# Nelarius/rayfinder

Hardware: AMD Instinct MI355X
Metric: Mrays/sec at 1920x1080 Sponza, 8 bounces; achieved HBM GB/s on traversal (higher is better)
Workload: dtype f32

## Files before the change

rayfinder_amd/csrc/rf_device.hpp:

```cpp
#pragma once

#include "rf_types.hpp"

#include <hip/hip_runtime.h>

namespace rf
{
constexpr int      kBlock = 256;
constexpr int      kLdsStack = 24;
constexpr int      kSpillStack = 72;
constexpr uint32_t kMiss = 0xFFFFFFFFu;
constexpr uint32_t kLeafAxis = 3u;
constexpr uint32_t kTriStride = 4u;

struct DeviceScene
{
    const float4*            nodes;
    const float4*            triangles;
    const float4*            attributes;
    const float4*            shadeRecords;
    const TextureDescriptor* textureDescriptors;
    const uint32_t*          texels;
    uint64_t                 numTexels;
    const uint8_t*           blueNoise;
    const float*             albedoLut;
};

#if defined(__HIPCC__)
struct RayPrep
{
    Vec3     origin;
    Vec3     direction;
    Vec3     invDir;
    uint32_t negX, negY, negZ;
};

__device__ __forceinline__ RayPrep prepareRay(Vec3 o, Vec3 d)
{
    RayPrep r;
    r.origin = o;
    r.direction = d;
    r.invDir = vec3(1.0f / d.x, 1.0f / d.y, 1.0f / d.z);
    r.negX = r.invDir.x < 0.0f;
    r.negY = r.invDir.y < 0.0f;
    r.negZ = r.invDir.z < 0.0f;
    return r;
}

__device__ __forceinline__ bool slabTest(const RayPrep& r, float4 lo, float4 hi, float rayTMax)
{
    float       tmin = ((r.negX ? hi.x : lo.x) - r.origin.x) * r.invDir.x;
    float       tmax = ((r.negX ? lo.x : hi.x) - r.origin.x) * r.invDir.x;
    const float tymin = ((r.negY ? hi.y : lo.y) - r.origin.y) * r.invDir.y;
    const float tymax = ((r.negY ? lo.y : hi.y) - r.origin.y) * r.invDir.y;
    if ((tmin > tymax) || (tymin > tmax)) return false;
    tmin = maxf(tymin, tmin);
    tmax = minf(tymax, tmax);
    const float tzmin = ((r.negZ ? hi.z : lo.z) - r.origin.z) * r.invDir.z;
    const float tzmax = ((r.negZ ? lo.z : hi.z) - r.origin.z) * r.invDir.z;
    if ((tmin > tzmax) || (tzmin > tmax)) return false;
    tmin = maxf(tzmin, tmin);
    tmax = minf(tzmax, tmax);
    return (tmin < rayTMax) && (tmax > 0.0f);
}

__device__ __forceinline__ Vec3 offsetRay(Vec3 p, Vec3 n)
{
    constexpr float kOrigin = 1.0f / 32.0f;
    constexpr float kFloatScale = 1.0f / 65536.0f;
    constexpr float kIntScale = 256.0f;
    const int       ox = static_cast<int>(kIntScale * n.x);
    const int       oy = static_cast<int>(kIntScale * n.y);
    const int       oz = static_cast<int>(kIntScale * n.z);
    const Vec3      shifted = vec3(__int_as_float(__float_as_int(p.x) + (p.x < 0 ? -ox : ox)),
                                   __int_as_float(__float_as_int(p.y) + (p.y < 0 ? -oy : oy)),
                                   __int_as_float(__float_as_int(p.z) + (p.z < 0 ? -oz : oz)));
    return vec3(fabsf(p.x) < kOrigin ? p.x + kFloatScale * n.x : shifted.x,
                fabsf(p.y) < kOrigin ? p.y + kFloatScale * n.y : shifted.y,
                fabsf(p.z) < kOrigin ? p.z + kFloatScale * n.z : shifted.z);
}

struct TriangleHit
{
    float t, u, v;
};

__device__ __forceinline__ bool
intersectTriangle(Vec3 origin, Vec3 direction, Vec3 p0, Vec3 p1, Vec3 p2, float rayTMax, TriangleHit& hit)
{
    constexpr float kEpsilon = 0.00001f;
    const Vec3      e1 = p1 - p0;
    const Vec3      e2 = p2 - p0;
    const Vec3      h = cross(direction, e2);
    const float     det = dot(e1, h);
    if (det > -kEpsilon && det < kEpsilon) return false;
    const float invDet = 1.0f / det;
    const Vec3  s = origin - p0;
    const float u = invDet * dot(s, h);
    if (u < 0.0f || u > 1.0f) return false;
    const Vec3  q = cross(s, e1);
    const float v = invDet * dot(direction, q);
    if (v < 0.0f || u + v > 1.0f) return false;
    const float t = invDet * dot(e2, q);
    if (t > kEpsilon && t < rayTMax)
    {
        hit.t = t;
        hit.u = u;
        hit.v = v;
        return true;
    }
    return false;
}
__device__ __forceinline__ bool
intersectTriangle(const RayPrep& r, Vec3 p0, Vec3 p1, Vec3 p2, float rayTMax, TriangleHit& hit)
{
    return intersectTriangle(r.origin, r.direction, p0, p1, p2, rayTMax, hit);
}

struct ClosestHit
{
    uint32_t triangle;
    float    t, u, v;
    Vec3     p;
};

struct TraversalCounters
{
    uint32_t nodesVisited = 0;
    uint32_t triangleTests = 0;
    uint32_t stackHigh = 0;
    uint32_t abandoned = 0;
};

template<bool ANY_HIT, bool COUNT, int LDS = kLdsStack>
__device__ __forceinline__ bool traverse(const DeviceScene& scene, Vec3 origin, Vec3 direction, float rayTMax,
                                         uint32_t* ldsStackLane, ClosestHit& out, TraversalCounters& counters)
{
    const RayPrep ray = prepareRay(origin, direction);
    constexpr int kSpill = kLdsStack + kSpillStack - LDS;
    uint32_t      spill[kSpill];
    int           stackSize = 0;
    uint32_t      current = 0;
    bool          found = false;
    out.triangle = kMiss;

    for (;;)
    {
        const float4 lo = scene.nodes[2 * current];
        const float4 hi = scene.nodes[2 * current + 1];
        if (COUNT) ++counters.nodesVisited;
        bool advance = false;
        if (slabTest(ray, lo, hi, rayTMax))
        {
            const uint32_t link = __float_as_uint(lo.w);
            const uint32_t meta = __float_as_uint(hi.w);
            const uint32_t axis = meta & 3u;
            if (axis == kLeafAxis)
            {
                const uint32_t count = meta >> 2;
                for (uint32_t i = 0; i < count; ++i)
                {
                    const uint32_t tri = link + i;
                    const float4   a = scene.triangles[kTriStride * tri];
                    const float4   b = scene.triangles[kTriStride * tri + 1];
                    const float4   c = scene.triangles[kTriStride * tri + 2];
                    if (COUNT) ++counters.triangleTests;
                    TriangleHit th;
                    const Vec3  p0 = vec3(a.x, a.y, a.z), p1 = vec3(b.x, b.y, b.z), p2 = vec3(c.x, c.y, c.z);
                    if (intersectTriangle(ray, p0, p1, p2, rayTMax, th))
                    {
                        if (ANY_HIT) return true;
                        rayTMax = th.t;
                        found = true;
                        const Vec3 e1 = p1 - p0, e2 = p2 - p0;
                        const Vec3 p = p0 + th.u * e1 + th.v * e2;
                        const Vec3 n = normalize(cross(e1, e2));
                        out.p = offsetRay(p, n);
                        out.t = th.t;
// ... 46 lines not shown
    if (x < -745.0) return 0.0;
    const double k = __builtin_rint(x * 1.44269504088896338700e+00);
    double       r = __builtin_fma(-k, 6.93147180369123816490e-01, x);
    r = __builtin_fma(-k, 1.90821492927058770002e-10, r);
    double p = 1.6059043836821613e-10;
    p = __builtin_fma(p, r, 2.08767569878681e-09);
    p = __builtin_fma(p, r, 2.505210838544172e-08);
    p = __builtin_fma(p, r, 2.755731922398589e-07);
    p = __builtin_fma(p, r, 2.7557319223985893e-06);
    p = __builtin_fma(p, r, 2.48015873015873e-05);
    p = __builtin_fma(p, r, 0.0001984126984126984);
    p = __builtin_fma(p, r, 0.001388888888888889);
    p = __builtin_fma(p, r, 0.008333333333333333);
    p = __builtin_fma(p, r, 0.041666666666666664);
    p = __builtin_fma(p, r, 0.16666666666666666);
    p = __builtin_fma(p, r, 0.5);
    p = __builtin_fma(p, r, 1.0);
    p = __builtin_fma(p, r, 1.0);
    return __builtin_ldexp(p, static_cast<int>(k));
}
__device__ __forceinline__ double dReduce(double x, long long& quadrant)
{
    const double k = __builtin_rint(x * 6.36619772367581382433e-01);
    double       r = __builtin_fma(-k, 1.57079632673412561417e+00, x);
    r = __builtin_fma(-k, 6.07710050650619224932e-11, r);
    r = __builtin_fma(-k, 2.02226624879595063154e-21, r);
    quadrant = static_cast<long long>(k);
    return r;
}
__device__ __forceinline__ double dSinCosKernel(double r, bool cosine)
{
    const double z = r * r;
    const double c5 = cosine ? -1.13596475577881948265e-11 : 1.58969099521155010221e-10, c4 = cosine ? 2.08757232129817482790e-09 : -2.50507602534068634195e-08;
    const double c3 = cosine ? -2.75573143513906633035e-07 : 2.75573137070700676789e-06, c2 = cosine ? 2.48015872894767294178e-05 : -1.98412698298579493134e-04;
    const double c1 = cosine ? -1.38888888888741095749e-03 : 8.33333333332248946124e-03, c0 = cosine ? 4.16666666666666019037e-02 : -1.66666666666666324348e-01;
    const double t = c0 + z * (c1 + z * (c2 + z * (c3 + z * (c4 + z * c5))));
    return cosine ? (1.0 - 0.5 * z) + (z * z) * t : r + (r * z) * t;
}
__device__ __forceinline__ double dSin(double x)
{
    if (!(__builtin_fabs(x) < 1.0e15)) return x - x;
    long long    q;
    const double r = dReduce(x, q), v = dSinCosKernel(r, (q & 1) != 0);
    return (q & 2) ? -v : v;
}
__device__ __forceinline__ double dCos(double x)
{
    if (!(__builtin_fabs(x) < 1.0e15)) return x - x;
    long long    q;
    const double r = dReduce(x, q), v = dSinCosKernel(r, (q & 1) == 0);
    return ((q + 1) & 2) ? -v : v;
}
__device__ __forceinline__ double dAcosRatio(double z)
{
    const double p = z * (1.66666666666666657415e-01 + z * (-3.25565818622400915405e-01 + z * (2.01212532134862925881e-01 + z * (-4.00555345006794114027e-02 + z * (7.91534994289814532176e-04 + z * 3.47933107596021167570e-05)))));
    const double q = 1.0 + z * (-2.40339491173441421878e+00 + z * (2.02094576023350569471e+00 + z * (-6.88283971605453293030e-01 + z * 7.70381505559019352791e-02)));
    return p / q;
}
__device__ __forceinline__ double dAcos(double x)
{
    const double pio2_hi = 1.57079632679489655800e+00, pio2_lo = 6.12323399573676603587e-17, pi = 3.14159265358979311600e+00;
    if (x != x) return x;
    if (__builtin_fabs(x) >= 1.0)
    {
        if (x == 1.0) return 0.0;
        if (x == -1.0) return pi + 2.0 * pio2_lo;
        return (x - x) / (x - x);
    }
    const bool   small = __builtin_fabs(x) < 0.5, negative = x < 0.0;
    if (small && __builtin_fabs(x) <= 6.938893903907228e-18) return pio2_hi + pio2_lo;
    const double z = small ? x * x : (negative ? (1.0 + x) * 0.5 : (1.0 - x) * 0.5);
    const double r = dAcosRatio(z);
    if (small) return pio2_hi - (x - (pio2_lo - x * r));
    const double s = __builtin_sqrt(z);
    if (negative)
    {
        const double w = r * s - pio2_lo;
        return pi - 2.0 * (s + w);
    }
    const double df = __longlong_as_double(__double_as_longlong(s) & static_cast<long long>(0xFFFFFFFF00000000ull));
    const double c = (z - df * df) / (s + df), w = r * s + c;
    return 2.0 * (df + w);
}
__device__ __forceinline__ float wSin(float x) { return static_cast<float>(dSin(static_cast<double>(x))); }
__device__ __forceinline__ float wCos(float x) { return static_cast<float>(dCos(static_cast<double>(x))); }
__device__ __forceinline__ float wAcos(float x) { return static_cast<float>(dAcos(static_cast<double>(x))); }
__device__ __forceinline__ float wExp(float x) { return static_cast<float>(dExp(static_cast<double>(x))); }
__device__ __forceinline__ float wPow(float x, float y)
{
    return static_cast<float>(pow(static_cast<double>(x), static_cast<double>(y)));
}
__device__ __forceinline__ float wPow15(float x)
{
    const double xd = static_cast<double>(x);
    return static_cast<float>(xd * __builtin_sqrt(xd));
}
__device__ __forceinline__ float wFract(float x) { return x - floorf(x); }

template<bool F32> __device__ __forceinline__ float tSin(float x) { if constexpr (F32) return sinf(x); else return wSin(x); }
template<bool F32> __device__ __forceinline__ float tCos(float x) { if constexpr (F32) return cosf(x); else return wCos(x); }
template<bool F32> __device__ __forceinline__ float tAcos(float x) { if constexpr (F32) return acosf(x); else return wAcos(x); }
template<bool F32> __device__ __forceinline__ float tExp(float x) { if constexpr (F32) return expf(x); else return wExp(x); }
template<bool F32> __device__ __forceinline__ float tPow15(float x) { if constexpr (F32) return powf(x, 1.5f); else return wPow15(x); }

constexpr float kPi = 3.1415927f;
constexpr float kFrac1Pi = 0.31830987f;
constexpr float kTMax = 10000.0f;
constexpr uint32_t kSolarCosThetaMaxBits = 0x3F7FFF5Au;
constexpr uint32_t kSolarInvPdfBits = 0x38826048u;

__host__ __device__ __forceinline__ void pixarOnb(Vec3 n, Vec3& u, Vec3& v)
{
    const float s = (n.z >= 0.0f) ? 1.0f : -1.0f;
    const float a = -1.0f / (s + n.z);
    const float b = n.x * n.y * a;
    u = vec3(1.0f + s * n.x * n.x * a, s * b, -s * n.x);
    v = vec3(b, s + n.y * n.y * a, -n.y);
}

__device__ __forceinline__ Vec3 basisTimes(Vec3 c0, Vec3 c1, Vec3 c2, Vec3 v)
{
    return (v.x * c0 + v.y * c1) + v.z * c2;
}

template<bool F32 = false>
__device__ __forceinline__ float skyRadiance(const SkyStateGpu& sky, float cosTheta, float gamma, float cosGamma, int channel)
{
    const float  r = sky.skyRadiances[channel];
    const float* p = sky.params + 9 * channel;
    const float  cosGamma2 = cosGamma * cosGamma;
    const float  expM = tExp<F32>(p[4] * gamma);
    const float  mieLhs = 1.0f + cosGamma2;
    const float  mieRhs = tPow15<F32>(1.0f + p[8] * p[8] - 2.0f * p[8] * cosGamma);
    const float  mie = mieLhs / mieRhs;
    const float  zenith = rf_sqrt(cosTheta);
    const float  lhs = 1.0f + p[0] * tExp<F32>(p[1] / (cosTheta + 0.01f));
    const float  rhs = p[2] + p[3] * expM + p[5] * cosGamma2 + p[6] * mie + p[7] * zenith;
    return r * (lhs * rhs);
}

__device__ __forceinline__ Vec3 evalTexture(const DeviceScene& scene, const float* lut, uint32_t descriptorIdx, float uvx, float uvy)
{
    const TextureDescriptor d = scene.textureDescriptors[descriptorIdx];
    const float             u = wFract(uvx);
    const float             v = wFract(uvy);
    const uint32_t          j = static_cast<uint32_t>(u * static_cast<float>(d.width));
    const uint32_t          i = static_cast<uint32_t>(v * static_cast<float>(d.height));
    uint64_t                idx = static_cast<uint64_t>(d.offset) + static_cast<uint64_t>(i * d.width + j);
    if (idx >= scene.numTexels) idx = scene.numTexels - 1;
    const uint32_t bgra = scene.texels[idx];
    return vec3(lut[(bgra >> 16) & 0xffu], lut[(bgra >> 8) & 0xffu], lut[bgra & 0xffu]);
}

__device__ __forceinline__ void animatedBlueNoiseN(const uint8_t* table, uint32_t x, uint32_t y, uint32_t n, float& nx, float& ny)
{
    const uint32_t idx = (y % 128u) * 128u + (x % 128u);
    const float    bx = static_cast<float>(table[2 * idx]) / 255.0f;
    const float    by = static_cast<float>(table[2 * idx + 1]) / 255.0f;
    const float    a1 = 0.7548776662466927f;
    const float    a2 = 0.5698402909980532f;
    nx = wFract(bx + wFract(a1 * static_cast<float>(n)));
    ny = wFract(by + wFract(a2 * static_cast<float>(n)));
}
__device__ __forceinline__ void animatedBlueNoise(const uint8_t* table, uint32_t x, uint32_t y, uint32_t frameIdx, uint32_t totalSampleCount, float& nx, float& ny)
{
    animatedBlueNoiseN(table, x, y, frameIdx % totalSampleCount, nx, ny);
}
#endif
}
```

rayfinder_amd/csrc/rf_kernels.hpp:

```cpp
#pragma once

#include "rf_renderer.hpp"

#include "rf_bvh.hpp"
#include "rf_camera.hpp"
#include "rf_data.hpp"
#include "rf_device.hpp"
#include "rf_hip_host.hpp"
#include "rf_wide.hpp"

#include <hip/hip_runtime.h>

#include <algorithm>
#include <cfloat>
#include <cmath>
#include <cstdio>
#include <cstdlib>
#include <cstring>
#include <functional>
#include <stdexcept>
#include <string>
#include <type_traits>

namespace rf
{
namespace kern
{
struct __attribute__((packed, aligned(4))) P3
{
    float x, y, z;
};

struct PathStreams
{
    P3*     rayO;
    P3*     rayD;
    P3*     thr;
    float4* rad;
    float4* hit;
    P3*     pending;
    P3*     noise;
    P3*     rayDOut;
    P3*     thrOut;
    P3*     noiseOut;
};

typedef float v3f __attribute__((ext_vector_type(3)));
__device__ __forceinline__ Vec3 load3(const float4* p)
{
    const v3f v = *reinterpret_cast<const v3f*>(p);
    return vec3(v.x, v.y, v.z);
}
__device__ __forceinline__ Vec3 load3(const P3* p)
{
    const P3 v = *p;
    return vec3(v.x, v.y, v.z);
}
__device__ __forceinline__ void store3(P3* p, Vec3 v)
{
    P3 o;
    o.x = v.x, o.y = v.y, o.z = v.z;
    *p = o;
}
typedef float v3fu __attribute__((ext_vector_type(3), aligned(4)));
__device__ __forceinline__ void store3nt(P3* p, Vec3 v)
{
    v3fu o;
    o.x = v.x, o.y = v.y, o.z = v.z;
    __builtin_nontemporal_store(o, reinterpret_cast<v3fu*>(p));
}
__device__ __forceinline__ Vec3 load3nt(const P3* p)
{
    const v3fu v = __builtin_nontemporal_load(reinterpret_cast<const v3fu*>(p));
    return vec3(v.x, v.y, v.z);
}

__device__ __forceinline__ Vec3     load3s(const float4* p) { return load3(p); }
__device__ __forceinline__ Vec3     load3s(const P3* p) { return load3(p); }
__device__ __forceinline__ uint32_t loadQ(const uint32_t* p) { return *p; }
__device__ __forceinline__ void     store4s(float4* p, float x, float y, float z, float w) { *p = make_float4(x, y, z, w); }

struct DeviceCounters
{
    unsigned long long primaryRays, closestRays, shadowRays;
    unsigned long long closestNodeVisits, closestTriangleTests, shadowNodeVisits, shadowTriangleTests;
    unsigned int       stackHigh;
    unsigned int       pad;
    unsigned long long closestRecordFetches, shadowRecordFetches;
    unsigned long long descendTrips[2], leafTrips[2], leafPhases[2], refillTrips[2], popLaneTrips[2], outerTrips[2];
    unsigned long long scalarRedo[2];
    unsigned long long abandonedRays;
    unsigned long long occluderTried, occluderHit, occludedRays;
    unsigned long long descendParked[2], descendIdle[2], leafInterior[2], leafIdle[2];
};

struct FastDiv
{
    uint32_t mul, shift1, shift2, divisor;
    static FastDiv make(uint32_t d)
    {
        FastDiv f{0u, 0u, 0u, d ? d : 1u};
        uint32_t l = 0;
        while ((1ull << l) < f.divisor) ++l;
        f.mul = static_cast<uint32_t>(((1ull << 32) * ((1ull << l) - f.divisor)) / f.divisor + 1ull);
        f.shift1 = l < 1u ? l : 1u;
        f.shift2 = l > 1u ? l - 1u : 0u;
        return f;
    }
    __host__ __device__ __forceinline__ uint32_t div(uint32_t n) const
    {
#if defined(__HIP_DEVICE_COMPILE__)
        const uint32_t t = __umulhi(mul, n);
#else
        const uint32_t t = static_cast<uint32_t>((static_cast<uint64_t>(mul) * n) >> 32);
#endif
        return (t + ((n - t) >> shift1)) >> shift2;
    }
    __host__ __device__ __forceinline__ void divmod(uint32_t n, uint32_t& q, uint32_t& r) const
    {
        q = div(n);
        r = n - q * divisor;
    }
};

struct FrameParams
{
    uint32_t width, height;
    Camera   camera;
    uint32_t samplesPerPixel, numBounces;
    uint32_t firstFrame;
    uint32_t numSamples;
    uint32_t numTiles;
    uint32_t pixelsPadded;
    uint32_t slotGroupShift;
    const uint32_t* samplePerm;
    const uint32_t* sampleInvPerm;
    uint32_t tilesX;
    uint32_t skipOrigins;
    const uint32_t* tileValidBefore;
    uint32_t        validPixels;
    FastDiv         divNumSamples, divPixelsPadded, divTilesX, divSamplesPerPixel;
};

__device__ __forceinline__ uint32_t validRankInTile(uint32_t w, uint32_t vw, uint32_t vh)
{
    const uint32_t block = w >> 6, lane = w & 63u, bx = block & 3u, by = block >> 2, lx = lane & 7u, ly = lane >> 3;
    const uint32_t ch = min(8u, vh - min(vh, 8u * by)), cw = min(8u, vw - min(vw, 8u * bx));
    return vw * min(vh, 8u * by) + ch * min(vw, 8u * bx) + cw * ly + lx;
}

constexpr uint32_t kSlotSampleMajor = 31u;

__device__ __forceinline__ void slotToSamplePixel(const FrameParams& fp, uint32_t slot, uint32_t& k, uint32_t& lp)
{
    if (fp.slotGroupShift == kSlotSampleMajor) fp.divPixelsPadded.divmod(slot, k, lp);
    else
    {
        const uint32_t g = fp.slotGroupShift, chunk = slot >> g;
        uint32_t       group;
        fp.divNumSamples.divmod(chunk, group, k);
        lp = (group << g) + (slot & ((1u << g) - 1u));
    }
}
__device__ __forceinline__ size_t samplePixelToSlot(const FrameParams& fp, uint32_t k, uint32_t lp)
{
    if (fp.slotGroupShift == kSlotSampleMajor) return static_cast<size_t>(k) * fp.pixelsPadded + lp;
    const uint32_t g = fp.slotGroupShift;
    return ((static_cast<size_t>(lp >> g) * fp.numSamples + k) << g) + (lp & ((1u << g) - 1u));
}

__device__ __forceinline__ bool localPixelToXY(const FrameParams& fp, const uint32_t* tileIds, uint32_t lp, uint32_t& x, uint32_t& y)
{
    const uint32_t tile = tileIds[lp >> 10];
    const uint32_t w = lp & 1023u;
    const uint32_t block = w >> 6, lane = w & 63u;
    uint32_t       tileX, tileY;
    fp.divTilesX.divmod(tile, tileY, tileX);
    x = tileX * kTileSize + (block & 3u) * 8u + (lane & 7u);
    y = tileY * kTileSize + (block >> 2) * 8u + (lane >> 3);
    return x < fp.width && y < fp.height;
}

constexpr int kItems = 4;

template<int ITEMS>
__device__ __forceinline__ void blockAppend(const bool (&keep)[ITEMS], const uint32_t (&slot)[ITEMS], uint32_t* queue, uint32_t* count, uint32_t* sScratch,
                                            uint32_t (*position)[ITEMS] = nullptr, const uint32_t (*second)[ITEMS] = nullptr, uint32_t* queue2 = nullptr)
{
    const uint32_t lane = __lane_id(), wave = threadIdx.x >> 6;
    uint32_t       offs[ITEMS];
    uint32_t       waveTotal = 0;
#pragma unroll
    for (int k = 0; k < ITEMS; ++k)
    {
        const unsigned long long mask = __ballot(keep[k]);
        offs[k] = waveTotal + __popcll(mask & ((1ull << lane) - 1ull));
        waveTotal += __popcll(mask);
    }
    if (lane == 0) sScratch[wave] = waveTotal;
    __syncthreads();
    if (threadIdx.x == 0)
    {
        const uint32_t total = sScratch[0] + sScratch[1] + sScratch[2] + sScratch[3];
        sScratch[4] = total ? atomicAdd(count, total) : 0u;
    }
    __syncthreads();
    uint32_t base = sScratch[4];
    for (uint32_t w = 0; w < wave; ++w) base += sScratch[w];
#pragma unroll
    for (int k = 0; k < ITEMS; ++k)
    {
        if (keep[k]) queue[base + offs[k]] = slot[k];
        if (second != nullptr && keep[k]) queue2[base + offs[k]] = (*second)[k];
        if (position) (*position)[k] = base + offs[k];
    }
    __syncthreads();
}

__device__ __forceinline__ unsigned long long waveSum(unsigned long long v)
{
    for (int off = 32; off > 0; off >>= 1) v += __shfl_down(v, off);
    return v;
}
__device__ __forceinline__ uint32_t waveMax(uint32_t v)
{
    for (int off = 32; off > 0; off >>= 1) v = max(v, static_cast<uint32_t>(__shfl_down(v, off)));
    return v;
}

template<bool MAX>
__device__ __forceinline__ uint32_t waveScanInclusive(uint32_t x)
{
    const auto step = [&](auto ctrl, auto rowMask) {
        const uint32_t y = static_cast<uint32_t>(__builtin_amdgcn_update_dpp(0, static_cast<int>(x), decltype(ctrl)::value, decltype(rowMask)::value, 0xF, true));
        x = MAX ? max(x, y) : x + y;
    };
    step(std::integral_constant<int, 0x111>{}, std::integral_constant<int, 0xF>{});
    step(std::integral_constant<int, 0x112>{}, std::integral_constant<int, 0xF>{});
    step(std::integral_constant<int, 0x114>{}, std::integral_constant<int, 0xF>{});
    step(std::integral_constant<int, 0x118>{}, std::integral_constant<int, 0xF>{});
    step(std::integral_constant<int, 0x142>{}, std::integral_constant<int, 0xA>{});
    step(std::integral_constant<int, 0x143>{}, std::integral_constant<int, 0xC>{});
    return x;
}
__device__ __forceinline__ uint32_t laneGather(uint32_t value, uint32_t srcLane) { return static_cast<uint32_t>(__builtin_amdgcn_ds_bpermute(static_cast<int>(srcLane << 2), static_cast<int>(value))); }
__device__ __forceinline__ float    laneGather(float value, uint32_t srcLane) { return __uint_as_float(laneGather(__float_as_uint(value), srcLane)); }

__device__ __forceinline__ uint32_t sampleKey(uint32_t firstFrame, uint32_t spp, uint32_t k)
{
    const uint32_t n = (firstFrame + k) % spp;
    const float    rx = wFract(0.7548776662466927f * static_cast<float>(n)), ry = wFract(0.5698402909980532f * static_cast<float>(n));
    uint32_t       x = static_cast<uint32_t>(rx * 65536.0f) & 0xFFFFu, y = static_cast<uint32_t>(ry * 65536.0f) & 0xFFFFu;
    const auto     spread = [](uint32_t v) {
        v = (v | (v << 8)) & 0x00FF00FFu;
        v = (v | (v << 4)) & 0x0F0F0F0Fu;
        v = (v | (v << 2)) & 0x33333333u;
        v = (v | (v << 1)) & 0x55555555u;
        return v;
    };
    return spread(x) | (spread(y) << 1);
}

__device__ __forceinline__ Vec3 hitPoint(const DeviceScene& scene, uint32_t tri, float u, float v)
{
    const Vec3 p0 = load3(scene.triangles + kTriStride * tri), p1 = load3(scene.triangles + kTriStride * tri + 1),
               p2 = load3(scene.triangles + kTriStride * tri + 2);
    const Vec3   e1 = p1 - p0, e2 = p2 - p0;
    const Vec3   p = p0 + u * e1 + v * e2;
    return offsetRay(p, normalize(cross(e1, e2)));
}

struct SunBasis
{
    Vec3 u, v;
};

__device__ __forceinline__ Vec3 sunSample(const SkyStateGpu& sky, const SunBasis& basis, float nx, float cosPhi, float sinPhi)
{
    const float cosThetaMax = __uint_as_float(kSolarCosThetaMaxBits);
    const float cosTheta = 1.0f - nx * (1.0f - cosThetaMax);
    const float sinTheta = rf_sqrt(1.0f - cosTheta * cosTheta);
    const Vec3  local = vec3(cosPhi * sinTheta, sinPhi * sinTheta, cosTheta);
    const Vec3  sun = vec3(sky.sunDirection[0], sky.sunDirection[1], sky.sunDirection[2]);
    return basisTimes(basis.u, basis.v, sun, local);
}

constexpr uint32_t kShadeLastBounce = 1u, kShadeFirstBounce = 2u;
constexpr uint32_t kShadeSelfShadow = 4u;
constexpr uint32_t kLookFirstBounce = 1u, kLookNoRayCount = 2u;


constexpr uint32_t kSortBins = 256;
#if defined(RF_EXP_ACC_PIXELS)
constexpr uint32_t kAccPixels = RF_EXP_ACC_PIXELS;
#else
constexpr uint32_t kAccPixels = 4;
#endif
constexpr uint32_t kAccMaxSamples = 1024;
constexpr uint32_t kAovPixels = 8, kAovChunk = 32;

constexpr uint32_t kChunk = 128;
constexpr uint32_t kShards = 16;
constexpr uint32_t kLineWords = 16;
constexpr uint32_t kRefillMin = 40;
constexpr uint32_t kLeafVote = 20;

constexpr int kLayoutBinary = 0, kLayoutCompact = 1, kLayoutHot = 2, kLayoutQuad = 3, kLayoutQuadHalf = 4, kLayoutQuadLocal = 5, kLayoutOct = 6, kLayoutScalar = 7, kLayoutPacket = 8;
constexpr uint32_t kFlagShadowDirFromStream = 1u;
constexpr uint32_t kFlagUniformTri = 8u;
constexpr uint32_t kFlagUniformFetch = 4u;
constexpr uint32_t kFlagFirstBounce = 2u;
constexpr uint32_t kFlagOccluderCache = 16u;
constexpr uint32_t kFlagOccluderNoTry = 32u;
constexpr uint32_t kFlagNoRayCount = 64u;
constexpr uint32_t kFlagConstOrigin = 128u;
constexpr uint32_t kFlagDenseLeafShift = 8u;
#if defined(RF_EXP_OCC_SLOTS)
constexpr int kOccSlots = RF_EXP_OCC_SLOTS;
#else
constexpr int kOccSlots = 4;
#endif
static_assert(kOccSlots == 1 || kOccSlots == 2 || kOccSlots == 4, "one aligned load per cell");
constexpr uint32_t kNodeIdle = 0xFFFFFFFFu;
constexpr uint32_t kNodeDone = 0xFFFFFFFEu;


using SamplePermutationKernel = void (*)(uint32_t firstFrame, uint32_t spp, uint32_t numSamples, uint32_t* perm, uint32_t* inv);
using RaygenKernel = void (*)(FrameParams fp, DeviceScene scene, const uint32_t* tileIds, PathStreams ps, uint32_t* queue, uint32_t* queueCount, DeviceCounters* counters);
using TraceClosestKernel = void (*)(DeviceScene scene, PathStreams ps, const uint32_t* queue, const uint32_t* queueCount, DeviceCounters* counters);
using ShadeKernel = void (*)(DeviceScene scene, SkyStateGpu sky, SunBasis sunBasis, PathStreams ps, const uint32_t* queue, const uint32_t* queueCount, uint32_t* hitQueue, uint32_t* hitCount, uint32_t* missQueue, uint32_t* missSlots, uint32_t* missCount, uint32_t* shadowList, uint32_t* shadowListCount, uint32_t bounceFlags, uint32_t sortScale, float4* aov);
using SkyKernel = void (*)(SkyStateGpu sky, PathStreams ps, const uint32_t* missSlots, const uint32_t* missQueue, const uint32_t* missCount, uint32_t firstBounce);
using TraceShadowKernel = void (*)(DeviceScene scene, SkyStateGpu sky, SunBasis sunBasis, PathStreams ps, const uint32_t* queue, const uint32_t* queueCount, DeviceCounters* counters, uint32_t firstBounce);
using TraceWideKernel = void (*)(DeviceScene scene, WideScene wide, SkyStateGpu sky, SunBasis sunBasis, PathStreams ps, const uint32_t* queue, const uint32_t* queueCount, uint32_t* cursor, DeviceCounters* counters, uint32_t refillMin, uint32_t leafVote, uint32_t chunkMax, float tMax, uint32_t flags);
using ShadowFirstLookKernel = void (*)(DeviceScene scene, WideScene wide, SkyStateGpu sky, SunBasis sunBasis, PathStreams ps, const uint32_t* queue, const uint32_t* inList, const uint32_t* inCount, uint32_t* list, uint32_t* listCount, DeviceCounters* counters, float tMax, uint32_t flags);
using TracePacketKernel = void (*)(DeviceScene scene, WideScene wide, SkyStateGpu sky, SunBasis sunBasis, PathStreams ps, const uint32_t* queue, const uint32_t* queueCount, DeviceCounters* counters, float tMax, uint32_t flags);
using HitPointsKernel = void (*)(DeviceScene scene, const float4* hit, P3* rayO, uint32_t n);
using BounceTotalsKernel = void (*)(const uint32_t* queueCounts, uint32_t numBounces, unsigned long long* totals, const uint32_t* listCounts, unsigned long long lookMask, unsigned long long* lookBatch, const uint32_t* shadowListCounts, unsigned long long selfMask, DeviceCounters* counters);
using AccumulateKernel = void (*)(FrameParams fp, const uint32_t* tileIds, PathStreams ps, float4* image);
using AccumulateRunsKernel = void (*)(FrameParams fp, const uint32_t* tileIds, PathStreams ps, float4* image);
using AccumulateAovKernel = void (*)(FrameParams fp, const uint32_t* tileIds, const float4* aov, float4* albedoCoverage, float4* normalDepth);
using TonemapKernel = void (*)(const float4* image, uint32_t n, uint32_t accumulatedSamples, float exposure, uint32_t* out);
using PrimaryStatsKernel = void (*)(DeviceScene scene, Camera cam, uint32_t width, uint32_t height, uint32_t* nodesVisited, uint8_t* hitOut, float* tOut, uint32_t* triTests, DeviceCounters* counters);
using IntersectRaysKernel = void (*)(DeviceScene scene, const float* rays, uint64_t n, float tMax, uint32_t* triOut, float* tOut, float* uvOut, float* pOut, uint32_t* nvOut, uint32_t* ttOut, DeviceCounters* counters);
using OccludedRaysKernel = void (*)(DeviceScene scene, const float* rays, uint64_t n, float tMax, float* visOut, DeviceCounters* counters);
using DeferredLightingKernel = void (*)(DeviceScene scene, SkyStateGpu sky, SunBasis sunBasis, Camera cam, uint32_t width, uint32_t height, uint32_t frameCount, float jitterX, float jitterY, float exposure, float* sampleBuffer, float* accumulationBuffer, uint32_t* bgraOut, DeviceCounters* counters);

TraceWideKernel       traceWideKernel(bool anyHit, bool count, bool nearestFirst, int compact, bool denseLeaves);
TraceClosestKernel    traceClosestKernel(bool count);
TraceShadowKernel     traceShadowKernel(bool count);
ShadowFirstLookKernel shadowFirstLookKernel();
TracePacketKernel     tracePacketKernel(bool anyHit);
HitPointsKernel       hitPointsKernel();
PrimaryStatsKernel    primaryStatsKernel();
IntersectRaysKernel   intersectRaysKernel();
OccludedRaysKernel    occludedRaysKernel();
SamplePermutationKernel samplePermutationKernel();
RaygenKernel            raygenKernel(bool f32Transcendentals);
ShadeKernel             shadeKernel(bool sorted, bool aov = false);
SkyKernel               skyKernel(bool f32Transcendentals);
BounceTotalsKernel      bounceTotalsKernel();
AccumulateKernel        accumulateKernel();
AccumulateRunsKernel    accumulateRunsKernel(uint32_t pixelsPerWorkgroup);
AccumulateAovKernel     accumulateAovKernel(bool runs);
TonemapKernel           tonemapKernel();
DeferredLightingKernel  deferredLightingKernel();
}
using namespace kern;
}
```

rayfinder_amd/csrc/rf_renderer.hip:

```cpp
#include "rayfinder_amd.h"
#include "rf_denoise.hpp"
#include "rf_kernels.hpp"
#include "rf_noise.hpp"

#include <map>

#include <algorithm>
#include <cfloat>
#include <cmath>
#include <cstdio>
#include <cstdlib>
#include <cstring>
#include <functional>
#include <stdexcept>
#include <string>
#include <type_traits>

namespace rf
{
bool operator==(const RenderParameters& a, const RenderParameters& b)
{
    return a.width == b.width && a.height == b.height && std::memcmp(&a.camera, &b.camera, sizeof(Camera)) == 0 &&
           a.samplingParams == b.samplingParams && a.sky == b.sky && a.exposure == b.exposure;
}

namespace
{
uint32_t tileMortonKey(uint32_t tx, uint32_t ty)
{
    const auto spread = [](uint32_t v) {
        v &= 0xFFFFu;
        v = (v | (v << 8)) & 0x00FF00FFu;
        v = (v | (v << 4)) & 0x0F0F0F0Fu;
        v = (v | (v << 2)) & 0x33333333u;
        v = (v | (v << 1)) & 0x55555555u;
        return v;
    };
    return spread(tx) | (spread(ty) << 1);
}
}

std::vector<uint32_t> tilesForRank(uint32_t width, uint32_t height, uint32_t rank, uint32_t worldSize)
{
    const uint32_t tilesX = TileGrid(width, height).tilesX, n = TileGrid(width, height).count();
    std::vector<uint32_t> order(n);
    for (uint32_t i = 0; i < n; ++i) order[i] = i;
    if (worldSize > 1)
    {
        std::stable_sort(order.begin(), order.end(), [tilesX](uint32_t a, uint32_t b) { return tileMortonKey(a % tilesX, a / tilesX) < tileMortonKey(b % tilesX, b / tilesX); });
    }
    std::vector<uint32_t> mine;
    for (uint32_t i = 0; i < n; ++i)
        if ((i % worldSize + i / worldSize) % worldSize == rank) mine.push_back(order[i]);
    std::sort(mine.begin(), mine.end());
    return mine;
}

void untileHost(const float* compact, const uint32_t* tileIds, uint32_t numTiles, uint32_t width, uint32_t height, float* image)
{
    untileHostTexels(compact, tileIds, numTiles, width, height, 4 * sizeof(float), image);
}

void untileHostTexels(const void* compact, const uint32_t* tileIds, uint32_t numTiles, uint32_t width, uint32_t height, size_t texelBytes, void* image)
{
    const uint32_t tilesX = TileGrid(width, height).tilesX;
    const auto*    src = static_cast<const unsigned char*>(compact);
    auto*          dst = static_cast<unsigned char*>(image);
    for (uint32_t t = 0; t < numTiles; ++t)
    {
        const uint32_t tx = tileIds[t] % tilesX, ty = tileIds[t] / tilesX;
        for (uint32_t w = 0; w < kTileSize * kTileSize; ++w)
        {
            const uint32_t block = w >> 6, lane = w & 63u;
            const uint32_t x = tx * kTileSize + (block & 3u) * 8u + (lane & 7u);
            const uint32_t y = ty * kTileSize + (block >> 2) * 8u + (lane >> 3);
            if (x >= width || y >= height) continue;
            std::memcpy(dst + texelBytes * (static_cast<size_t>(y) * width + x), src + texelBytes * (static_cast<size_t>(t) * 1024 + w), texelBytes);
        }
    }
}

struct SumChannel
{
    bool                 on = false;
    bool                 dirty = true;
    uint32_t             samples = 0;
    DeviceBuffer<float4> buffers[2];
    uint32_t             numBuffers = 0;

    SumChannel(bool on_, uint32_t numBuffers_) : on(on_), numBuffers(numBuffers_) {}
    void restart()
    {
        samples = 0;
        dirty = true;
    }
    void release()
    {
        for (auto& b : buffers) b.release();
    }
    bool covers(uint32_t accumulated) const { return !dirty && samples == accumulated; }
    bool empty() const { return !on || dirty || samples == 0u; }
    void zeroIfStale(hipStream_t stream, uint64_t pixelsPadded)
    {
        if (!on || !dirty) return;
        if (numBuffers != 0u && buffers[0].count < pixelsPadded)
        {
            RF_HIP(hipStreamSynchronize(stream));
            for (uint32_t i = 0; i < numBuffers; ++i) buffers[i].alloc(pixelsPadded);
        }
        for (uint32_t i = 0; i < numBuffers; ++i) RF_HIP(hipMemsetAsync(buffers[i].ptr, 0, pixelsPadded * sizeof(float4), stream));
        dirty = false;
    }
};

struct Renderer::Impl
{
    int         device = 0;
    hipStream_t stream = nullptr;

    DeviceBuffer<float4>            nodes, triangles, wideNodes, wideCompact, wideHot, wideOwn, wideQuad;
    DeviceBuffer<uint4>             wideQuadHalf, wideQuadLocal, wideOct;
    DeviceBuffer<uint2>             bigLeaves;
    WideScene                       wide{};
    DeviceBuffer<float4>            attributes;
    DeviceBuffer<float4>            shadeRecords;
    DeviceBuffer<TextureDescriptor> textureDescriptors;
    DeviceBuffer<uint32_t>          texels;
    DeviceBuffer<uint8_t>           blueNoise;
    DeviceBuffer<float>             albedoLut;
    DeviceScene                     scene{};

    RenderParameters params;
    SkyStateGpu      sky{};
    SunBasis         sunBasis{};

    void updateSunBasis() { pixarOnb(vec3(sky.sunDirection[0], sky.sunDirection[1], sky.sunDirection[2]), sunBasis.u, sunBasis.v); }
    uint32_t         maxWidth = 0, maxHeight = 0;
    uint32_t         frameCount = 0, accumulated = 0;
    uint32_t         rank = 0, worldSize = 1;

    std::vector<uint32_t>   tiles;
    DeviceBuffer<uint32_t>  tileIds;
    DeviceBuffer<uint32_t>  tileValidBefore;
    bool                    optDenseRaygen = true;
    DeviceBuffer<float4>    ownedImage;
    float4*                 image = nullptr;
    uint64_t                imageBytes = 0;
    SumChannel              imageSums{true, 0};
    SumChannel              aovSums{false, 2};
    uint32_t                aovFlags = 0;
    bool                    aovTileCounts() const { return (aovFlags & kAovTileCounts) != 0u; }
    SumChannel              momentSums{false, 1};
    float4*                 aovAlbedoCoverage() const { return aovSums.buffers[0].ptr; }
    float4*                 aovNormalDepth() const { return aovSums.buffers[1].ptr; }
    float4*                 moments() const { return momentSums.buffers[0].ptr; }
    DenoiseWork             denoiseWork;
    bool                    denoisedValid = false;
    uint32_t                denoisedSamples = 0;
    NoiseWork               noiseWork;
    std::vector<uint32_t>   tileSamples;
    DeviceBuffer<uint32_t>  tileSamplesDevice;
    DeviceBuffer<float4>    meanImage;

    bool nonUniform() const { return !tileSamples.empty(); }
    void requireUniform(const char* what, const char* unless = "") const
    {
        if (nonUniform())
            throw std::invalid_argument(std::string(what) + ": the tiles hold different sample counts after rf_renderer_render_adaptive" + unless +
                                        " (continue with render_adaptive, or restart the accumulation with rf_renderer_set_render_parameters)");
    }

    uint64_t                validPixels = 0;
    unsigned long long      primaryRaysHost = 0;
    uint64_t                maxPaths = 0;
    DeviceBuffer<P3>        sRayO, sRayD, sRayD2, sThr, sThr2, sPending, sNoise, sNoise2;
    DeviceBuffer<float4>    sRad, sHit;
    DeviceBuffer<float4>    sAov;
    DeviceBuffer<uint32_t>  queueA, queueB, missQueue, missSlots, shadowList, queueCounts;
    DeviceBuffer<DeviceCounters> counters;
    DeviceBuffer<unsigned long long> bounceTotals;

    uint32_t               deferredFrameCount = 0;
    DeviceBuffer<float>    deferredSample, deferredAccum;
    DeviceBuffer<uint32_t> deferredBgra;

    bool counting = false, timing = false;
    int      traversalVariant = 2;
    uint32_t wideBlocks = 0;
    bool     wideBlocksForced = false;
    uint32_t multiProcessors = 0;
    std::map<std::pair<const void*, uint32_t>, uint32_t> residentCache;
    uint32_t skyBlocks = 2048;
    bool     wideUsable = true;
    int      queryVariant = 0;
    bool     shadowNearestFirst = true;
    uint32_t optShadowFirstLookFromBounce = 2;
    bool     occluderGridWarm = false;
    DeviceBuffer<unsigned long long> lookBatch;
    unsigned long long*              lookBatchHost = nullptr;
    hipEvent_t                       lookEvent = nullptr;
    bool                             lookPending = false;
    uint32_t                         firstLookHoldOff = 0;
    uint32_t occluderHintLevels = 0;
    bool     leafBoxesValid = false;
    uint32_t optOccluderGridLog2Cells = 22;
    uint32_t optOccluderGridCells = 1024;
    DeviceBuffer<uint32_t> occluderGrid;
    uint32_t optOccluderCacheBounces = 64;
    bool     optShadowSignOrder = true;
    uint32_t optRefillMin = kRefillMin, optLeafVote = kLeafVote, optChunk = kChunk;
    uint32_t optLeafVoteClosest = 14;
    uint32_t optDenseLeafMin = 5, optDenseLeafFromBounce = 1;
    uint32_t maxLeafTriangles = 0;
    uint32_t optShadeSortFromBounce = 2, sortScale = 0;
    uint32_t optChunkEarly = 256, optChunkEarlyBounces = 2;
    uint32_t optRefillMinDeep = 12, optRefillMinDeepDense = 22, optRefillMinDeepQuad = 40, optRefillDeepFromBounce = 2;
    uint32_t optShadeBlocks = 0;
    bool     optTranscendentalsF32 = false;
    bool     optShadowSelfTest = true;
    bool     selfShadowOk = false;
    bool     optConstPrimaryOrigin = true;
    bool                   optSampleSort = true, optAccumulateRuns = true;
    uint32_t               optCompactFromBounce = 3;
    uint32_t               optCompactShadowFromBounce = 2;
    uint32_t               optQuadFromBounce = 1, optQuadShadowFromBounce = 1;
    uint32_t               optQuadExceptMask = 0, optQuadShadowExceptMask = 0;
    uint32_t               optQuadHalfFromBounce = 0, optQuadHalfShadowFromBounce = 0;
    float                  quadHalfAreaRatio = 0.0f;
    uint32_t               optQuadLocalFromBounce = 0, optQuadLocalShadowFromBounce = 0;
    uint32_t               optOctFromBounce = 0;
    uint64_t               treeBytes = 0;
    uint32_t               optHotFromBounce = 0, optHotShadowFromBounce = 0;
    int                    optQueryCompact = 0;
    uint32_t               optExtraLds = 0;
    uint32_t               optPacketBounces = 0;
    int                    optUniformFetch = 2;
    DeviceBuffer<uint32_t> samplePerm;
    uint32_t optSlotGroupShift = 0;
    RenderStats hostStats;

    struct TimedLaunch
    {
        hipEvent_t start, stop;
        int        kind;
        uint32_t   bounce;
    };
    std::vector<TimedLaunch> timed;
    std::vector<hipEvent_t>  eventPool;

    struct BatchTiming
    {
        hipEvent_t start, stop;
        uint32_t   samples;
    };
    std::vector<BatchTiming> pendingBatches;
    std::deque<float>        passDurationsMs;

    hipEvent_t getEvent()
    {
        if (!eventPool.empty())
        {
            hipEvent_t e = eventPool.back();
            eventPool.pop_back();
            return e;
        }
        hipEvent_t e;
        RF_HIP(hipEventCreate(&e));
        return e;
    }

    uint64_t allocatedPaths = 0;
    uint64_t effectivePaths = 0;

    static constexpr uint64_t kBytesPerPath = 8 * sizeof(P3) + 2 * sizeof(float4) + 5 * sizeof(uint32_t);
    static constexpr uint64_t kAovBytesPerPath = 2 * sizeof(float4);
    uint64_t bytesPerPath() const { return kBytesPerPath + (aovSums.on ? kAovBytesPerPath : 0u); }
    uint64_t pathStateBytes() const { return allocatedPaths * kBytesPerPath + sAov.count * sizeof(float4); }
    bool pathStateHolds(uint64_t paths) const { return paths <= allocatedPaths && (!aovSums.on || sAov.count >= 2 * paths); }

    void releasePathState()
    {
        sRayO.release(), sRayD.release(), sRayD2.release(), sThr.release(), sThr2.release(), sRad.release(), sHit.release();
        sPending.release(), sNoise.release(), sNoise2.release(), queueA.release(), queueB.release(), missQueue.release(), missSlots.release(), shadowList.release();
        sAov.release();
        allocatedPaths = 0;
    }

    bool ensurePathState(uint64_t paths)
    {
        if (pathStateHolds(paths)) return true;
        RF_HIP(hipStreamSynchronize(stream));
        releasePathState();
        const auto tryAlloc = [](auto& buf, uint64_t n) -> bool {
            void* p = nullptr;
            const hipError_t e = hipMalloc(&p, n * sizeof(*buf.ptr));
            if (e == hipErrorOutOfMemory || e == hipErrorMemoryAllocation)
            {
                (void)hipGetLastError();
                return false;
            }
            RF_HIP(e);
            buf.ptr = static_cast<decltype(buf.ptr)>(p);
            buf.count = n;
            return true;
        };
        const bool ok = tryAlloc(sRayO, paths) && tryAlloc(sRayD, paths) && tryAlloc(sRayD2, paths) && tryAlloc(sThr, paths) && tryAlloc(sThr2, paths) &&
                        tryAlloc(sRad, paths) && tryAlloc(sHit, paths) && tryAlloc(sPending, paths) && tryAlloc(sNoise, paths) && tryAlloc(sNoise2, paths) &&
                        tryAlloc(queueA, paths) && tryAlloc(queueB, paths) && tryAlloc(missQueue, paths) && tryAlloc(missSlots, paths) && tryAlloc(shadowList, paths) &&
                        (!aovSums.on || tryAlloc(sAov, 2 * paths));
        if (!ok)
        {
            releasePathState();
            return false;
        }
        allocatedPaths = paths;
        return true;
    }

    uint64_t pathsThatFit()
    {
        size_t freeBytes = 0, totalBytes = 0;
        RF_HIP(hipMemGetInfo(&freeBytes, &totalBytes));
        const uint64_t budget = static_cast<uint64_t>(freeBytes) + pathStateBytes();
        return budget / 10 * 9 / bytesPerPath();
    }

    void configureShard()
    {
// ... 124 lines not shown
        uint32_t occMask;
        bool     firstLookReady;
        bool     runs, tileList;
        uint32_t accumulateKernel, accumulatePixels, aovPixels, momentPixels;
    };
    struct BouncePlan
    {
        TraversalPlan closest, shadow;
        bool          shadeSorted, shadeAov;
        uint32_t      shadeFlags, sortScale, skyFirstBounce;
        uint32_t      itemGridCap;
        bool          cached, firstLook, selfShadow;
        uint32_t      lookFlags, shadowSource;
    };
    struct BatchCounters
    {
        uint32_t*                 base;
        uint32_t                  numBounces;
        static constexpr uint32_t kLine = kLineWords, kCursorWords = kLine * kShards;
        uint32_t words() const { return kLine * (2 * numBounces + 1) + kCursorWords * 2 * numBounces + kLine * numBounces + kLine * numBounces; }
        uint32_t queueWord(uint32_t b) const { return kLine * b; }
        uint32_t missWord(uint32_t b) const { return kLine * (numBounces + 1) + kLine * (b - 1); }
        uint32_t cursorClosestWord(uint32_t b) const { return kLine * (2 * numBounces + 1) + kCursorWords * 2 * (b - 1); }
        uint32_t cursorShadowWord(uint32_t b) const { return cursorClosestWord(b) + kCursorWords; }
        uint32_t listWord(uint32_t b) const { return kLine * (2 * numBounces + 1) + kCursorWords * 2 * numBounces + kLine * (b - 1); }
        uint32_t shadowListWord(uint32_t b) const { return listWord(b) + kLine * numBounces; }
        uint32_t shadowCountWord(uint32_t b, uint32_t source) const { return source == kFromLookList ? listWord(b) : (source == kFromShadeList ? shadowListWord(b) : queueWord(b)); }
        uint32_t* queueCount(uint32_t b) const { return base + queueWord(b); }
        uint32_t* missCount(uint32_t b) const { return base + missWord(b); }
        uint32_t* cursorClosest(uint32_t b) const { return base + cursorClosestWord(b); }
        uint32_t* cursorShadow(uint32_t b) const { return base + cursorShadowWord(b); }
        uint32_t* listCount(uint32_t b) const { return base + listWord(b); }
        uint32_t* shadowListCount(uint32_t b) const { return base + shadowListWord(b); }
        uint32_t* shadowCount(uint32_t b, uint32_t source) const { return base + shadowCountWord(b, source); }
    };
    struct WideArgs
    {
        PathStreams     ps;
        const uint32_t* queue;
        const uint32_t* count;
        uint32_t*       cursor;
        float           tMax;
        dim3            grid;
        uint32_t        blocksWanted = 0;
    };
    uint32_t residentBlocks(TraceWideKernel k, uint32_t extraLds)
    {
        const auto key = std::make_pair(reinterpret_cast<const void*>(k), extraLds);
        const auto it = residentCache.find(key);
        if (it != residentCache.end()) return it->second;
        int perCu = 0;
        RF_HIP(hipOccupancyMaxActiveBlocksPerMultiprocessor(&perCu, reinterpret_cast<const void*>(k), kBlock, extraLds));
        const uint32_t n = static_cast<uint32_t>(std::max(perCu, 1)) * std::max(multiProcessors, 1u);
        residentCache[key] = n;
        return n;
    }
    void launchWide(const TraversalPlan& t, const WideScene& w, const WideArgs& a)
    {
        const TraceWideKernel k = traceWideKernel(t.anyHit, t.count, t.nearest, t.layout, t.dense);
        if (k == nullptr) throw std::logic_error("kTraceWide: record layout " + std::to_string(t.layout) + " is not compiled into this build");
        dim3 grid = a.grid;
        if (a.blocksWanted != 0u && !wideBlocksForced && !t.count) grid = dim3(std::min(a.blocksWanted, residentBlocks(k, t.extraLds)));
        hipLaunchKernelGGL(k, grid, dim3(kBlock), t.extraLds, stream, scene, w, sky, sunBasis, a.ps, a.queue, a.count, a.cursor, counters.ptr, t.refillMin, t.leafVote, t.chunk, a.tMax, t.flags);
    }
    int layoutIfPresent(int want) const
    {
        switch (want)
        {
        case kLayoutOct: return wide.oct != nullptr ? want : kLayoutBinary;
        case kLayoutQuadLocal: return wide.quadLocal != nullptr ? want : kLayoutBinary;
        case kLayoutQuadHalf: return wide.quadHalf != nullptr ? want : kLayoutBinary;
        case kLayoutQuad: return wide.quad != nullptr ? want : kLayoutBinary;
        case kLayoutHot: return wide.hot != nullptr ? want : kLayoutBinary;
        case kLayoutCompact: return wide.compact != nullptr ? want : kLayoutBinary;
        default: return kLayoutBinary;
        }
    }
    bool denseWanted(uint32_t flags) const
    {
        const uint32_t threshold = (flags >> kFlagDenseLeafShift) & 15u;
        return threshold != 0u && maxLeafTriangles >= threshold;
    }
    static bool conservativeLayout(int layout) { return layout == kLayoutQuadLocal || layout == kLayoutQuadHalf; }
    static bool worksThroughList(int layout) { return layout == kLayoutQuad || layout == kLayoutQuadHalf || layout == kLayoutQuadLocal; }
    TraversalPlan resolveTraversal(bool anyHit, int layout, bool count, bool nearest, uint32_t flags, uint32_t refillMin, uint32_t chunk, uint32_t leafVote, uint32_t extraLds) const
    {
        TraversalPlan t{};
        t.kernel = layout == kLayoutScalar ? kKernelScalar : (layout == kLayoutPacket ? kKernelPacket : kKernelWide);
        t.layout = layout, t.anyHit = anyHit, t.count = count, t.flags = flags;
        if (t.kernel != kKernelWide) return t;
        if (count) t.layout = kLayoutBinary, t.nearest = anyHit && nearest;
        else if (!anyHit) t.layout = layout <= kLayoutOct ? layout : kLayoutBinary;
        else
        {
            t.layout = (layout <= kLayoutQuadLocal) ? layout : kLayoutBinary;
            t.nearest = (t.layout == kLayoutCompact || t.layout == kLayoutHot) ? true : nearest;
        }
        t.dense = !count && denseWanted(flags) && traceWideKernel(anyHit, false, t.nearest, t.layout, true) != nullptr;
        t.refillMin = refillMin, t.chunk = chunk, t.leafVote = leafVote ? leafVote : optLeafVote, t.extraLds = extraLds;
        return t;
    }
    int closestLayoutFor(uint32_t bounce) const
    {
        if (traversalVariant == 0) return kLayoutScalar;
        if (counting) return kLayoutBinary;
#if defined(RF_EXP_LEGACY_LAYOUTS)
        if (bounce <= optPacketBounces) return kLayoutPacket;
#endif
        const bool  quadNow = wide.quad != nullptr && optQuadFromBounce != 0u && bounce >= optQuadFromBounce && !((optQuadExceptMask >> std::min(bounce - 1u, 31u)) & 1u);
        const float camReach = std::max({std::fabs(params.camera.origin.x), std::fabs(params.camera.origin.y), std::fabs(params.camera.origin.z)}) + (std::fabs(params.camera.lensRadius) * 2.0f);
        const bool  primaryOutside = bounce == 1u && !(camReach <= wide.originBound);
        if (quadNow && !primaryOutside)
        {
            if (wide.oct != nullptr && optOctFromBounce != 0u && bounce >= optOctFromBounce) return kLayoutOct;
            if (wide.quadHalf != nullptr && optQuadHalfFromBounce != 0u && bounce >= optQuadHalfFromBounce) return kLayoutQuadHalf;
            if (wide.quadLocal != nullptr && optQuadLocalFromBounce != 0u && bounce >= optQuadLocalFromBounce) return kLayoutQuadLocal;
        }
        if (quadNow) return kLayoutQuad;
        if (wide.hot != nullptr && optHotFromBounce != 0u && bounce >= optHotFromBounce) return kLayoutHot;
        if (wide.compact != nullptr && optCompactFromBounce != 0u && bounce >= optCompactFromBounce) return kLayoutCompact;
        return kLayoutBinary;
    }
    int shadowLayoutFor(uint32_t bounce) const
    {
        if (traversalVariant == 0) return kLayoutScalar;
#if defined(RF_EXP_LEGACY_LAYOUTS)
        if (!counting && bounce <= optPacketBounces) return kLayoutPacket;
#endif
        if (counting || !shadowNearestFirst) return kLayoutBinary;
        const bool quadShadowNow = optQuadShadowFromBounce != 0u && bounce >= optQuadShadowFromBounce && !((optQuadShadowExceptMask >> std::min(bounce - 1u, 31u)) & 1u);
        if (quadShadowNow)
        {
            if (wide.quadLocal != nullptr && optQuadLocalShadowFromBounce != 0u && bounce >= optQuadLocalShadowFromBounce) return kLayoutQuadLocal;
            if (wide.quadHalf != nullptr && optQuadHalfShadowFromBounce != 0u && bounce >= optQuadHalfShadowFromBounce) return kLayoutQuadHalf;
            if (wide.quad != nullptr) return kLayoutQuad;
        }
        if (wide.hot != nullptr && optHotShadowFromBounce != 0u && bounce >= optHotShadowFromBounce) return kLayoutHot;
        if (wide.compact != nullptr && optCompactShadowFromBounce != 0u && bounce >= optCompactShadowFromBounce) return kLayoutCompact;
        return kLayoutBinary;
    }
    bool cachedShadowFor(uint32_t bounce) const
    {
        const int layout = shadowLayoutFor(bounce);
        const bool exactQuad = layout == kLayoutQuad && leafBoxesValid;
        return layout != kLayoutScalar && layout != kLayoutPacket && !counting && shadowNearestFirst && (conservativeLayout(layout) || exactQuad) && bounce <= optOccluderCacheBounces &&
               optOccluderGridCells != 0u;
    }

    struct ActiveTiles
    {
        uint32_t numTiles;
        uint64_t validPixels;
    };
    BatchPlan planBatch(uint32_t numSamples, const ActiveTiles* active) const
    {
        BatchPlan b{};
        const uint64_t validPixels = active ? active->validPixels : this->validPixels;
        b.numSamples = numSamples;
        b.numBounces = params.samplingParams.numBounces;
        b.numTiles = active ? active->numTiles : static_cast<uint32_t>(tiles.size());
        b.pixelsPadded = b.numTiles * 1024u;
        b.samplePerm = optSampleSort && numSamples > 1 && numSamples <= 8192 && optSlotGroupShift != kSlotSampleMajor;
        const auto finite3 = [](Vec3 v) { return std::isfinite(v.x) && std::isfinite(v.y) && std::isfinite(v.z); };
        const Camera& camNow = params.camera;
        b.primaryLayout = closestLayoutFor(1);
        b.constOrigin = optConstPrimaryOrigin && camNow.lensRadius == 0.0f && camNow.origin.x != 0.0f && camNow.origin.y != 0.0f && camNow.origin.z != 0.0f &&
                        finite3(camNow.origin) && finite3(camNow.right) && finite3(camNow.up) && b.primaryLayout != kLayoutScalar && b.primaryLayout != kLayoutPacket;
        b.denseRaygen = optDenseRaygen && (optSlotGroupShift == 0u || optSlotGroupShift == kSlotSampleMajor) && static_cast<uint64_t>(validPixels) * numSamples <= 0xFFFFFFFFull;
        b.occluderGrid = optOccluderCacheBounces != 0u && optOccluderGridCells != 0u;
        if (b.occluderGrid)
        {
            b.occluderGridEntries = (uint64_t{1} << optOccluderGridLog2Cells) * kOccSlots;
            const float extent = std::max({wide.rootHi.x - wide.rootLo.x, wide.rootHi.y - wide.rootLo.y, wide.rootHi.z - wide.rootLo.z, 1e-20f});
            b.occScale = static_cast<float>(optOccluderGridCells) / extent;
            b.occMask = static_cast<uint32_t>(b.occluderGridEntries / kOccSlots - 1);
        }
        b.runs = optSlotGroupShift == 0u && numSamples > 4u && optAccumulateRuns;
        b.tileList = active != nullptr;
        const uint32_t perThread = static_cast<uint32_t>(kBlock);
        if (b.tileList) b.accumulateKernel = kAccumulateTiles, b.accumulatePixels = b.runs ? kMomentPixels : perThread;
        else if (b.runs && numSamples <= kAccMaxSamples)
        {
            b.accumulateKernel = kAccumulateRuns, b.accumulatePixels = numSamples > 640u ? 1u : (numSamples > 160u ? 2u : kAccPixels);
        }
        else b.accumulateKernel = kAccumulatePixels, b.accumulatePixels = perThread;
        b.aovPixels = (aovSums.on && b.numBounces != 0u) ? (b.runs ? kAovPixels : perThread) : 0u;
        b.momentPixels = (!b.tileList && momentSums.on) ? (b.runs ? kMomentPixels : perThread) : 0u;
        return b;
    }
    bool nextBatchFirstLookReady(const BatchPlan& b) const
    {
        if (!b.occluderGrid || occluderGrid.count != b.occluderGridEntries || !occluderGridWarm) return false;
        if (lookPending && hipEventQuery(lookEvent) == hipSuccess) return !(lookBatchHost[1] != 0ull && lookBatchHost[0] * 4ull < lookBatchHost[1]) && firstLookHoldOff == 0u;
        return firstLookHoldOff <= 1u;
    }
    BouncePlan planBounce(uint32_t bounce, const BatchPlan& batch) const
    {
        BouncePlan p{};
        const uint32_t uniformFlag = ((optUniformFetch < 0 ? bounce <= 2 : optUniformFetch > 0) ? kFlagUniformFetch : 0u) | (optUniformFetch >= 2 ? kFlagUniformTri : 0u) |
                                     (bounce >= optDenseLeafFromBounce ? (std::min(optDenseLeafMin, 15u) << kFlagDenseLeafShift) : 0u);
        const uint32_t chunkNow = bounce <= optChunkEarlyBounces ? optChunkEarly : optChunk;
        const int      layoutClosest = closestLayoutFor(bounce);
        const uint32_t refillClosest = bounce >= optRefillDeepFromBounce ? (layoutClosest == kLayoutQuad ? optRefillMinDeepQuad : (denseWanted(uniformFlag) ? optRefillMinDeepDense : optRefillMinDeep)) : optRefillMin;
        const uint32_t leafVoteClosest = (!counting && !denseWanted(uniformFlag) && treeBytes <= (192ull << 20)) ? optLeafVoteClosest : 0u;
        const bool     wideClosest = layoutClosest != kLayoutScalar && layoutClosest != kLayoutPacket;
        p.closest = resolveTraversal(false, layoutClosest, counting, false, wideClosest ? (uniformFlag | (bounce == 1 && batch.constOrigin ? kFlagConstOrigin : 0u)) : 0u,
                                     counting ? optRefillMin : refillClosest, chunkNow, leafVoteClosest, counting ? 0u : optExtraLds);
        const int layoutShadow = shadowLayoutFor(bounce);
        p.selfShadow = optShadowSelfTest && selfShadowOk && !counting && bounce <= 64u && worksThroughList(layoutShadow);
        p.shadeAov = aovSums.on && bounce == 1;
        p.shadeSorted = !p.shadeAov && optShadeSortFromBounce != 0u && bounce >= optShadeSortFromBounce;
        p.shadeFlags = (bounce == batch.numBounces ? kShadeLastBounce : 0u) | (bounce == 1 ? kShadeFirstBounce : 0u) | (p.selfShadow ? kShadeSelfShadow : 0u);
        p.sortScale = p.shadeSorted ? sortScale : 0u;
        p.skyFirstBounce = bounce == 1 ? 1u : 0u;
        p.itemGridCap = optShadeBlocks;
        p.cached = cachedShadowFor(bounce);
        p.firstLook = p.cached && occluderHintLevels == 0u && optShadowFirstLookFromBounce != 0u && bounce >= optShadowFirstLookFromBounce && bounce <= 64u && batch.firstLookReady;
        p.shadowSource = p.firstLook ? kFromLookList : (p.selfShadow ? kFromShadeList : kFromQueue);
        p.lookFlags = p.firstLook ? ((bounce == 1 ? kLookFirstBounce : 0u) | (p.selfShadow ? kLookNoRayCount : 0u)) : 0u;
        const uint32_t shadowFlags = (bounce == 1 ? kFlagFirstBounce : 0u) | uniformFlag | (p.cached ? kFlagOccluderCache : 0u) | (p.firstLook ? (kFlagOccluderNoTry | kFlagNoRayCount) : 0u) | (p.selfShadow ? kFlagNoRayCount : 0u);
        const bool nearest = shadowNearestFirst && !(conservativeLayout(layoutShadow) && optShadowSignOrder);
        const uint32_t flagsRun = layoutShadow == kLayoutScalar ? (bounce == 1 ? 1u : 0u) : (layoutShadow == kLayoutPacket ? (shadowFlags & kFlagFirstBounce) : shadowFlags);
        p.shadow = resolveTraversal(true, layoutShadow, counting, nearest, flagsRun, optRefillMin, chunkNow, 0u, counting ? 0u : optExtraLds);
        return p;
    }

    void queryWide(const float* rays6, uint64_t n, float tMax, bool shadow, std::vector<float4>& out0, std::vector<float4>& out1)
    {
        if (n > 0xFFFFFFFFull) throw std::runtime_error("too many rays");
        const uint32_t denseFlag = std::min(optDenseLeafMin, 15u) << kFlagDenseLeafShift;
        if (!ensurePathState(n)) throw std::runtime_error("out of device memory for the ray batch");
        std::vector<P3>       o(n), d(n);
        std::vector<uint32_t> ids(n);
        for (uint64_t i = 0; i < n; ++i)
        {
            o[i] = P3{rays6[6 * i], rays6[6 * i + 1], rays6[6 * i + 2]};
            d[i] = P3{rays6[6 * i + 3], rays6[6 * i + 4], rays6[6 * i + 5]};
            ids[i] = static_cast<uint32_t>(i);
        }
        RF_HIP(hipStreamSynchronize(stream));
        RF_HIP(hipMemcpyAsync(sRayO.ptr, o.data(), n * sizeof(P3), hipMemcpyHostToDevice, stream));
        RF_HIP(hipMemcpyAsync(sRayD.ptr, d.data(), n * sizeof(P3), hipMemcpyHostToDevice, stream));
        RF_HIP(hipMemcpyAsync(queueA.ptr, ids.data(), n * sizeof(uint32_t), hipMemcpyHostToDevice, stream));
        const BatchCounters qc{nullptr, 0u};
        const uint32_t words = qc.words() + BatchCounters::kCursorWords;
        if (queueCounts.count < words) queueCounts.alloc(words);
        RF_HIP(hipMemsetAsync(queueCounts.ptr, 0, queueCounts.count * sizeof(uint32_t), stream));
        const uint32_t count = static_cast<uint32_t>(n);
        RF_HIP(hipMemcpyAsync(queueCounts.ptr, &count, sizeof count, hipMemcpyHostToDevice, stream));
        PathStreams ps{sRayO.ptr, sRayD.ptr, sThr.ptr, sRad.ptr, sHit.ptr, sPending.ptr, sNoise.ptr, sRayD2.ptr, sThr2.ptr, sNoise2.ptr};
        const dim3  grid(std::min<uint32_t>(static_cast<uint32_t>((n + kBlock - 1) / kBlock), wideBlocks));
        const WideArgs wa{ps, queueA.ptr, queueCounts.ptr + qc.queueWord(0), queueCounts.ptr + qc.cursorClosestWord(1), tMax, grid};
        if (shadow)
        {
            std::vector<P3> ones(n, P3{1.0f, 1.0f, 1.0f});
            RF_HIP(hipMemcpyAsync(sPending.ptr, ones.data(), n * sizeof(P3), hipMemcpyHostToDevice, stream));
            RF_HIP(hipMemsetAsync(sRad.ptr, 0, n * sizeof(float4), stream));
            RF_HIP(hipStreamSynchronize(stream));
            const int layout = layoutIfPresent((optQueryCompact == kLayoutOct || (!shadowNearestFirst && optQueryCompact < kLayoutQuad)) ? kLayoutBinary : optQueryCompact);
            launchWide(resolveTraversal(true, layout, false, shadowNearestFirst, kFlagShadowDirFromStream | denseFlag, optRefillMin, optChunk, 0u, 0u), wide, wa);
        }
        else
        {
            WideScene wq = wide;
            wq.rayList = nullptr;
            if (const char* listPath = std::getenv("RF_DEBUG_QUERY_LIST"))
            {
                std::vector<uint32_t> list(n);
                FILE* f = std::fopen(listPath, "rb");
                if (f == nullptr || std::fread(list.data(), sizeof(uint32_t), n, f) != n) throw std::runtime_error("RF_DEBUG_QUERY_LIST: cannot read the ray list");
                std::fclose(f);
                RF_HIP(hipMemcpyAsync(queueB.ptr, list.data(), n * sizeof(uint32_t), hipMemcpyHostToDevice, stream));
                RF_HIP(hipStreamSynchronize(stream));
                wq.rayList = queueB.ptr;
            }
            const bool timed = std::getenv("RF_DEBUG_QUERY_MS") != nullptr;
            hipEvent_t e0 = nullptr, e1 = nullptr;
            if (timed)
            {
                RF_HIP(hipEventCreate(&e0));
                RF_HIP(hipEventCreate(&e1));
                RF_HIP(hipEventRecord(e0, stream));
            }
            launchWide(resolveTraversal(false, layoutIfPresent(optQueryCompact), false, false, denseFlag, optRefillMin, optChunk, 0u, 0u), wq, wa);
            if (timed) RF_HIP(hipEventRecord(e1, stream));
            hipLaunchKernelGGL(hitPointsKernel(), dim3((count + 255) / 256), dim3(256), 0, stream, scene, sHit.ptr, sRayO.ptr, count);
            if (timed)
            {
                RF_HIP(hipStreamSynchronize(stream));
                float ms = 0.0f;
                RF_HIP(hipEventElapsedTime(&ms, e0, e1));
                std::fprintf(stderr, "[rf-query] closest-hit launch: %u rays, %.4f ms\n", count, ms);
                RF_HIP(hipEventDestroy(e0));
                RF_HIP(hipEventDestroy(e1));
            }
        }
        RF_HIP(hipGetLastError());
        RF_HIP(hipStreamSynchronize(stream));
        out0.resize(n);
        RF_HIP(hipMemcpy(out0.data(), shadow ? sRad.ptr : sHit.ptr, n * sizeof(float4), hipMemcpyDeviceToHost));
        if (!shadow)
        {
            std::vector<P3> packed(n);
            RF_HIP(hipMemcpy(packed.data(), sRayO.ptr, n * sizeof(P3), hipMemcpyDeviceToHost));
            out1.resize(n);
            for (uint64_t i = 0; i < n; ++i) out1[i] = make_float4(packed[i].x, packed[i].y, packed[i].z, 0.0f);
        }
    }

    void clearStaleSums(uint64_t pixelsPadded)
    {
        zeroImageIfStale(pixelsPadded * sizeof(float4));
        aovSums.zeroIfStale(stream, pixelsPadded);
        momentSums.zeroIfStale(stream, pixelsPadded);
    }

    uint32_t batchSamples(uint32_t todo, uint64_t pixelsPadded)
    {
        uint32_t       n = 0;
        uint64_t       depth = maxPaths;
        for (;;)
        {
            const uint32_t perBatch = static_cast<uint32_t>(std::max<uint64_t>(1, depth / pixelsPadded));
            const uint32_t numBatches = (todo + perBatch - 1) / perBatch;
            n = (todo + numBatches - 1) / numBatches;
            const uint64_t need = static_cast<uint64_t>(n) * pixelsPadded;
            if (pathStateHolds(need)) break;
            const uint64_t fit = pathsThatFit();
            if (need > fit && n > 1)
            {
                depth = std::max<uint64_t>(pixelsPadded, std::min(depth / 2, fit));
                continue;
            }
            if (ensurePathState(need)) break;
            if (n == 1) throw std::runtime_error("out of device memory: one sample of the frame (" + std::to_string(need * bytesPerPath() >> 20) + " MiB of path state) does not fit");
            depth = std::max<uint64_t>(pixelsPadded, depth / 2);
        }
        if (depth != effectivePaths)
        {
            if (depth < maxPaths)
                std::fprintf(stderr, "[rf] device memory is short: batches of %llu paths instead of the configured %llu (%u samples per batch); same image, shorter launches\n",
                             static_cast<unsigned long long>(depth), static_cast<unsigned long long>(maxPaths), n);
            else if (effectivePaths != 0 && effectivePaths < maxPaths)
                std::fprintf(stderr, "[rf] device memory is back: batches of the configured %llu paths again\n", static_cast<unsigned long long>(maxPaths));
            effectivePaths = depth;
        }
        return n;
    }

    const uint32_t* uploadTileSamples()
    {
        RF_HIP(hipStreamSynchronize(stream));
        if (tileSamplesDevice.count < tileSamples.size()) tileSamplesDevice.alloc(tileSamples.size());
        RF_HIP(hipMemcpy(tileSamplesDevice.ptr, tileSamples.data(), tileSamples.size() * sizeof(uint32_t), hipMemcpyHostToDevice));
        return tileSamplesDevice.ptr;
    }
    const float4* meanOnDevice()
    {
        const uint32_t n = static_cast<uint32_t>(tiles.size() * 1024);
        RF_HIP(hipStreamSynchronize(stream));
        if (meanImage.count < n) meanImage.alloc(n);
        zeroImageIfStale(static_cast<size_t>(n) * sizeof(float4));
        const uint32_t* counts = nonUniform() ? uploadTileSamples() : nullptr;
        hipLaunchKernelGGL(tileMeanKernel(), dim3((n + 255) / 256), dim3(256), 0, stream, static_cast<const float4*>(image), counts, accumulated, n, meanImage.ptr);
        RF_HIP(hipGetLastError());
        RF_HIP(hipStreamSynchronize(stream));
        return meanImage.ptr;
    }

    uint64_t uploadTileList(const std::vector<uint32_t>& list)
    {
        const auto [before, valid] = grid().validPrefix(list);
        if (list.size() > tileIds.count || before.size() > tileValidBefore.count) throw std::logic_error("tile list longer than the frame's");
        if (!list.empty()) RF_HIP(hipMemcpy(tileIds.ptr, list.data(), list.size() * sizeof(uint32_t), hipMemcpyHostToDevice));
        RF_HIP(hipMemcpy(tileValidBefore.ptr, before.data(), before.size() * sizeof(uint32_t), hipMemcpyHostToDevice));
        return valid;
    }

    uint32_t step(uint32_t todo, uint64_t pixelsPadded, const ActiveTiles* active)
    {
        const uint32_t n = batchSamples(todo, pixelsPadded);
        traceBatch(frameCount, n, active);
        hostStats.batchSamplesUsed = n, hostStats.batchPathsUsed = static_cast<uint64_t>(n) * pixelsPadded, ++hostStats.batchesTraced;
        frameCount += n;
        accumulated += n;
        if (aovSums.on) aovSums.samples += n;
        if (momentSums.on) momentSums.samples += n;
        return n;
    }

    struct BounceIo
    {
        uint32_t      bounce;
        PathStreams   ps;
        uint32_t*     in;
        uint32_t*     out;
        BatchCounters words;
        uint32_t      blocks, itemBlocks;
        dim3          persistentGrid;
    };
    static dim3 cappedGrid(uint32_t blocks, uint32_t cap) { return dim3(cap ? std::min(blocks, cap) : blocks); }
    void enqueueClosest(const TraversalPlan& t, const BounceIo& io)
    {
        uint32_t* const countIn = io.words.queueCount(io.bounce - 1);
        if (t.kernel == kKernelScalar)
            hipLaunchKernelGGL(traceClosestKernel(t.count), dim3(io.blocks), dim3(kBlock), 0, stream, scene, io.ps, io.in, countIn, counters.ptr);
#if defined(RF_EXP_LEGACY_LAYOUTS)
        else if (t.kernel == kKernelPacket)
            hipLaunchKernelGGL(tracePacketKernel(false), io.persistentGrid, dim3(kBlock), 0, stream, scene, wide, sky, sunBasis, io.ps, io.in, countIn, counters.ptr, kTMax, t.flags);
#endif
        else
            launchWide(t, wide, WideArgs{io.ps, io.in, countIn, io.words.cursorClosest(io.bounce), kTMax, io.persistentGrid, io.blocks});
    }
    void enqueueShadeAndSky(const BouncePlan& p, const BounceIo& io)
    {
        uint32_t* const missCount = io.words.missCount(io.bounce);
        hipLaunchKernelGGL(shadeKernel(p.shadeSorted, p.shadeAov), cappedGrid(io.itemBlocks, p.itemGridCap), dim3(kBlock), 0, stream, scene, sky, sunBasis, io.ps, io.in,
                           io.words.queueCount(io.bounce - 1), io.out, io.words.queueCount(io.bounce), missQueue.ptr, missSlots.ptr, missCount, shadowList.ptr,
                           io.words.shadowListCount(io.bounce), p.shadeFlags, p.sortScale, p.shadeAov ? sAov.ptr : nullptr);
        hipLaunchKernelGGL(skyKernel(optTranscendentalsF32), dim3(std::min(io.blocks, skyBlocks)), dim3(kBlock), 0, stream, sky, io.ps, missSlots.ptr, missQueue.ptr, missCount, p.skyFirstBounce);
    }
    void enqueueShadow(const BouncePlan& p, const BounceIo& io)
    {
        uint32_t* const countOut = io.words.queueCount(io.bounce);
        WideScene       wide = this->wide;
        if (p.firstLook)
        {
            hipLaunchKernelGGL(shadowFirstLookKernel(), cappedGrid(io.itemBlocks, p.itemGridCap), dim3(kBlock), 0, stream, scene, wide, sky, sunBasis, io.ps, io.out,
                               p.selfShadow ? shadowList.ptr : nullptr, io.words.shadowCount(io.bounce, p.selfShadow ? kFromShadeList : kFromQueue), io.in, io.words.listCount(io.bounce),
                               counters.ptr, kTMax, p.lookFlags);
            wide.rayList = io.in;
        }
        else if (p.selfShadow) wide.rayList = shadowList.ptr;
        const TraversalPlan& t = p.shadow;
        if (t.kernel == kKernelScalar)
            hipLaunchKernelGGL(traceShadowKernel(t.count), dim3(io.blocks), dim3(kBlock), 0, stream, scene, sky, sunBasis, io.ps, io.out, countOut, counters.ptr, t.flags);
#if defined(RF_EXP_LEGACY_LAYOUTS)
        else if (t.kernel == kKernelPacket)
            hipLaunchKernelGGL(tracePacketKernel(true), io.persistentGrid, dim3(kBlock), 0, stream, scene, wide, sky, sunBasis, io.ps, io.out, countOut, counters.ptr, kTMax, t.flags);
#endif
        else
            launchWide(t, wide, WideArgs{io.ps, io.out, io.words.shadowCount(io.bounce, p.shadowSource), io.words.cursorShadow(io.bounce), kTMax, io.persistentGrid, io.blocks});
    }
    void enqueueSums(const BatchPlan& b, const FrameParams& fp, const PathStreams& ps)
    {
        const auto sumGrid = [&](uint32_t pixelsPerGroup) { return dim3((fp.pixelsPadded + pixelsPerGroup - 1) / pixelsPerGroup); };
        const dim3 sumBlock(b.runs ? 64u : static_cast<uint32_t>(kBlock));
        if (b.accumulateKernel == kAccumulateTiles)
        {
            hipLaunchKernelGGL(accumulateTilesKernel(b.runs), sumGrid(b.accumulatePixels), sumBlock, 0, stream, fp, tileIds.ptr, static_cast<const float4*>(ps.rad), image, moments());
            if (b.aovPixels != 0u)
                hipLaunchKernelGGL(accumulateTilesAovKernel(b.runs), sumGrid(b.aovPixels), sumBlock, 0, stream, fp, tileIds.ptr, static_cast<const float4*>(sAov.ptr), aovAlbedoCoverage(),
                                   aovNormalDepth());
            return;
        }
        if (b.accumulateKernel == kAccumulateRuns)
            hipLaunchKernelGGL(accumulateRunsKernel(b.accumulatePixels), sumGrid(b.accumulatePixels), dim3(64), b.accumulatePixels * 3u * (b.numSamples + 1u) * sizeof(float), stream, fp,
                               tileIds.ptr, ps, image);
        else
            hipLaunchKernelGGL(accumulateKernel(), sumGrid(b.accumulatePixels), dim3(kBlock), 0, stream, fp, tileIds.ptr, ps, image);
        if (b.aovPixels != 0u)
            hipLaunchKernelGGL(accumulateAovKernel(b.runs), sumGrid(b.aovPixels), sumBlock, 0, stream, fp, tileIds.ptr, sAov.ptr, aovAlbedoCoverage(), aovNormalDepth());
        if (b.momentPixels != 0u)
            hipLaunchKernelGGL(accumulateMomentsKernel(b.runs), sumGrid(b.momentPixels), sumBlock, 0, stream, fp, tileIds.ptr, static_cast<const float4*>(ps.rad), moments());
    }

    void traceBatch(uint32_t firstFrame, uint32_t numSamples, const ActiveTiles* active = nullptr)
    {
        const uint64_t validPixels = active ? active->validPixels : this->validPixels;
        BatchPlan      batch = planBatch(numSamples, active);
        FrameParams    fp{};
        fp.width = params.width;
        fp.height = params.height;
        fp.camera = params.camera;
        fp.samplesPerPixel = params.samplingParams.numSamplesPerPixel;
        fp.numBounces = batch.numBounces;
        fp.firstFrame = firstFrame;
        fp.numSamples = numSamples;
        fp.numTiles = batch.numTiles;
        fp.pixelsPadded = batch.pixelsPadded;
        fp.slotGroupShift = optSlotGroupShift;
        fp.samplePerm = fp.sampleInvPerm = nullptr;
        if (batch.samplePerm)
        {
            if (samplePerm.count < 2ull * numSamples) samplePerm.alloc(2ull * numSamples);
            fp.samplePerm = samplePerm.ptr;
            fp.sampleInvPerm = samplePerm.ptr + numSamples;
        }
        fp.tilesX = grid().tilesX;
        if (fp.numTiles == 0) return;
        fp.divNumSamples = FastDiv::make(fp.numSamples), fp.divPixelsPadded = FastDiv::make(fp.pixelsPadded), fp.divTilesX = FastDiv::make(fp.tilesX);
        fp.divSamplesPerPixel = FastDiv::make(fp.samplesPerPixel);
        fp.skipOrigins = batch.constOrigin ? 1u : 0u;
        fp.tileValidBefore = batch.denseRaygen ? tileValidBefore.ptr : nullptr;
        fp.validPixels = static_cast<uint32_t>(validPixels);
        wide.constOriginX = params.camera.origin.x, wide.constOriginY = params.camera.origin.y, wide.constOriginZ = params.camera.origin.z;

        const uint64_t paths = static_cast<uint64_t>(numSamples) * fp.pixelsPadded;
        const uint32_t blocks = static_cast<uint32_t>((paths + kBlock - 1) / kBlock);
        primaryRaysHost += static_cast<unsigned long long>(numSamples) * validPixels;
        PathStreams    ps{sRayO.ptr, sRayD.ptr, sThr.ptr, sRad.ptr, sHit.ptr, sPending.ptr, sNoise.ptr, sRayD2.ptr, sThr2.ptr, sNoise2.ptr};
        const uint32_t numBounces = fp.numBounces;

        wide.occGrid = nullptr;
        wide.rayList = nullptr;
        if (batch.occluderGrid)
        {
            if (occluderGrid.count != batch.occluderGridEntries)
            {
                occluderGrid.alloc(batch.occluderGridEntries);
                occluderGridWarm = false;
                RF_HIP(hipMemsetAsync(occluderGrid.ptr, 0, batch.occluderGridEntries * sizeof(uint32_t), stream));
            }
            wide.occGrid = occluderGrid.ptr;
            wide.occScale = batch.occScale;
            wide.occMask = batch.occMask;
        }
        if (lookBatch.count == 0)
        {
            lookBatch.alloc(2);
            RF_HIP(hipHostMalloc(reinterpret_cast<void**>(&lookBatchHost), 2 * sizeof(unsigned long long)));
            RF_HIP(hipEventCreateWithFlags(&lookEvent, hipEventDisableTiming));
        }
        if (lookPending && hipEventQuery(lookEvent) == hipSuccess)
        {
            lookPending = false;
            if (lookBatchHost[1] != 0ull && lookBatchHost[0] * 4ull < lookBatchHost[1]) firstLookHoldOff = 16u;
        }
        else if (firstLookHoldOff != 0u) --firstLookHoldOff;
        batch.firstLookReady = occluderGridWarm && firstLookHoldOff == 0u;
        RF_HIP(hipMemsetAsync(lookBatch.ptr, 0, 2 * sizeof(unsigned long long), stream));
        BatchTiming bt{getEvent(), getEvent(), numSamples};
        RF_HIP(hipEventRecord(bt.start, stream));

        const uint32_t countWords = BatchCounters{nullptr, numBounces}.words();
        if (queueCounts.count < countWords) queueCounts.alloc(countWords);
        const BatchCounters words{queueCounts.ptr, numBounces};
        unsigned long long  lookMask = 0ull, selfMask = 0ull;
        const uint32_t      itemBlocks = static_cast<uint32_t>((paths + kBlock * kItems - 1) / (kBlock * kItems));
        RF_HIP(hipMemsetAsync(queueCounts.ptr, 0, queueCounts.count * sizeof(uint32_t), stream));

        BounceIo io{0u, ps, queueA.ptr, queueB.ptr, words, blocks, itemBlocks, dim3(std::min(blocks, wideBlocks))};
        if (fp.samplePerm)
            hipLaunchKernelGGL(samplePermutationKernel(), dim3((numSamples + 255) / 256), dim3(256), 0, stream, firstFrame, fp.samplesPerPixel, numSamples,
                               const_cast<uint32_t*>(fp.samplePerm), const_cast<uint32_t*>(fp.sampleInvPerm));
        launchTimed(0, [&] {
            hipLaunchKernelGGL(raygenKernel(optTranscendentalsF32), dim3(itemBlocks), dim3(kBlock), 0, stream, fp, scene, tileIds.ptr, io.ps, io.in, words.queueCount(0), counters.ptr);
        });
        for (io.bounce = 1; io.bounce <= numBounces; ++io.bounce)
        {
            const BouncePlan plan = planBounce(io.bounce, batch);
            if (plan.selfShadow) selfMask |= 1ull << (io.bounce - 1);
            if (plan.firstLook) lookMask |= 1ull << (io.bounce - 1);
            launchTimed(1, [&] { enqueueClosest(plan.closest, io); }, io.bounce - 1);
            launchTimed(2, [&] { enqueueShadeAndSky(plan, io); });
            launchTimed(3, [&] { enqueueShadow(plan, io); }, io.bounce - 1);
            std::swap(io.in, io.out);
            std::swap(io.ps.rayD, io.ps.rayDOut);
            std::swap(io.ps.thr, io.ps.thrOut);
            std::swap(io.ps.noise, io.ps.noiseOut);
        }
        hipLaunchKernelGGL(bounceTotalsKernel(), dim3(1), dim3(64), 0, stream, words.base, std::min(numBounces, 64u), bounceTotals.ptr, words.listCount(1), lookMask, lookBatch.ptr, words.shadowListCount(1), selfMask, counters.ptr);
        if (lookMask != 0ull && lookBatchHost != nullptr)
        {
            RF_HIP(hipMemcpyAsync(lookBatchHost, lookBatch.ptr, 2 * sizeof(unsigned long long), hipMemcpyDeviceToHost, stream));
            RF_HIP(hipEventRecord(lookEvent, stream));
            lookPending = true;
        }
        if (wide.occGrid != nullptr) occluderGridWarm = true;
        launchTimed(4, [&] { enqueueSums(batch, fp, io.ps); });
        RF_HIP(hipGetLastError());
        RF_HIP(hipEventRecord(bt.stop, stream));
        pendingBatches.push_back(bt);
        if (timing) collectTimings();
        if (pendingBatches.size() > 64) collectBatchTimings();
    }
};

Renderer::Renderer(const RendererDescriptor& desc, const SceneView& sceneView) : mImpl(std::make_unique<Impl>())
{
    Impl& m = *mImpl;
    requireAnyDevice();
    m.device = desc.deviceOrdinal;
    RF_HIP(hipSetDevice(m.device));
    RF_HIP(hipStreamCreateWithFlags(&m.stream, hipStreamNonBlocking));

    if (sceneView.bvhNodes.empty()) throw std::runtime_error("scene has no BVH nodes");
    if (sceneView.positionAttributes.size() != sceneView.vertexAttributes.size())
        throw std::runtime_error("position and vertex attribute counts differ");
    validateScene(sceneView.bvhNodes, sceneView.positionAttributes.size(), sceneView.vertexAttributes, sceneView.baseColorTextures.size());
    m.sortScale = static_cast<uint32_t>(std::min<uint64_t>((static_cast<uint64_t>(kSortBins) << 32) / std::max<uint64_t>(sceneView.positionAttributes.size(), 1), 0xFFFFFFFFull));

    bool                  treeNestedRegular = false;
    std::vector<uint32_t> quadIndexOfNode;
    {
        std::vector<float4> packed(2 * sceneView.bvhNodes.size());
        for (size_t i = 0; i < sceneView.bvhNodes.size(); ++i)
        {
            const BvhNode& n = sceneView.bvhNodes[i];
            const bool     leaf = n.triangleCount > 0;
            if (n.triangleCount >= (1u << 30)) throw std::runtime_error("BVH leaf too large");
            const uint32_t link = leaf ? n.trianglesOffset : n.secondChildOffset;
            const uint32_t meta = leaf ? ((n.triangleCount << 2) | kLeafAxis) : (n.splitAxis & 3u);
            if (!leaf && n.splitAxis > 2) throw std::runtime_error("interior BVH node with invalid split axis");
            packed[2 * i] = make_float4(n.aabb.min.x, n.aabb.min.y, n.aabb.min.z, bitsFloat(link));
            packed[2 * i + 1] = make_float4(n.aabb.max.x, n.aabb.max.y, n.aabb.max.z, bitsFloat(meta));
        }
        m.nodes.upload(packed.data(), packed.size());
        const WideBuild wb = buildWide(sceneView.bvhNodes.data(), sceneView.bvhNodes.size());
        quadIndexOfNode = wb.quadIndexOfNode;
        treeNestedRegular = wb.boxesNested && wb.boxesRegular;
        m.wideNodes.upload(wb.nodes.data(), wb.nodes.size());
        m.bigLeaves.upload(wb.bigLeaves.data(), wb.bigLeaves.size());
        m.wide.nodes = m.wideNodes.ptr;
        m.wide.compact = nullptr;
#if defined(RF_EXP_LEGACY_LAYOUTS)
        if (wb.compactUsable && !wb.compact.empty())
        {
            m.wideCompact.upload(wb.compact.data(), wb.compact.size());
            m.wide.compact = m.wideCompact.ptr;
        }
#endif
        m.wide.hot = m.wide.own = nullptr;
#if defined(RF_EXP_LEGACY_LAYOUTS)
        if (wb.hotUsable && !wb.hot.empty())
        {
            m.wideHot.upload(wb.hot.data(), wb.hot.size());
            m.wideOwn.upload(wb.own.data(), wb.own.size());
            m.wide.hot = m.wideHot.ptr;
            m.wide.own = m.wideOwn.ptr;
        }
#endif
        m.wide.quad = nullptr;
        if (wb.quadUsable && !wb.quad.empty())
        {
            m.wideQuad.upload(wb.quad.data(), wb.quad.size());
            m.wide.quad = m.wideQuad.ptr;
        }
        m.wide.quadHalf = nullptr;
        m.wide.originBound = wb.originBound;
        if (!wb.quadHalf.empty())
        {
            m.wideQuadHalf.upload(wb.quadHalf.data(), wb.quadHalf.size());
            m.wide.quadHalf = m.wideQuadHalf.ptr;
            m.optQuadHalfFromBounce = m.optQuadHalfShadowFromBounce = wb.quadHalfAreaRatio <= kQuadHalfMaxAreaRatio ? 1u : 0u;
            m.quadHalfAreaRatio = wb.quadHalfAreaRatio;
        }
        m.wide.quadLocal = nullptr;
        if (!wb.quadLocal.empty())
        {
            m.wideQuadLocal.upload(wb.quadLocal.data(), wb.quadLocal.size());
            m.wide.quadLocal = m.wideQuadLocal.ptr;
            const float ratio = wb.quadHalf.empty() ? 2.0f : wb.quadHalfAreaRatio;
            m.optQuadLocalFromBounce = m.optQuadHalfFromBounce == 0u ? 2u : 0u;
            m.optQuadLocalShadowFromBounce = ratio <= kQuadLocalShadowMaxAreaRatio ? 2u : 0u;
        }
        m.wide.oct = nullptr;
        m.treeBytes = static_cast<uint64_t>(wb.quadLocal.size()) * sizeof(uint4) + static_cast<uint64_t>(sceneView.positionAttributes.size()) * kTriStride * sizeof(float4);
        if (!wb.oct.empty())
        {
            m.wideOct.upload(wb.oct.data(), wb.oct.size());
            m.wide.oct = m.wideOct.ptr;
            m.optOctFromBounce = 0u;
        }
        m.wide.bigLeaves = m.bigLeaves.ptr;
        m.wide.rootLo = wb.rootLo;
        m.wide.rootHi = wb.rootHi;
        m.wide.rootLeaf = wb.rootLeaf;
        m.wide.numRecords = static_cast<uint32_t>(wb.nodes.size() / 4);
        m.wideUsable = wb.boxesRegular;
    }
    {
        const size_t        n = sceneView.positionAttributes.size();
        std::vector<float4> padded(kTriStride * n, make_float4(0.0f, 0.0f, 0.0f, 0.0f));
        for (size_t i = 0; i < n; ++i)
        {
            const PositionAttribute& t = sceneView.positionAttributes[i];
            padded[kTriStride * i] = make_float4(t.p0.x, t.p0.y, t.p0.z, 0.0f);
            padded[kTriStride * i + 1] = make_float4(t.p1.x, t.p1.y, t.p1.z, 0.0f);
            padded[kTriStride * i + 2] = make_float4(t.p2.x, t.p2.y, t.p2.z, 0.0f);
        }
        {
            std::vector<float> diag;
            diag.reserve(sceneView.bvhNodes.size() / 2 + 1);
            for (const BvhNode& nd : sceneView.bvhNodes)
                if (nd.triangleCount != 0)
                {
                    m.maxLeafTriangles = std::max(m.maxLeafTriangles, nd.triangleCount);
                    const float dx = nd.aabb.max.x - nd.aabb.min.x, dy = nd.aabb.max.y - nd.aabb.min.y, dz = nd.aabb.max.z - nd.aabb.min.z;
                    diag.push_back(std::sqrt(dx * dx + dy * dy + dz * dz));
                }
            const Aabb& root = sceneView.bvhNodes[0].aabb;
            const float extent = std::max({root.max.x - root.min.x, root.max.y - root.min.y, root.max.z - root.min.z});
            m.occluderHintLevels = 0;
            if (!diag.empty() && extent > 0.0f)
            {
                std::nth_element(diag.begin(), diag.begin() + diag.size() / 2, diag.end());
                const float median = diag[diag.size() / 2];
                if (median > 0.0f && std::isfinite(median) && std::isfinite(extent))
                    m.occluderHintLevels = static_cast<uint32_t>(std::clamp(static_cast<int>(std::floor(std::log2(0.003f * extent / median))) + 1, 0, 3));
// ... 1207 lines not shown
```

rayfinder_amd/csrc/rf_shade.hip:

```cpp
#include "rf_kernels.hpp"

namespace rf
{
namespace
{
__global__ void kSamplePermutation(uint32_t firstFrame, uint32_t spp, uint32_t numSamples, uint32_t* perm, uint32_t* inv)
{
    const uint32_t k = blockIdx.x * blockDim.x + threadIdx.x;
    if (k >= numSamples) return;
    const uint32_t mine = sampleKey(firstFrame, spp, k);
    uint32_t       rank = 0;
    for (uint32_t j = 0; j < numSamples; ++j)
    {
        const uint32_t other = sampleKey(firstFrame, spp, j);
        rank += (other < mine || (other == mine && j < k)) ? 1u : 0u;
    }
    perm[rank] = k;
    inv[k] = rank;
}

template<bool F32>
__global__ __launch_bounds__(kBlock) void kRaygen(FrameParams fp, DeviceScene scene, const uint32_t* tileIds, PathStreams ps,
                                                   uint32_t* queue, uint32_t* queueCount, DeviceCounters* counters)
{
    __shared__ uint32_t sScratch[8];
    const uint32_t      total = fp.numSamples * fp.pixelsPadded;
    bool                keep[kItems];
    uint32_t            slots[kItems], pos[kItems], px[kItems], py[kItems], sample[kItems];
#pragma unroll
    for (int k = 0; k < kItems; ++k)
    {
        const uint32_t slot = (blockIdx.x * kItems + k) * kBlock + threadIdx.x;
        bool           valid = slot < total;
        uint32_t       x = 0, y = 0, sampleIdx = 0, lp = 0;
        if (valid) slotToSamplePixel(fp, slot, sampleIdx, lp);
        if (valid) valid = localPixelToXY(fp, tileIds, lp, x, y);
        keep[k] = valid;
        slots[k] = slot;
        px[k] = x, py[k] = y, sample[k] = sampleIdx;
    }
    if (fp.tileValidBefore != nullptr)
    {
#pragma unroll
        for (int k = 0; k < kItems; ++k)
        {
            if (!keep[k]) continue;
            uint32_t sampleIdx, lp;
            slotToSamplePixel(fp, slots[k], sampleIdx, lp);
            const uint32_t tile = tileIds[lp >> 10];
            uint32_t       tileX, tileY;
            fp.divTilesX.divmod(tile, tileY, tileX);
            const uint32_t x0 = tileX * kTileSize, y0 = tileY * kTileSize;
            const uint32_t rank = fp.tileValidBefore[lp >> 10] + validRankInTile(lp & 1023u, min(kTileSize, fp.width - x0), min(kTileSize, fp.height - y0));
            pos[k] = fp.slotGroupShift == kSlotSampleMajor ? sampleIdx * fp.validPixels + rank : rank * fp.numSamples + sampleIdx;
            queue[pos[k]] = slots[k];
        }
        if (blockIdx.x == 0 && threadIdx.x == 0) *queueCount = fp.validPixels * fp.numSamples;
    }
    else
        blockAppend<kItems>(keep, slots, queue, queueCount, sScratch, &pos);
#pragma unroll
    for (int k = 0; k < kItems; ++k)
    {
        if (!keep[k]) continue;
        const uint32_t x = px[k], y = py[k];
        const uint32_t frame = fp.firstFrame + (fp.samplePerm ? fp.samplePerm[sample[k]] : sample[k]);
        float          nx, ny;
        animatedBlueNoiseN(scene.blueNoise, x, y, frame - fp.divSamplesPerPixel.div(frame) * fp.samplesPerPixel, nx, ny);

        const float u = (static_cast<float>(x) + 0.5f) / static_cast<float>(fp.width);
        const float v = (static_cast<float>(y) + 0.5f) / static_cast<float>(fp.height);
        const float s = u + nx / static_cast<float>(fp.width);
        const float t = (1.0f - v) + ny / static_cast<float>(fp.height);

        const float phi = 2.0f * kPi * ny;
        const float cosPhi = tCos<F32>(phi), sinPhi = tSin<F32>(phi);
        const float r = rf_sqrt(nx);
        const float lensX = fp.camera.lensRadius * (r * cosPhi);
        const float lensY = fp.camera.lensRadius * (r * sinPhi);
        const Vec3  origin = fp.camera.origin + (lensX * fp.camera.right + lensY * fp.camera.up);
        const Vec3  dir = normalize(fp.camera.lowerLeftCorner + s * fp.camera.horizontal + t * fp.camera.vertical - origin);

        if (!fp.skipOrigins) store3(ps.rayO + pos[k], origin);
        store3(ps.rayD + pos[k], dir);
        store3(ps.noise + pos[k], vec3(nx, cosPhi, sinPhi));
    }
    (void)counters;
}

typedef float v4f __attribute__((ext_vector_type(4)));
__device__ __forceinline__ void storeAov(float4* aov, uint32_t slot, Vec3 albedo, float coverage, Vec3 normal, float depth)
{
    v4f* const p = reinterpret_cast<v4f*>(aov + 2 * static_cast<size_t>(slot));
    __builtin_nontemporal_store(v4f{albedo.x, albedo.y, albedo.z, coverage}, p);
    __builtin_nontemporal_store(v4f{normal.x, normal.y, normal.z, depth}, p + 1);
}

#if defined(RF_EXP_SHADE_WAVES)
#define RF_SHADE_BOUNDS __launch_bounds__(kBlock, RF_EXP_SHADE_WAVES)
#else
#define RF_SHADE_BOUNDS __launch_bounds__(kBlock)
#endif
template<bool SORTED, bool AOV>
__global__ RF_SHADE_BOUNDS void kShade(DeviceScene scene, SkyStateGpu sky, SunBasis sunBasis, PathStreams ps, const uint32_t* queue,
                                                  const uint32_t* queueCount, uint32_t* hitQueue, uint32_t* hitCount, uint32_t* missQueue, uint32_t* missSlots,
                                                  uint32_t* missCount, uint32_t* shadowList, uint32_t* shadowListCount, uint32_t bounceFlags, uint32_t sortScale, float4* aov)
{
    static_assert(kSortBins == kBlock, "one bin per thread");
    static_assert(!(SORTED && AOV), "the AOVs are written by the unsorted bounce-1 kernel");
    __shared__ uint32_t sScratch[8];
    __shared__ uint32_t sHist[SORTED ? kSortBins : 1], sStart[SORTED ? kSortBins : 1], sPerm[SORTED ? kItems * kBlock : 1];
    __shared__ float    sLut[256];
    constexpr uint32_t  kTile = kItems * kBlock;
    __shared__ float    sIn[SORTED ? 10 * kTile : 1];
    const uint32_t      count = *queueCount;
    const uint32_t tiles = (count + kItems * kBlock - 1) / (kItems * kBlock);
    if (blockIdx.x >= tiles) return;
    static_assert(kBlock == 256, "one table entry per thread");
    sLut[threadIdx.x] = scene.albedoLut[threadIdx.x];
    __syncthreads();
    const bool isLastBounce = (bounceFlags & kShadeLastBounce) != 0u, isFirstBounce = (bounceFlags & kShadeFirstBounce) != 0u;
    const bool selfShadow = (bounceFlags & kShadeSelfShadow) != 0u;
  for (uint32_t tile = blockIdx.x; tile < tiles; tile += gridDim.x)
  {
    bool       isHit[kItems], isMiss[kItems];
    uint32_t   slots[kItems], missEntries[kItems], missSlot[kItems], outPos[kItems], hitTri[kItems];
    Vec3       hitRecs[kItems];
#pragma unroll
    for (int k = 0; k < kItems; ++k)
    {
        const uint32_t i = (tile * kItems + k) * kBlock + threadIdx.x;
        const uint32_t iL = i < count ? i : 0u;
        slots[k] = queue[iL];
        hitRecs[k] = SORTED ? load3(ps.hit + iL) : vec3(ps.hit[iL].x, 0.0f, 0.0f);
    }
#pragma unroll
    for (int k = 0; k < kItems; ++k)
    {
        const uint32_t i = (tile * kItems + k) * kBlock + threadIdx.x;
        const bool     valid = i < count;
        const uint32_t tri = valid ? __float_as_uint(hitRecs[k].x) : kMiss;
        slots[k] = valid ? slots[k] : 0u;
        missSlot[k] = slots[k];
        missEntries[k] = valid ? i : 0u;
        hitTri[k] = tri;
        isMiss[k] = valid && tri == kMiss;
        isHit[k] = valid && tri != kMiss;
        if constexpr (AOV)
            if (isMiss[k]) storeAov(aov, slots[k], Vec3{}, 0.0f, Vec3{}, 0.0f);
    }
    if constexpr (SORTED)
    {
        Vec3 thrIn[kItems], noiseIn[kItems];
#pragma unroll
        for (int k = 0; k < kItems; ++k)
        {
            const uint32_t i = (tile * kItems + k) * kBlock + threadIdx.x;
            const uint32_t iL = isHit[k] ? i : 0u;
            thrIn[k] = isFirstBounce ? vec3(1.0f, 1.0f, 1.0f) : load3nt(ps.thr + iL);
            noiseIn[k] = load3nt(ps.noise + iL);
        }
#pragma unroll
        for (int k = 0; k < kItems; ++k)
        {
            if (!isHit[k]) continue;
            const uint32_t l = static_cast<uint32_t>(k) * kBlock + threadIdx.x;
            const Vec3     t = thrIn[k], z = noiseIn[k], hitRec = hitRecs[k];
            sIn[l] = t.x, sIn[kTile + l] = t.y, sIn[2 * kTile + l] = t.z;
            sIn[3 * kTile + l] = z.x, sIn[4 * kTile + l] = z.y, sIn[5 * kTile + l] = z.z;
            sIn[6 * kTile + l] = hitRec.x, sIn[7 * kTile + l] = hitRec.y, sIn[8 * kTile + l] = hitRec.z;
            sIn[9 * kTile + l] = __uint_as_float(slots[k]);
        }
    }
    uint32_t sortedHits = 0, sortedBase = 0;
    if constexpr (SORTED)
    {
        uint32_t bin[kItems], rank[kItems];
        sHist[threadIdx.x] = 0u;
        __syncthreads();
#pragma unroll
        for (int k = 0; k < kItems; ++k)
        {
            bin[k] = rank[k] = 0u;
            if (!isHit[k]) continue;
            bin[k] = min(__umulhi(hitTri[k], sortScale), kSortBins - 1u);
            rank[k] = atomicAdd(&sHist[bin[k]], 1u);
        }
        __syncthreads();
        {
            const uint32_t n = sHist[threadIdx.x], lane = __lane_id(), wave = threadIdx.x >> 6;
            uint32_t       incl = n;
            for (int off = 1; off < 64; off <<= 1)
            {
                const uint32_t up = __shfl_up(incl, off);
                if (static_cast<int>(lane) >= off) incl += up;
            }
            if (lane == 63) sScratch[wave] = incl;
            __syncthreads();
            uint32_t before = 0;
            for (uint32_t w = 0; w < wave; ++w) before += sScratch[w];
            sStart[threadIdx.x] = before + incl - n;
            if (threadIdx.x == 0)
            {
                const uint32_t total = sScratch[0] + sScratch[1] + sScratch[2] + sScratch[3];
                sScratch[5] = total;
                sScratch[4] = total ? atomicAdd(hitCount, total) : 0u;
            }
        }
        __syncthreads();
#pragma unroll
        for (int k = 0; k < kItems; ++k)
            if (isHit[k]) sPerm[sStart[bin[k]] + rank[k]] = static_cast<uint32_t>(k) * kBlock + threadIdx.x;
        __syncthreads();
        const uint32_t tileHits = sScratch[5], base = sScratch[4];
        sortedHits = tileHits, sortedBase = base;
#pragma unroll
        for (int k = 0; k < kItems; ++k)
        {
            const uint32_t p = static_cast<uint32_t>(k) * kBlock + threadIdx.x;
            isHit[k] = p < tileHits;
            outPos[k] = base + p;
            if (!isHit[k]) continue;
            const uint32_t local = sPerm[p];
            hitTri[k] = local;
            slots[k] = __float_as_uint(sIn[9 * kTile + local]);
            hitQueue[outPos[k]] = slots[k];
        }
        __syncthreads();
    }
    else
        blockAppend<kItems>(isHit, slots, hitQueue, hitCount, sScratch, &outPos);
    blockAppend<kItems>(isMiss, missEntries, missQueue, missCount, sScratch, nullptr, &missSlot, missSlots);

    constexpr bool kPipelined = SORTED;
    Vec3           hits[kPipelined ? kItems : 1];
    const auto     entryIndex = [&](int k) -> uint32_t {
        return SORTED ? (tile * kItems + hitTri[k] / kBlock) * kBlock + (hitTri[k] % kBlock) : (tile * kItems + static_cast<uint32_t>(k)) * kBlock + threadIdx.x;
    };
    if constexpr (kPipelined)
    {
#pragma unroll
        for (int k = 0; k < kItems; ++k) hits[k] = isHit[k] ? vec3(sIn[6 * kTile + hitTri[k]], sIn[7 * kTile + hitTri[k]], sIn[8 * kTile + hitTri[k]]) : Vec3{};
    }
    struct ShadeRecord
    {
        Vec3   p0, p1, p2;
        float4 a0, a1, a2, a3;
        Vec3   boxLo;
        float4 boxHi;
    };
    const auto fetchRecord = [&](uint32_t tri) {
        ShadeRecord   r;
        const float4* rec = scene.shadeRecords + 8 * static_cast<size_t>(tri);
#if defined(RF_EXP_SHADE_ABLATE) && RF_EXP_SHADE_ABLATE >= 3
        if constexpr (SORTED) rec = scene.shadeRecords + 8 * static_cast<size_t>(tri & 63u);
#endif
        if (selfShadow)
        {
            const float4 q0 = rec[0], q1 = rec[1], q2 = rec[2];
            r.p0 = vec3(q0.x, q0.y, q0.z), r.p1 = vec3(q1.x, q1.y, q1.z), r.p2 = vec3(q2.x, q2.y, q2.z);
            r.boxLo = vec3(q0.w, q1.w, q2.w);
            r.boxHi = rec[7];
        }
        else
        {
            r.p0 = load3(rec), r.p1 = load3(rec + 1), r.p2 = load3(rec + 2);
            r.boxLo = Vec3{}, r.boxHi = make_float4(0.0f, 0.0f, 0.0f, 0.0f);
        }
        r.a0 = rec[3], r.a1 = rec[4], r.a2 = rec[5], r.a3 = rec[6];
        return r;
    };
    const auto shade = [&](int k, float hu, float hv, float hitT, const ShadeRecord& cur, uint32_t out) -> bool {
        const uint32_t i = entryIndex(k);
        (void)i;
        Vec3 shadowOrigin;
        {
            const Vec3 p0 = cur.p0, p1 = cur.p1, p2 = cur.p2;
            const Vec3 e1 = p1 - p0, e2 = p2 - p0;
            const Vec3 hp = offsetRay(p0 + hu * e1 + hv * e2, normalize(cross(e1, e2)));
            store3nt(ps.rayO + out, hp);
            shadowOrigin = hp;
        }
        Vec3 throughput, nz;
        if constexpr (SORTED)
        {
            const uint32_t local = hitTri[k];
            throughput = vec3(sIn[local], sIn[kTile + local], sIn[2 * kTile + local]);
            nz = vec3(sIn[3 * kTile + local], sIn[4 * kTile + local], sIn[5 * kTile + local]);
        }
        else
        {
            throughput = isFirstBounce ? vec3(1.0f, 1.0f, 1.0f) : load3nt(ps.thr + i);
            nz = load3nt(ps.noise + i);
        }
        const float nx = nz.x, cosPhi = nz.y, sinPhi = nz.z;
        store3nt(ps.noiseOut + out, nz);
        const float4  a0 = cur.a0, a1 = cur.a1, a2 = cur.a2, a3 = cur.a3;
        const Vec3    n0 = vec3(a0.x, a0.y, a0.z), n1 = vec3(a0.w, a1.x, a1.y), n2 = vec3(a1.z, a1.w, a2.x);
        const float   b0 = 1.0f - hu - hv, b1 = hu, b2 = hv;
        const Vec3    n = (b0 * n0 + b1 * n1) + b2 * n2;
        const float   uvx = (b0 * a2.y + b1 * a2.w) + b2 * a3.y;
        const float   uvy = (b0 * a2.z + b1 * a3.x) + b2 * a3.z;
#if defined(RF_EXP_SHADE_ABLATE) && (RF_EXP_SHADE_ABLATE == 1 || RF_EXP_SHADE_ABLATE == 4)
        const Vec3    albedo = SORTED ? vec3(sLut[__float_as_uint(a3.w) & 255u], uvx - floorf(uvx), uvy - floorf(uvy)) : evalTexture(scene, sLut, __float_as_uint(a3.w), uvx, uvy);
#else
        const Vec3    albedo = evalTexture(scene, sLut, __float_as_uint(a3.w), uvx, uvy);
#endif
        if constexpr (AOV)
        {
            const float nn = dot(n, n);
            const Vec3  unitN = (nn != 0.0f && isfinite(nn)) ? normalize(n) : Vec3{};
            storeAov(aov, slots[k], albedo, 1.0f, unitN, hitT);
        }
        else (void)hitT, (void)aov;

        const Vec3 lightDirection = sunSample(sky, sunBasis, nx, cosPhi, sinPhi);
        const Vec3 lightIntensity = vec3(sky.solarRadiances[0], sky.solarRadiances[1], sky.solarRadiances[2]);
        const Vec3 brdf = albedo * kFrac1Pi;
        const Vec3 reflectance = brdf * dot(n, lightDirection);
        const Vec3 pend = (throughput * lightIntensity) * reflectance;
        bool       settled = false;
        if (selfShadow && cur.boxHi.w != 0.0f)
        {
            const RayPrep ray = prepareRay(shadowOrigin, lightDirection);
            if (classifyRay(ray) == kRayPlain)
            {
                const PackedRay pr = packRay(ray);
                float           bn, bf;
                bool            boxNaN;
                slabSingleBounds(pr, cur.boxLo.x, cur.boxLo.y, cur.boxLo.z, cur.boxHi.x, cur.boxHi.y, cur.boxHi.z, bn, bf, boxNaN);
                if (bn <= bf && bf > 0.0f && bn < kTMax)
                {
                    TriangleHit th;
                    settled = intersectTriangle(shadowOrigin, lightDirection, cur.p0, cur.p1, cur.p2, kTMax, th);
                }
            }
        }
        if (settled)
        {
            const Vec3 add = (pend * 0.0f) * __uint_as_float(kSolarInvPdfBits);
            const bool unchanged = !isFirstBounce && add.x == 0.0f && add.y == 0.0f && add.z == 0.0f;
            if (!unchanged)
            {
                const uint32_t slot = slots[k];
                const Vec3     radiance = (isFirstBounce ? vec3(0.0f, 0.0f, 0.0f) : load3(ps.rad + slot)) + add;
                ps.rad[slot] = make_float4(radiance.x, radiance.y, radiance.z, 0.0f);
            }
        }
        else store3nt(ps.pending + out, pend);

        if (!isLastBounce)
        {
            const float sinTheta = rf_sqrt(1.0f - nx);
            const Vec3  local = vec3(cosPhi * sinTheta, sinPhi * sinTheta, rf_sqrt(nx));
            Vec3        bu, bv;
            pixarOnb(n, bu, bv);
            const Vec3 wi = basisTimes(bu, bv, n, local);
            const Vec3 t2 = throughput * albedo;
            store3nt(ps.rayDOut + out, wi);
            store3nt(ps.thrOut + out, t2);
        }
        return !settled;
    };
    bool needShadow[kItems];
    if constexpr (kPipelined)
    {
        const uint32_t tileHits = sortedHits, base = sortedBase;
        ShadeRecord    cur{};
        if (threadIdx.x < tileHits) cur = fetchRecord(__float_as_uint(hits[0].x));
#pragma unroll
        for (int k = 0; k < kItems; ++k)
        {
            const uint32_t p = static_cast<uint32_t>(k) * kBlock + threadIdx.x, pNext = p + kBlock;
            ShadeRecord    next{};
            if (k + 1 < kItems && pNext < tileHits) next = fetchRecord(__float_as_uint(hits[k + 1 < kItems ? k + 1 : k].x));
            needShadow[k] = p < tileHits && shade(k, hits[k].y, hits[k].z, 0.0f, cur, base + p);
            cur = next;
        }
    }
    else
    {
#pragma unroll
        for (int k = 0; k < kItems; ++k) needShadow[k] = false;
#pragma unroll 1
        for (int k = 0; k < kItems; ++k)
        {
            if (!isHit[k]) continue;
            Vec3  h;
            float hitT = 0.0f;
            if constexpr (AOV)
            {
                const float4 rec = ps.hit[entryIndex(k)];
                h = vec3(rec.x, rec.y, rec.z), hitT = rec.w;
            }
            else h = load3(ps.hit + entryIndex(k));
            const bool need = shade(k, h.y, h.z, hitT, fetchRecord(__float_as_uint(h.x)), outPos[k]);
#pragma unroll
            for (int j = 0; j < kItems; ++j) needShadow[j] = j == k ? need : needShadow[j];
        }
    }
    if (selfShadow) blockAppend<kItems>(needShadow, outPos, shadowList, shadowListCount, sScratch);
    if constexpr (SORTED) __syncthreads();
  }
}

template<bool F32>
__global__ __launch_bounds__(kBlock) void kSky(SkyStateGpu sky, PathStreams ps, const uint32_t* missSlots, const uint32_t* missQueue, const uint32_t* missCount,
                                                uint32_t firstBounce)
{
    const uint32_t n = *missCount;
    const bool     first = firstBounce != 0u;
    for (uint32_t i = blockIdx.x * kBlock + threadIdx.x; i < n; i += gridDim.x * kBlock)
    {
        const uint32_t q = missQueue[i];
        const uint32_t slot = missSlots[i];
        const Vec3     v = load3(ps.rayD + q);
        const Vec3     thrIn = load3(ps.thr + q), radIn = load3(ps.rad + slot);
        const Vec3     thr = first ? vec3(1.0f, 1.0f, 1.0f) : thrIn;
        const Vec3     rad = first ? vec3(0.0f, 0.0f, 0.0f) : radIn;
        const Vec3     s = vec3(sky.sunDirection[0], sky.sunDirection[1], sky.sunDirection[2]);
        const float    theta = tAcos<F32>(v.y);
        const float    gamma = tAcos<F32>(minf(maxf(dot(v, s), -1.0f), 1.0f));
        const float cosGamma = tCos<F32>(gamma), cosTheta = fabsf(tCos<F32>(theta));
        const Vec3  dome = vec3(skyRadiance<F32>(sky, cosTheta, gamma, cosGamma, 0), skyRadiance<F32>(sky, cosTheta, gamma, cosGamma, 1), skyRadiance<F32>(sky, cosTheta, gamma, cosGamma, 2));
        const Vec3  radiance = rad + thr * dome;
        ps.rad[slot] = make_float4(radiance.x, radiance.y, radiance.z, 0.0f);
    }
}

__global__ void kBounceTotals(const uint32_t* queueCounts, uint32_t numBounces, unsigned long long* totals, const uint32_t* listCounts, unsigned long long lookMask, unsigned long long* lookBatch,
                              const uint32_t* shadowListCounts, unsigned long long selfMask, DeviceCounters* counters)
{
    const uint32_t b = threadIdx.x;
    if (b >= numBounces) return;
    const uint32_t k = min(b, RenderStats::kMaxBounceStats - 1);
    atomicAdd(&totals[k], static_cast<unsigned long long>(queueCounts[kLineWords * b]));
    atomicAdd(&totals[RenderStats::kMaxBounceStats + k], static_cast<unsigned long long>(queueCounts[kLineWords * (b + 1)]));
    const bool self = ((selfMask >> b) & 1ull) != 0ull;
    if (self)
    {
        const unsigned long long rays = queueCounts[kLineWords * (b + 1)];
        atomicAdd(&totals[3 * RenderStats::kMaxBounceStats + k], rays - shadowListCounts[kLineWords * b]);
        atomicAdd(&counters->shadowRays, rays);
    }
    if ((lookMask >> b) & 1ull)
    {
        const unsigned long long rays = self ? shadowListCounts[kLineWords * b] : queueCounts[kLineWords * (b + 1)], answered = rays - listCounts[kLineWords * b];
        atomicAdd(&totals[2 * RenderStats::kMaxBounceStats + k], answered);
        atomicAdd(&lookBatch[0], answered);
// ... 124 lines not shown
    out[i] = q[2] | (q[1] << 8) | (q[0] << 16) | (255u << 24);
}

__device__ __forceinline__ Vec3 offsetPositionDeferred(Vec3 p, Vec3 n)
{
    constexpr float kOrigin = 1.0f / 32.0f, kFloatScale = 1.0f / 16384.0f, kIntScale = 1024.0f;
    const int       ox = static_cast<int>(kIntScale * n.x), oy = static_cast<int>(kIntScale * n.y), oz = static_cast<int>(kIntScale * n.z);
    const Vec3      shifted = vec3(__int_as_float(__float_as_int(p.x) + (p.x < 0 ? -ox : ox)), __int_as_float(__float_as_int(p.y) + (p.y < 0 ? -oy : oy)),
                                   __int_as_float(__float_as_int(p.z) + (p.z < 0 ? -oz : oz)));
    return vec3(fabsf(p.x) < kOrigin ? p.x + kFloatScale * n.x : shifted.x, fabsf(p.y) < kOrigin ? p.y + kFloatScale * n.y : shifted.y,
                fabsf(p.z) < kOrigin ? p.z + kFloatScale * n.z : shifted.z);
}

struct DeferredSurface
{
    Vec3 plain, offset, normal, albedo;
};

__device__ __forceinline__ DeferredSurface deferredSurface(const DeviceScene& scene, const float* lut, const ClosestHit& h)
{
    DeferredSurface out;
    const Vec3 p0 = load3(scene.triangles + kTriStride * h.triangle), p1 = load3(scene.triangles + kTriStride * h.triangle + 1),
               p2 = load3(scene.triangles + kTriStride * h.triangle + 2);
    const Vec3 e1 = p1 - p0, e2 = p2 - p0;
    out.plain = p0 + h.u * e1 + h.v * e2;
    out.offset = offsetPositionDeferred(out.plain, normalize(cross(e1, e2)));
    const float4* va = scene.attributes + 4 * static_cast<size_t>(h.triangle);
    const float4  a0 = va[0], a1 = va[1], a2 = va[2], a3 = va[3];
    const Vec3    n0 = vec3(a0.x, a0.y, a0.z), n1 = vec3(a0.w, a1.x, a1.y), n2 = vec3(a1.z, a1.w, a2.x);
    const float   b0 = 1.0f - h.u - h.v, b1 = h.u, b2 = h.v;
    out.normal = (b0 * n0 + b1 * n1) + b2 * n2;
    const float uvx = (b0 * a2.y + b1 * a2.w) + b2 * a3.y, uvy = (b0 * a2.z + b1 * a3.x) + b2 * a3.z;
    out.albedo = evalTexture(scene, lut, __float_as_uint(a3.w), uvx, uvy);
    return out;
}

__device__ __forceinline__ Vec3 skyWithSun(const SkyStateGpu& sky, Vec3 v)
{
    const Vec3  s = vec3(sky.sunDirection[0], sky.sunDirection[1], sky.sunDirection[2]);
    const float theta = wAcos(v.y), gamma = wAcos(minf(maxf(dot(v, s), -1.0f), 1.0f));
    const float cosGamma = wCos(gamma), cosTheta = fabsf(wCos(theta));
    const bool  inDisk = gamma / __uint_as_float(0x3B91D640u) <= 1.0f;
    return vec3(skyRadiance(sky, cosTheta, gamma, cosGamma, 0) + (inDisk ? sky.solarRadiances[0] : 0.0f),
                skyRadiance(sky, cosTheta, gamma, cosGamma, 1) + (inDisk ? sky.solarRadiances[1] : 0.0f),
                skyRadiance(sky, cosTheta, gamma, cosGamma, 2) + (inDisk ? sky.solarRadiances[2] : 0.0f));
}

__global__ __launch_bounds__(kBlock) void kDeferredLighting(DeviceScene scene, SkyStateGpu sky, SunBasis sunBasis, Camera cam, uint32_t width, uint32_t height,
                                                             uint32_t frameCount, float jitterX, float jitterY, float exposure, float* sampleBuffer,
                                                             float* accumulationBuffer, uint32_t* bgraOut, DeviceCounters* counters)
{
    __shared__ uint32_t sStack[kLdsStack * kBlock];
    __shared__ float    sLut[256];
    sLut[threadIdx.x] = scene.albedoLut[threadIdx.x];
    __syncthreads();
    const uint32_t blocksX = (width + 7u) / 8u;
    const uint32_t wave = (blockIdx.x * kBlock + threadIdx.x) >> 6, lane = threadIdx.x & 63u;
    const uint32_t x = (wave % blocksX) * 8u + (lane & 7u), y = (wave / blocksX) * 8u + (lane >> 3);
    unsigned long long closest = 0, shadow = 0;
    if (x < width && y < height)
    {
    const float W = static_cast<float>(width), H = static_cast<float>(height);
    const float su = (static_cast<float>(x) + 0.5f) / W - (jitterX - 0.5f) / (2.0f * W);
    const float tv = (1.0f - (static_cast<float>(y) + 0.5f) / H) - (jitterY - 0.5f) / (2.0f * H);
    const Vec3  rd = normalize(cam.lowerLeftCorner + cam.horizontal * su + cam.vertical * tv - cam.origin);
    TraversalCounters  tc;
    ClosestHit         h;
    closest = 1;
    Vec3               color;
    const Vec3         lightIntensity = vec3(sky.solarRadiances[0], sky.solarRadiances[1], sky.solarRadiances[2]);
    if (!traverse<false, false>(scene, cam.origin, rd, kTMax, &sStack[threadIdx.x], h, tc)) color = skyWithSun(sky, rd);
    else
    {
        DeferredSurface sf = deferredSurface(scene, sLut, h);
        Vec3            normal = sf.normal, albedo = sf.albedo;
        Vec3            position = offsetPositionDeferred(sf.plain, normal);
        float           ux, uy;
        animatedBlueNoise(scene.blueNoise, x, y, frameCount, 1u << 20, ux, uy);
        const float phi = 2.0f * kPi * uy;
        const float cosPhi = wCos(phi), sinPhi = wSin(phi);
        const Vec3  light = sunSample(sky, sunBasis, ux, cosPhi, sinPhi);
        const auto  lightSample = [&](Vec3 pos, Vec3 n, Vec3 alb) {
            const Vec3 reflectance = (alb * kFrac1Pi) * dot(n, light);
            ClosestHit unused;
            ++shadow;
            const float vis = traverse<true, false>(scene, pos, light, kTMax, &sStack[threadIdx.x], unused, tc) ? 0.0f : 1.0f;
            return ((lightIntensity * reflectance) * vis) * __uint_as_float(kSolarInvPdfBits);
        };
        Vec3 radiance = vec3(0.0f, 0.0f, 0.0f), throughput = vec3(1.0f, 1.0f, 1.0f);
        radiance = radiance + throughput * lightSample(position, normal, albedo);
        for (int bounce = 1; bounce < 2; ++bounce)
        {
            const float sinTheta = rf_sqrt(1.0f - ux);
            Vec3        bu, bv;
            pixarOnb(normal, bu, bv);
            const Vec3 wi = basisTimes(bu, bv, normal, vec3(cosPhi * sinTheta, sinPhi * sinTheta, rf_sqrt(ux)));
            throughput = throughput * albedo;
            ++closest;
            if (traverse<false, false>(scene, position, wi, kTMax, &sStack[threadIdx.x], h, tc))
            {
                sf = deferredSurface(scene, sLut, h);
                position = sf.offset;
                normal = sf.normal;
                albedo = sf.albedo;
            }
            else
            {
                radiance = radiance + throughput * skyWithSun(sky, wi);
                break;
            }
            radiance = radiance + throughput * lightSample(position, normal, albedo);
        }
        color = radiance;
    }
    const size_t idx = static_cast<size_t>(y) * width + x;
    sampleBuffer[3 * idx] = color.x;
    sampleBuffer[3 * idx + 1] = color.y;
    sampleBuffer[3 * idx + 2] = color.z;
    Vec3 outc = color;
    if (frameCount != 0u)
    {
        const Vec3 prev = vec3(accumulationBuffer[3 * idx], accumulationBuffer[3 * idx + 1], accumulationBuffer[3 * idx + 2]);
        outc = 0.1f * color + 0.9f * prev;
    }
    accumulationBuffer[3 * idx] = outc.x;
    accumulationBuffer[3 * idx + 1] = outc.y;
    accumulationBuffer[3 * idx + 2] = outc.z;
    const float in[3] = {outc.x, outc.y, outc.z};
    uint32_t    q[3];
    for (int c = 0; c < 3; ++c)
    {
        const float xx = exposure * in[c];
        const float a = 2.51f, b = 0.03f, cc = 2.43f, d = 0.59f, e = 0.14f;
        float       yy = (xx * (a * xx + b)) / (xx * (cc * xx + d) + e);
        yy = minf(maxf(yy, 0.0f), 1.0f);
        q[c] = static_cast<uint32_t>(floorf(wPow(yy, 1.0f / 2.2f) * 255.0f + 0.5f));
    }
    bgraOut[idx] = q[2] | (q[1] << 8) | (q[0] << 16) | (255u << 24);
    if (tc.abandoned) atomicAdd(&counters->abandonedRays, 1ull);
    }
    const unsigned long long cr = waveSum(closest), sr = waveSum(shadow);
    if (__lane_id() == 0)
    {
        atomicAdd(&counters->closestRays, cr);
        atomicAdd(&counters->shadowRays, sr);
    }
}

}

namespace kern
{
SamplePermutationKernel samplePermutationKernel() { return kSamplePermutation; }
RaygenKernel            raygenKernel(bool f32) { return f32 ? kRaygen<true> : kRaygen<false>; }
ShadeKernel             shadeKernel(bool sorted, bool aov) { return aov ? kShade<false, true> : sorted ? kShade<true, false> : kShade<false, false>; }
SkyKernel               skyKernel(bool f32) { return f32 ? kSky<true> : kSky<false>; }
BounceTotalsKernel      bounceTotalsKernel() { return kBounceTotals; }
AccumulateKernel        accumulateKernel() { return kAccumulate; }
AccumulateRunsKernel    accumulateRunsKernel(uint32_t pixels) { return pixels == 1u ? kAccumulateRuns<1> : pixels == 2u ? kAccumulateRuns<2> : kAccumulateRuns<kAccPixels>; }
AccumulateAovKernel     accumulateAovKernel(bool runs) { return runs ? kAccumulateAovRuns : kAccumulateAov; }
TonemapKernel           tonemapKernel() { return kTonemap; }
DeferredLightingKernel  deferredLightingKernel() { return kDeferredLighting; }
}
}
```

rayfinder_amd/csrc/rf_trace.hip:

```cpp
#include "rf_kernels.hpp"

namespace rf
{
namespace
{
template<bool COUNT>
__global__ __launch_bounds__(kBlock) void kTraceClosest(DeviceScene scene, PathStreams ps, const uint32_t* queue,
                                                         const uint32_t* queueCount, DeviceCounters* counters)
{
    __shared__ uint32_t sStack[kLdsStack * kBlock];
    const uint32_t      i = blockIdx.x * kBlock + threadIdx.x;
    const uint32_t      count = *queueCount;
    if (blockIdx.x * kBlock >= count) return;
    TraversalCounters tc;
    if (i < count)
    {
        const Vec3 o = load3(ps.rayO + i);
        const Vec3 d = load3(ps.rayD + i);
        ClosestHit h;
        traverse<false, COUNT>(scene, o, d, kTMax, &sStack[threadIdx.x], h, tc);
        if (tc.abandoned) atomicAdd(&counters->abandonedRays, 1ull);
        ps.hit[i] = make_float4(__uint_as_float(h.triangle), h.u, h.v, h.t);
    }
    if (COUNT)
    {
        const unsigned long long nv = waveSum(tc.nodesVisited), tt = waveSum(tc.triangleTests);
        const uint32_t           sh = waveMax(tc.stackHigh);
        if (__lane_id() == 0)
        {
            atomicAdd(&counters->closestNodeVisits, nv);
            atomicAdd(&counters->closestTriangleTests, tt);
            atomicMax(&counters->stackHigh, sh);
        }
    }
    if (i == 0) atomicAdd(&counters->closestRays, static_cast<unsigned long long>(count));
}

template<bool COUNT>
__global__ __launch_bounds__(kBlock) void kTraceShadow(DeviceScene scene, SkyStateGpu sky, SunBasis sunBasis, PathStreams ps, const uint32_t* queue,
                                                        const uint32_t* queueCount, DeviceCounters* counters, uint32_t firstBounce)
{
    __shared__ uint32_t sStack[kLdsStack * kBlock];
    const uint32_t      i = blockIdx.x * kBlock + threadIdx.x;
    const uint32_t      count = *queueCount;
    if (blockIdx.x * kBlock >= count) return;
    TraversalCounters tc;
    if (i < count)
    {
        const uint32_t slot = queue[i];
        const Vec3     o = load3(ps.rayO + i);
        const Vec3     nz = load3(ps.noiseOut + i);
        const Vec3     l = sunSample(sky, sunBasis, nz.x, nz.y, nz.z);
        ClosestHit     h;
        const bool     occluded = traverse<true, COUNT>(scene, o, l, kTMax, &sStack[threadIdx.x], h, tc);
        if (tc.abandoned) atomicAdd(&counters->abandonedRays, 1ull);
        const float    visibility = occluded ? 0.0f : 1.0f;
        const Vec3     pend = load3(ps.pending + i);
        const Vec3     rad0 = firstBounce ? vec3(0.0f, 0.0f, 0.0f) : load3(ps.rad + slot);
        const Vec3 add = (pend * visibility) * __uint_as_float(kSolarInvPdfBits);
        const Vec3 radiance = rad0 + add;
        ps.rad[slot] = make_float4(radiance.x, radiance.y, radiance.z, 0.0f);
    }
    if (COUNT)
    {
        const unsigned long long nv = waveSum(tc.nodesVisited), tt = waveSum(tc.triangleTests);
        if (__lane_id() == 0)
        {
            atomicAdd(&counters->shadowNodeVisits, nv);
            atomicAdd(&counters->shadowTriangleTests, tt);
        }
    }
    if (i == 0) atomicAdd(&counters->shadowRays, static_cast<unsigned long long>(count));
}

__device__ __forceinline__ uint32_t occluderCellIndex(const WideScene& wide, float ox, float oy, float oz)
{
    const uint32_t cx = static_cast<uint32_t>(__float2int_rd((ox - wide.rootLo.x) * wide.occScale)), cy = static_cast<uint32_t>(__float2int_rd((oy - wide.rootLo.y) * wide.occScale)),
                   cz = static_cast<uint32_t>(__float2int_rd((oz - wide.rootLo.z) * wide.occScale));
    return ((cx * 73856093u) ^ (cy * 19349663u) ^ (cz * 83492791u)) & wide.occMask;
}
__device__ __forceinline__ void loadOccluderCell(const uint32_t* cell, uint32_t (&e)[kOccSlots])
{
    if constexpr (kOccSlots == 1) e[0] = *cell;
    else if constexpr (kOccSlots == 2)
    {
        const uint2 v = *reinterpret_cast<const uint2*>(cell);
        e[0] = v.x, e[1] = v.y;
    }
    else
    {
        const uint4 v = *reinterpret_cast<const uint4*>(cell);
        e[0] = v.x, e[1] = v.y, e[kOccSlots > 2 ? 2 : 0] = v.z, e[kOccSlots > 3 ? 3 : 0] = v.w;
    }
}
__device__ __forceinline__ void storeOccluderCell(uint32_t* cell, const uint32_t (&e)[kOccSlots])
{
    if constexpr (kOccSlots == 1) *cell = e[0];
    else if constexpr (kOccSlots == 2) *reinterpret_cast<uint2*>(cell) = make_uint2(e[0], e[1]);
    else *reinterpret_cast<uint4*>(cell) = make_uint4(e[0], e[1], e[kOccSlots > 2 ? 2 : 0], e[kOccSlots > 3 ? 3 : 0]);
}

template<bool COUNT, bool NEAREST_FIRST>
constexpr int wideStackDepth()
{
    return (COUNT && !NEAREST_FIRST) ? 28 : kWideLdsStack;
}

#if defined(RF_EXP_ANYHIT_WAVES)
constexpr int kWideWavesAnyHit = RF_EXP_ANYHIT_WAVES;
#else
constexpr int kWideWavesAnyHit = kWideWaves;
#endif
template<bool ANY_HIT, bool COUNT, bool NEAREST_FIRST = false, int COMPACT = 0, bool DENSE_LEAVES = false>
__global__ __launch_bounds__(kBlock, (COUNT && !NEAREST_FIRST) ? 2 : ((ANY_HIT && !COUNT) ? kWideWavesAnyHit : kWideWaves)) void kTraceWide(DeviceScene scene, WideScene wide, SkyStateGpu sky, SunBasis sunBasis, PathStreams ps,
                                                                                        const uint32_t* queue, const uint32_t* queueCount, uint32_t* cursor,
                                                                                        DeviceCounters* counters, uint32_t refillMin, uint32_t leafVote,
                                                                                        uint32_t chunkMax, float tMax, uint32_t flags)
{
    constexpr int  kDepth = wideStackDepth<COUNT, NEAREST_FIRST>();
    constexpr bool kRefCount = COUNT && !NEAREST_FIRST;
    static_assert(!(COMPACT != 0 && COUNT), "the compact-record and quad-record variants have no counting build");
    static_assert(COMPACT >= 0 && COMPACT <= 6, "0: 64-byte records, 1: compact-capable, 2: 32-byte, 3: quad, 4: half-precision quad, 5: local-grid quad, 6: local-grid oct (closest-hit)");
    static_assert(!(COMPACT == 6 && ANY_HIT), "the oct records serve the closest-hit launches (the any-hit launches start at occluder-cache entries that name quad records)");
#if !defined(RF_EXP_LEGACY_LAYOUTS)
    static_assert(COMPACT != 1 && COMPACT != 2, "the compact-capable and the 32-byte records are experiment-build layouts (make EXP=RF_EXP_LEGACY_LAYOUTS)");
#endif
    constexpr bool kConservative = COMPACT == 4 || COMPACT == 5 || COMPACT == 6;
    using StackEntry = std::conditional_t<ANY_HIT && !kRefCount, uint32_t, uint2>;
    __shared__ StackEntry sStack[kDepth * kBlock];
    const uint32_t   count = *queueCount;
    const uint32_t   lane = __lane_id();
    const bool       shadowDirFromStream = flags & kFlagShadowDirFromStream;
    const bool       firstBounce = flags & kFlagFirstBounce;
    const bool       uniformFetch = flags & kFlagUniformFetch, uniformTri = flags & kFlagUniformTri;
    constexpr bool kOccluderCache = ANY_HIT && !COUNT && (COMPACT == 3 || COMPACT == 4 || COMPACT == 5);
    const bool     leafBoxAtLeaf = kConservative || (COMPACT == 3 && kOccluderCache && (flags & kFlagOccluderCache) != 0u && wide.occGrid != nullptr);
    const bool     occluderCache = kOccluderCache && (flags & kFlagOccluderCache) != 0u && wide.occGrid != nullptr;
    const auto occluderCell = [&](float ox, float oy, float oz) -> uint32_t { return occluderCellIndex(wide, ox, oy, oz); };
    constexpr uint32_t kNegTriedHint = 16u;

    uint32_t chunk = chunkMax;
    while (chunk > 64u && static_cast<unsigned long long>(chunk) * 8ull * gridDim.x * (kBlock / 64) > count) chunk >>= 1;
    const uint32_t shardLen = ((count + kShards - 1) / kShards + chunk - 1) / chunk * chunk;
    uint32_t       shard = blockIdx.x % kShards, shardsTried = 0;
    uint32_t       chunkPos = 0, chunkEnd = 0;
    bool           exhausted = count == 0;

    uint32_t  node = kNodeIdle;
    uint32_t  slot = 0;
    uint32_t  resultIndex = 0;
    Vec3      pendingTerm{};
    float tOuterLo = 0.0f, tOuterHi = 0.0f;
    bool  haveOuter = false;
    BoxT  own{};
    float hbx = 0.0f, hby = 0.0f, hbz = 0.0f;
    uint32_t lselX = 0u, lselY = 0u, lselZ = 0u;
    uint32_t octKey = 0u;
    uint32_t hrot = 0u, hrotY = 0u, hrotZ = 0u;
    PackedRay pr{};
    Vec3      rayDir{};
    uint32_t  negMask = 0;
    float     rayTMax = tMax;
    constexpr bool     kEagerLeaves = !ANY_HIT && !COUNT && !DENSE_LEAVES;
#if defined(RF_EXP_LEAF_REPEAT)
    constexpr uint32_t kLeafRepeat = RF_EXP_LEAF_REPEAT;
#else
    constexpr uint32_t kLeafRepeat = 8u;
#endif
    constexpr bool kPtrStack = !COUNT && !ANY_HIT;
    const int     spBase = kPtrStack ? static_cast<int>(threadIdx.x * sizeof(uint2)) : 0;
    constexpr int kSpStep = kPtrStack ? static_cast<int>(kBlock * sizeof(uint2)) : 1;
    constexpr int kSpLimit = kPtrStack ? kDepth * static_cast<int>(kBlock * sizeof(uint2)) : kDepth;
    int       stackSize = spBase;
    const auto stackAt = [&](int s) -> StackEntry& {
        if constexpr (kPtrStack) return *reinterpret_cast<StackEntry*>(reinterpret_cast<char*>(sStack) + s);
        else return sStack[s * kBlock + threadIdx.x];
    };
    bool      needScalar = false;
    constexpr bool kStackWordsOnly = ANY_HIT && !kRefCount;
    static_assert(std::is_same_v<StackEntry, uint32_t> == kStackWordsOnly, "the LDS stack's entry type follows kStackWordsOnly");
    constexpr bool kSpill = !kRefCount;
    constexpr int  kEvict = kDepth >= 9 ? 6 : (kDepth > 4 ? kDepth - 3 : 1), kSpillBlocks = 36 / kEvict;
    static_assert(kEvict >= 3 && kEvict <= kDepth - 2, "a quad step checks the bound once (depth < kDepth - 2) and then pushes up to three entries: an eviction must make room for all three");
    using SpillEntry = std::conditional_t<kStackWordsOnly, uint32_t, uint2>;
    SpillEntry spillBuf[kSpill ? kEvict * kSpillBlocks : 1];
    const auto slotS = [&](int i) -> int { return kPtrStack ? spBase + i * kSpStep : i; };
    const auto evict = [&]() -> bool {
        if constexpr (!kSpill) return false;
        const uint32_t spilled = negMask >> 8;
        if (spilled + kEvict > static_cast<uint32_t>(kEvict * kSpillBlocks)) return false;
        for (int i = 0; i < kEvict; ++i)
        {
            if constexpr (kStackWordsOnly) spillBuf[spilled + i] = stackAt(slotS(i));
            else spillBuf[spilled + i] = stackAt(slotS(i));
        }
        const int depth = kPtrStack ? (stackSize - spBase) / kSpStep : stackSize;
        for (int i = kEvict; i < depth; ++i)
        {
            if constexpr (kStackWordsOnly) stackAt(slotS(i - kEvict)) = stackAt(slotS(i));
            else stackAt(slotS(i - kEvict)) = stackAt(slotS(i));
        }
        stackSize -= kEvict * kSpStep;
        negMask += static_cast<uint32_t>(kEvict) << 8;
        return true;
    };
    const auto unspill = [&]() {
        negMask -= static_cast<uint32_t>(kEvict) << 8;
        const uint32_t spilled = negMask >> 8;
        for (int i = 0; i < kEvict; ++i)
        {
            if constexpr (kStackWordsOnly) stackAt(slotS(i)) = spillBuf[spilled + i];
            else stackAt(slotS(i)) = spillBuf[spilled + i];
        }
        stackSize = slotS(kEvict);
    };
    auto      push = [&](uint32_t word, float tmin) -> bool {
        if (stackSize >= kSpLimit && !evict()) return false;
        if constexpr (kStackWordsOnly) stackAt(stackSize) = word;
        else stackAt(stackSize) = make_uint2(word, __float_as_uint(tmin));
        stackSize += kSpStep;
        return true;
    };
    auto      pushUnchecked = [&](uint32_t word, float tmin) {
        if constexpr (kStackWordsOnly) stackAt(stackSize) = word;
        else stackAt(stackSize) = make_uint2(word, __float_as_uint(tmin));
        stackSize += kSpStep;
    };
    ClosestHit        best{};
    bool              occluded = false;
    TraversalCounters tc;
    uint32_t          rayNodes = 0, rayTris = 0, rayStackHigh = 0;
    uint32_t          recordFetches = 0;
    uint32_t          wDescend = 0, wLeaf = 0, wLeafPhase = 0, wRefill = 0, wPop = 0, wOuter = 0;
#if defined(RF_EXP_PHASE)
    constexpr bool kPhase = true;
    uint32_t       phaseTris = 0, phaseLeafWave = 0, phaseOccTried = 0, phaseOccHit = 0, phaseOccluded = 0;
    uint32_t       phaseParked = 0, phaseIdle = 0, phaseLeafInterior = 0, phaseLeafIdle = 0;
    bool           phaseFromCache = false;
#else
    constexpr bool kPhase = COUNT;
#endif

    auto popNext = [&]() {
        if (COMPACT != 0) haveOuter = false;
        node = kNodeDone;
        if constexpr (kStackWordsOnly)
        {
            if (stackSize > spBase)
            {
                stackSize -= kSpStep;
                node = stackAt(stackSize);
                if (COUNT) ++wPop;
            }
            return;
        }
        else
        {
            while (stackSize > spBase)
            {
                stackSize -= kSpStep;
                uint2 e = stackAt(stackSize);
                asm volatile("" : "+v"(e.x), "+v"(e.y));
                if (COUNT) ++wPop;
                if (kRefCount) ++rayNodes;
                if (__uint_as_float(e.y) < rayTMax)
                {
                    node = e.x;
                    break;
                }
            }
        }
    };

    for (;;)
    {
        if (kPhase) ++wOuter;
        const unsigned long long idleMask = __ballot(node == kNodeIdle);
        const uint32_t           idleCount = __popcll(idleMask);
        if (!exhausted && idleCount >= refillMin)
        {
            if (kPhase) ++wRefill;
            const uint32_t rankInIdle = __popcll(idleMask & ((1ull << lane) - 1ull));
            uint32_t       assigned = 0, myPos = 0xFFFFFFFFu;
            while (assigned < idleCount)
            {
                while (chunkPos == chunkEnd && !exhausted)
                {
                    const uint32_t shardBegin = shard * shardLen, shardEnd = min(shardBegin + shardLen, count);
                    uint32_t       base = 0;
                    if (lane == 0) base = shardBegin < count ? atomicAdd(cursor + shard * kLineWords, chunk) : shardLen;
                    base = shardBegin + static_cast<uint32_t>(__builtin_amdgcn_readfirstlane(static_cast<int>(base)));
                    if (base >= shardEnd)
                    {
                        shard = (shard + 1) % kShards;
                        if (++shardsTried == kShards) exhausted = true;
                    }
                    else
                    {
                        chunkPos = base;
                        chunkEnd = min(base + chunk, shardEnd);
                    }
                }
                if (chunkPos == chunkEnd) break;
                const uint32_t take = min(idleCount - assigned, chunkEnd - chunkPos);
                if (rankInIdle - assigned < take) myPos = chunkPos + (rankInIdle - assigned);
                chunkPos += take;
                assigned += take;
            }
            if (node == kNodeIdle && myPos != 0xFFFFFFFFu)
            {
                resultIndex = myPos;
                if (!ANY_HIT && wide.rayList != nullptr) resultIndex = wide.rayList[myPos];
                bool triedCell = false;
                if constexpr (kOccluderCache)
                {
                    if (wide.rayList != nullptr)
                    {
                        const uint32_t e = wide.rayList[myPos];
                        resultIndex = e & 0x7FFFFFFFu;
                        triedCell = (e >> 31) != 0u;
                    }
                }
                if (ANY_HIT) slot = loadQ(queue + resultIndex);
                if (ANY_HIT) pendingTerm = load3s(ps.pending + resultIndex);
                Vec3 dir{};
                if (!(ANY_HIT && !shadowDirFromStream)) dir = load3s(ps.rayD + resultIndex);
                const Vec3 o = (!ANY_HIT && (flags & kFlagConstOrigin) != 0u) ? vec3(wide.constOriginX, wide.constOriginY, wide.constOriginZ) : load3s(ps.rayO + resultIndex);
                if (ANY_HIT && !shadowDirFromStream)
                {
                    const Vec3 nz = load3s(ps.noiseOut + resultIndex);
                    dir = sunSample(sky, sunBasis, nz.x, nz.y, nz.z);
                }
                const RayPrep ray = prepareRay(o, dir);
                pr = packRay(ray);
                rayDir = dir;
                rayTMax = tMax;
                stackSize = spBase;
#if defined(RF_EXP_PHASE)
                phaseFromCache = false;
#endif
                best.triangle = kMiss;
                occluded = false;
                if (COMPACT == 1) haveOuter = false;
                if (COMPACT == 2)
                {
                    own = boxPlaneT(pr, make_float4(wide.rootLo.x, wide.rootLo.y, wide.rootHi.x, wide.rootHi.y), wide.rootLo.z, wide.rootHi.z);
                    haveOuter = true;
                }
                rayNodes = 1;
                rayTris = 0;
                rayStackHigh = 0;
                bool fastRay = false;
                if constexpr (kConservative && !COUNT)
                {
                    const float ax = fabsf(ray.invDir.x), ay = fabsf(ray.invDir.y), az = fabsf(ray.invDir.z);
                    fastRay = ax >= 1e-18f && ax <= 1e18f && ay >= 1e-18f && ay <= 1e18f && az >= 1e-18f && az <= 1e18f && fabsf(o.x) <= wide.originBound && fabsf(o.y) <= wide.originBound &&
                              fabsf(o.z) <= wide.originBound && wide.originBound < 1e30f;
                }
                uint32_t rayClass = kRayPlain;
                bool     rootOk = true;
                needScalar = false;
                if (__builtin_expect(!fastRay, 0))
                {
                    rayClass = classifyRay(ray);
                    needScalar = rayClass == kRayIrregular;
                    if constexpr (kConservative)
                    {
                        const auto ordinary = [](float inv) { const float a = fabsf(inv); return (a >= 1e-18f && a <= 1e18f) || a == __uint_as_float(0x7F800000u); };
                        const bool inside = fabsf(o.x) <= wide.originBound && fabsf(o.y) <= wide.originBound && fabsf(o.z) <= wide.originBound;
                        if (!(inside && ordinary(ray.invDir.x) && ordinary(ray.invDir.y) && ordinary(ray.invDir.z))) needScalar = true;
                        const float inf = __uint_as_float(0x7F800000u);
                        if (fabsf(pr.iXY.x) == inf) pr.iXY.x = __builtin_copysignf(1e30f, pr.iXY.x);
                        if (fabsf(pr.iXY.y) == inf) pr.iXY.y = __builtin_copysignf(1e30f, pr.iXY.y);
                        if (fabsf(pr.iZ) == inf) pr.iZ = __builtin_copysignf(1e30f, pr.iZ);
                    }
                    if (!(kConservative && !COUNT) || rayClass != kRayPlain)
                    {
                        float rootTMin;
                        rootOk = slabBounds(ray, wide.rootLo, wide.rootHi, rootTMin) && rootTMin < rayTMax;
                    }
                }
                negMask = ray.negX | (ray.negY << 1) | (ray.negZ << 2) | (rayClass == kRayHasInf ? 8u : 0u) | (triedCell ? 16u : 0u);
                if constexpr (kConservative)
                {
                    hbx = -(o.x * pr.iXY.x);
                    hby = -(o.y * pr.iXY.y);
                    hbz = -(o.z * pr.iZ);
                    hrot = ray.negX << 4, hrotY = ray.negY << 4, hrotZ = ray.negZ << 4;
                    lselX = ray.negX ? 0x00040005u : 0x00050004u, lselY = ray.negY ? 0x00040005u : 0x00050004u, lselZ = ray.negZ ? 0x00040005u : 0x00050004u;
                    const uint32_t signXY = ray.negX | (ray.negY << 1);
                    octKey = ray.negZ ? ((16u * (3u - signXY)) | (0x7777u << 8)) : 16u * signXY;
                }
                node = (needScalar || !rootOk) ? kNodeDone : (wide.rootLeaf != kWideNone ? wide.rootLeaf : 0u);
                if constexpr (kOccluderCache)
                {
                    uint32_t hint = 0u;
                    uint32_t later[kOccSlots > 1 ? kOccSlots - 1 : 1] = {};
                    if (occluderCache && (flags & kFlagOccluderNoTry) == 0u)
                    {
                        uint32_t e[kOccSlots];
                        loadOccluderCell(wide.occGrid + kOccSlots * static_cast<size_t>(occluderCell(o.x, o.y, o.z)), e);
                        if (e[0] != 0u)
                        {
                            hint = e[0];
#pragma unroll
                            for (int k = 1; k < kOccSlots; ++k) later[k - 1] = e[k];
                        }
                    }
                    if (occluderCache && hint != 0u && node == 0u)
                    {
                        push(0u, 0.0f);
#pragma unroll
                        for (int k = kOccSlots - 1; k >= 1; --k)
                            if (later[k - 1] != 0u) push(later[k - 1], 0.0f);
                        node = hint;
                        negMask |= kNegTriedHint;
#if defined(RF_EXP_PHASE)
                        ++phaseOccTried, phaseFromCache = true;
#endif
                    }
                }
            }
        }
        if (__ballot(node != kNodeIdle) == 0ull)
        {
            if (exhausted) break;
            continue;
        }

        if (!kEagerLeaves || !(__popcll(__ballot(static_cast<int32_t>(node) >= 0)) < leafVote &&
                               __popcll(__ballot(node - kWideLeafBit < kNodeDone - kWideLeafBit)) >= kLeafRepeat))
        do
        {
            if (kPhase) ++wDescend;
#if defined(RF_EXP_PHASE)
            if (node >= kNodeDone) ++phaseIdle;
            else if (static_cast<int32_t>(node) < 0) ++phaseParked;
#endif
            if (static_cast<int32_t>(node) >= 0)
            {
                if (kPhase) ++recordFetches;
                if constexpr (COMPACT == 6)
                {
                    const uint4* n = wide.oct + 8 * static_cast<size_t>(node);
                    const uint4  v0 = n[0], v1 = n[1], vx = n[2], vy = n[3], vz = n[4], wa = n[5], wb = n[6];
                    const float  ax = __uint_as_float(v0.w) * pr.iXY.x, ay = __uint_as_float(v1.x) * pr.iXY.y, az = __uint_as_float(v1.y) * pr.iZ;
                    const float  bx = __builtin_fmaf(-1024.0f, ax, (__uint_as_float(v0.x) - pr.oXY.x) * pr.iXY.x), by = __builtin_fmaf(-1024.0f, ay, (__uint_as_float(v0.y) - pr.oXY.y) * pr.iXY.y),
                                bz = __builtin_fmaf(-1024.0f, az, (__uint_as_float(v0.z) - pr.oZ) * pr.iZ);
                    float tq[8], fq[8];
                    localEntryBounds<0>(vx.x, vy.x, vz.x, lselX, lselY, lselZ, ax, ay, az, bx, by, bz, tq[0], fq[0]);
                    localEntryBounds<1>(vx.x, vy.x, vz.x, lselX, lselY, lselZ, ax, ay, az, bx, by, bz, tq[1], fq[1]);
                    localEntryBounds<0>(vx.y, vy.y, vz.y, lselX, lselY, lselZ, ax, ay, az, bx, by, bz, tq[2], fq[2]);
                    localEntryBounds<1>(vx.y, vy.y, vz.y, lselX, lselY, lselZ, ax, ay, az, bx, by, bz, tq[3], fq[3]);
                    localEntryBounds<0>(vx.z, vy.z, vz.z, lselX, lselY, lselZ, ax, ay, az, bx, by, bz, tq[4], fq[4]);
                    localEntryBounds<1>(vx.z, vy.z, vz.z, lselX, lselY, lselZ, ax, ay, az, bx, by, bz, tq[5], fq[5]);
                    localEntryBounds<0>(vx.w, vy.w, vz.w, lselX, lselY, lselZ, ax, ay, az, bx, by, bz, tq[6], fq[6]);
                    localEntryBounds<1>(vx.w, vy.w, vz.w, lselX, lselY, lselZ, ax, ay, az, bx, by, bz, tq[7], fq[7]);
                    const uint32_t words[8] = {wa.x, wa.y, wa.z, wa.w, wb.x, wb.y, wb.z, wb.w};
                    const unsigned long long table = (static_cast<unsigned long long>(v1.w) << 32) | v1.z;
                    const uint32_t           ord = static_cast<uint32_t>(table >> (octKey & 63u)) ^ (octKey >> 8);
                    const float tiny = __uint_as_float(1u), predTMax = __uint_as_float(__float_as_uint(rayTMax) - 1u);
                    uint32_t    pos[8], miss = 0u;
#pragma unroll
                    for (int j = 0; j < 4; ++j)
                    {
                        pos[2 * j] = (ord >> (4 * j)) & 7u;
                        pos[2 * j + 1] = pos[2 * j] ^ 1u;
                    }
                    float gap[8];
#pragma unroll
                    for (int e = 0; e < 8; ++e)
                    {
                        gap[e] = isaMin(fq[e], predTMax) - isaMax(tq[e], tiny);
                        miss |= (__float_as_uint(gap[e]) >> 31) << pos[e];
                    }
                    const uint32_t hits = ~miss & 0xFFu;
                    if (hits != 0u)
                    {
                        const int need = __popc(hits);
                        bool      room = true;
                        if constexpr (kPtrStack)
                        {
                            while (room && stackSize + need * kSpStep > kSpLimit + spBase) room = (stackSize - spBase) >= kEvict * kSpStep && evict();
// ... 677 lines not shown
        if (kSpill && node == kNodeDone && !needScalar && !occluded)
        {
            while (node == kNodeDone && (negMask >> 8) != 0u)
            {
                unspill();
                popNext();
            }
        }
        if (node == kNodeDone)
        {
            if (needScalar)
            {
                TraversalCounters c2;
                atomicAdd(&counters->scalarRedo[ANY_HIT ? 1 : 0], 1ull);
                best.triangle = kMiss;
                occluded = traverse<ANY_HIT, COUNT, 0>(scene, vec3(pr.oXY.x, pr.oXY.y, pr.oZ), rayDir, tMax, nullptr, best, c2);
                if (c2.abandoned) atomicAdd(&counters->abandonedRays, 1ull);
                rayTMax = best.triangle != kMiss ? best.t : tMax;
                rayNodes = c2.nodesVisited;
                rayTris = c2.triangleTests;
                rayStackHigh = c2.stackHigh;
            }
            if (COUNT)
            {
                tc.nodesVisited += rayNodes;
                tc.triangleTests += rayTris;
                tc.stackHigh = max(tc.stackHigh, rayStackHigh);
            }
            if constexpr (kOccluderCache)
            {
                if (occluderCache && (occluderWord != 0u || (!occluded && (negMask & kNegTriedHint) != 0u)))
                {
                    uint32_t* const cell = wide.occGrid + kOccSlots * static_cast<size_t>(occluderCell(pr.oXY.x, pr.oXY.y, pr.oZ));
                    uint32_t        old[kOccSlots], now[kOccSlots];
                    loadOccluderCell(cell, old);
                    if (occluderWord == 0u)
                    {
#pragma unroll
                        for (int k = 0; k < kOccSlots; ++k) now[k] = k + 1 < kOccSlots ? old[k + 1 < kOccSlots ? k + 1 : k] : 0u;
                        storeOccluderCell(cell, now);
                    }
                    else if (occluderWord != old[0])
                    {
                        int at = kOccSlots - 1;
#pragma unroll
                        for (int k = kOccSlots - 2; k >= 1; --k)
                            if (old[k] == occluderWord) at = k;
                        now[0] = occluderWord;
#pragma unroll
                        for (int k = 1; k < kOccSlots; ++k) now[k] = k <= at ? old[k - 1] : old[k];
                        storeOccluderCell(cell, now);
                    }
                }
            }
            if (ANY_HIT)
            {
                const float visibility = occluded ? 0.0f : 1.0f;
                const Vec3  add = (pendingTerm * visibility) * __uint_as_float(kSolarInvPdfBits);
                const bool unchanged = !firstBounce && add.x == 0.0f && add.y == 0.0f && add.z == 0.0f;
                if (!unchanged)
                {
                    const Vec3 radiance = (firstBounce ? vec3(0.0f, 0.0f, 0.0f) : load3s(ps.rad + slot)) + add;
                    store4s(ps.rad + slot, radiance.x, radiance.y, radiance.z, 0.0f);
                }
            }
            else
            {
                store4s(ps.hit + resultIndex, __uint_as_float(best.triangle), best.u, best.v, rayTMax);
            }
            node = kNodeIdle;
        }
    }

    if (COUNT)
    {
        const unsigned long long nv = waveSum(tc.nodesVisited), tt = waveSum(tc.triangleTests);
        const uint32_t           sh = waveMax(tc.stackHigh);
        if (lane == 0)
        {
            atomicAdd(ANY_HIT ? &counters->shadowNodeVisits : &counters->closestNodeVisits, nv);
            atomicAdd(ANY_HIT ? &counters->shadowTriangleTests : &counters->closestTriangleTests, tt);
            if (!ANY_HIT) atomicMax(&counters->stackHigh, sh);
        }
        const unsigned long long rf = waveSum(recordFetches);
        if (lane == 0) atomicAdd(ANY_HIT ? &counters->shadowRecordFetches : &counters->closestRecordFetches, rf);
        const int                k = ANY_HIT ? 1 : 0;
        const unsigned long long pops = waveSum(wPop);
        const uint32_t           d = waveMax(wDescend), l = waveMax(wLeaf), lp = waveMax(wLeafPhase), r = waveMax(wRefill), o = waveMax(wOuter);
        if (lane == 0)
        {
            atomicAdd(&counters->descendTrips[k], static_cast<unsigned long long>(d));
            atomicAdd(&counters->leafTrips[k], static_cast<unsigned long long>(l));
            atomicAdd(&counters->leafPhases[k], static_cast<unsigned long long>(lp));
            atomicAdd(&counters->refillTrips[k], static_cast<unsigned long long>(r));
            atomicAdd(&counters->popLaneTrips[k], pops);
            atomicAdd(&counters->outerTrips[k], static_cast<unsigned long long>(o));
        }
    }
#if defined(RF_EXP_PHASE)
    if (!COUNT)
    {
        const int                k = ANY_HIT ? 1 : 0;
        const unsigned long long laneSteps = waveSum(recordFetches), laneLeaves = waveSum(wLeafPhase), laneTris = waveSum(phaseTris);
        const uint32_t           d = waveMax(wDescend), lp = waveMax(phaseLeafWave), r = waveMax(wRefill), o = waveMax(wOuter);
        if (lane == 0)
        {
            atomicAdd(ANY_HIT ? &counters->shadowRecordFetches : &counters->closestRecordFetches, laneSteps);
            atomicAdd(&counters->descendTrips[k], static_cast<unsigned long long>(d));
            atomicAdd(&counters->leafPhases[k], static_cast<unsigned long long>(lp));
            atomicAdd(&counters->leafTrips[k], laneLeaves);
            atomicAdd(&counters->popLaneTrips[k], laneTris);
            atomicAdd(&counters->refillTrips[k], static_cast<unsigned long long>(r));
            atomicAdd(&counters->outerTrips[k], static_cast<unsigned long long>(o));
        }
        const unsigned long long pk = waveSum(phaseParked), pi = waveSum(phaseIdle), li = waveSum(phaseLeafInterior), ld = waveSum(phaseLeafIdle);
        if (lane == 0) atomicAdd(&counters->descendParked[k], pk), atomicAdd(&counters->descendIdle[k], pi), atomicAdd(&counters->leafInterior[k], li), atomicAdd(&counters->leafIdle[k], ld);
        const unsigned long long ot = waveSum(phaseOccTried), oh = waveSum(phaseOccHit), oc = waveSum(phaseOccluded);
        if (lane == 0 && ANY_HIT) atomicAdd(&counters->occluderTried, ot), atomicAdd(&counters->occluderHit, oh), atomicAdd(&counters->occludedRays, oc);
    }
#endif
    if (blockIdx.x == 0 && threadIdx.x == 0 && !(flags & kFlagNoRayCount)) atomicAdd(ANY_HIT ? &counters->shadowRays : &counters->closestRays, static_cast<unsigned long long>(count));
}


__global__ __launch_bounds__(kBlock) void kShadowFirstLook(DeviceScene scene, WideScene wide, SkyStateGpu sky, SunBasis sunBasis, PathStreams ps, const uint32_t* queue,
                                                            const uint32_t* inList, const uint32_t* inCount, uint32_t* list, uint32_t* listCount, DeviceCounters* counters, float tMax,
                                                            uint32_t flags)
{
    __shared__ uint32_t sScratch[8];
    const uint32_t      count = *inCount;
    const uint32_t      firstBounce = flags & kLookFirstBounce;
    const uint32_t      tiles = (count + kItems * kBlock - 1) / (kItems * kBlock);
    if (blockIdx.x == 0 && threadIdx.x == 0 && !(flags & kLookNoRayCount)) atomicAdd(&counters->shadowRays, static_cast<unsigned long long>(count));
    for (uint32_t tile = blockIdx.x; tile < tiles; tile += gridDim.x)
    {
        bool     keep[kItems];
        uint32_t entry[kItems];
#pragma unroll
        for (int k = 0; k < kItems; ++k)
        {
            const uint32_t j = (tile * kItems + k) * kBlock + threadIdx.x;
            keep[k] = j < count;
            entry[k] = j;
            if (j >= count) continue;
            const uint32_t i = inList != nullptr ? inList[j] : j;
            entry[k] = i;
            v3fu           o3 = *reinterpret_cast<const v3fu*>(ps.rayO + i);
            asm volatile("" : "+v"(o3));
            const Vec3     o = vec3(o3.x, o3.y, o3.z);
            uint32_t* const cell = wide.occGrid + kOccSlots * static_cast<size_t>(occluderCellIndex(wide, o.x, o.y, o.z));
            uint32_t        e[kOccSlots];
            loadOccluderCell(cell, e);
            if (e[0] == 0u) continue;
            const Vec3    nz = load3(ps.noiseOut + i);
            const Vec3    dir = sunSample(sky, sunBasis, nz.x, nz.y, nz.z);
            const RayPrep ray = prepareRay(o, dir);
            if (classifyRay(ray) != kRayPlain) continue;
            entry[k] = i | 0x80000000u;
            const PackedRay pr = packRay(ray);
            int             at = -1;
#pragma unroll
            for (int j = 0; j < kOccSlots; ++j)
            {
                const uint32_t w = e[j];
                if (at >= 0 || (w & kWideLeafBit) == 0u || ((w >> kWideIndexBits) & 7u) == 7u) continue;
                const uint32_t first = w & ((1u << kWideIndexBits) - 1u), n = ((w >> kWideIndexBits) & 7u) + 1u;
                const float4*  t0 = scene.triangles + kTriStride * static_cast<size_t>(first);
                typedef float v4f __attribute__((ext_vector_type(4)));
                const v4f*     t4 = reinterpret_cast<const v4f*>(t0);
                v4f            a = t4[0], b = t4[1], c = t4[2];
                v3f            hi = *reinterpret_cast<const v3f*>(t0 + 3);
                asm volatile("" : "+v"(a), "+v"(b), "+v"(c), "+v"(hi));
                float          bn, bf;
                bool           boxNaN;
                slabSingleBounds(pr, a.w, b.w, c.w, hi.x, hi.y, hi.z, bn, bf, boxNaN);
                if (!(bn <= bf && bf > 0.0f && bn < tMax)) continue;
                TriangleHit th;
                bool        stopped = intersectTriangle(o, dir, vec3(a.x, a.y, a.z), vec3(b.x, b.y, b.z), vec3(c.x, c.y, c.z), tMax, th);
                for (uint32_t t = 1; t < n && !stopped; ++t)
                {
                    const v3f q0 = *reinterpret_cast<const v3f*>(t0 + kTriStride * t), q1 = *reinterpret_cast<const v3f*>(t0 + kTriStride * t + 1),
                              q2 = *reinterpret_cast<const v3f*>(t0 + kTriStride * t + 2);
                    stopped = intersectTriangle(o, dir, vec3(q0.x, q0.y, q0.z), vec3(q1.x, q1.y, q1.z), vec3(q2.x, q2.y, q2.z), tMax, th);
                }
                if (stopped) at = j;
            }
            if (at < 0) continue;
            keep[k] = false;
            if (at > 0)
            {
                uint32_t now[kOccSlots];
                now[0] = e[at];
#pragma unroll
                for (int j = 1; j < kOccSlots; ++j) now[j] = j <= at ? e[j - 1] : e[j];
                storeOccluderCell(cell, now);
            }
            const Vec3 add = (load3(ps.pending + i) * 0.0f) * __uint_as_float(kSolarInvPdfBits);
            const bool unchanged = firstBounce == 0u && add.x == 0.0f && add.y == 0.0f && add.z == 0.0f;
            if (!unchanged)
            {
                const uint32_t slot = queue[i];
                const Vec3     radiance = (firstBounce != 0u ? vec3(0.0f, 0.0f, 0.0f) : load3(ps.rad + slot)) + add;
                ps.rad[slot] = make_float4(radiance.x, radiance.y, radiance.z, 0.0f);
            }
        }
        blockAppend<kItems>(keep, entry, list, listCount, sScratch);
    }
}


#if defined(RF_EXP_LEGACY_LAYOUTS)
constexpr int kPacketDepth = 24;

template<bool ANY_HIT>
__global__ __launch_bounds__(kBlock, 6) void kTracePacket(DeviceScene scene, WideScene wide, SkyStateGpu sky, SunBasis sunBasis, PathStreams ps,
                                                          const uint32_t* queue, const uint32_t* queueCount, DeviceCounters* counters, float tMax, uint32_t flags)
{
    __shared__ float    sTMin[kPacketDepth * kBlock];
    const uint32_t      count = *queueCount;
    const uint32_t      lane = __lane_id(), wave = threadIdx.x >> 6;
    const bool          shadowDirFromStream = flags & kFlagShadowDirFromStream;
    const bool          firstBounce = flags & kFlagFirstBounce;
    const float         kInf = __uint_as_float(0x7F800000u);
    float* const        myTMin = sTMin + threadIdx.x;
    const uint32_t      numChunks = (count + 63u) / 64u;
    const uint32_t      totalWaves = gridDim.x * (kBlock / 64);

    for (uint32_t chunkIdx = blockIdx.x * (kBlock / 64) + wave; chunkIdx < numChunks; chunkIdx += totalWaves)
    {
        const uint32_t idx = chunkIdx * 64u + lane;
        const bool     valid = idx < count;
        uint32_t       slot = 0;
        Vec3           o = vec3(0.0f, 0.0f, 0.0f), dir = vec3(0.0f, 0.0f, 1.0f);
        if (valid)
        {
            if (ANY_HIT) slot = loadQ(queue + idx);
            o = load3s(ps.rayO + idx);
            if (ANY_HIT && !shadowDirFromStream)
            {
                const Vec3 nz = load3s(ps.noiseOut + idx);
                dir = sunSample(sky, sunBasis, nz.x, nz.y, nz.z);
            }
            else dir = load3s(ps.rayD + idx);
        }
        const RayPrep   ray = prepareRay(o, dir);
        const PackedRay pr = packRay(ray);
        const uint32_t  rayClass = classifyRay(ray);
        const uint32_t  negMask = ray.negX | (ray.negY << 1) | (ray.negZ << 2);
        bool            needScalar = valid && rayClass != kRayPlain;
        const bool      regular = valid && rayClass == kRayPlain;
        float           rootTMin;
        const bool      rootOk = slabBounds(ray, wide.rootLo, wide.rootHi, rootTMin);
        ClosestHit      best{};
        best.triangle = kMiss;
        float resultT = tMax;
        bool  occluded = false;

        unsigned long long todo = __ballot(regular);
        while (todo != 0ull)
        {
            bool member = regular;
            if (!ANY_HIT)
            {
                const uint32_t leader = static_cast<uint32_t>(__ffsll(static_cast<long long>(todo))) - 1u;
                const uint32_t uNeg = __builtin_amdgcn_readlane(negMask, leader);
                member = regular && ((todo >> lane) & 1ull) != 0ull && negMask == uNeg;
            }
            const unsigned long long memberMask = __ballot(member);
            todo &= ~memberMask;
            const uint32_t passNeg = __builtin_amdgcn_readfirstlane(__builtin_amdgcn_readlane(negMask, static_cast<uint32_t>(__ffsll(static_cast<long long>(memberMask))) - 1u));

            float limit = member ? tMax : -kInf;
            bool  active = rootOk && rootTMin < limit;
            if (__ballot(active) == 0ull) continue;
            uint32_t node = wide.rootLeaf != kWideNone ? wide.rootLeaf : 0u;
            int      depth = 0;
            bool     overflow = false;
            uint32_t wordStack = 0;
            for (;;)
            {
                node = __builtin_amdgcn_readfirstlane(node);
                bool popNow = false;
                if (static_cast<int32_t>(node) >= 0)
                {
                    typedef uint32_t u8v __attribute__((ext_vector_type(8)));
                    typedef uint32_t u4v __attribute__((ext_vector_type(4)));
                    typedef uint32_t u2v __attribute__((ext_vector_type(2)));
                    const float4* un = wide.nodes + 4 * static_cast<size_t>(node);
                    u8v           a;
                    u4v           b;
                    u2v           c;
                    asm volatile("s_load_dwordx8 %0, %3, 0x0\n\ts_load_dwordx4 %1, %3, 0x20\n\ts_load_dwordx2 %2, %3, 0x30\n\ts_waitcnt lgkmcnt(0)"
                                 : "=&s"(a), "=&s"(b), "=&s"(c)
                                 : "s"(un)
                                 : "memory");
                    const float4   q0 = make_float4(__uint_as_float(a.s0), __uint_as_float(a.s1), __uint_as_float(a.s2), __uint_as_float(a.s3));
                    const float4   q1 = make_float4(__uint_as_float(a.s4), __uint_as_float(a.s5), __uint_as_float(a.s6), __uint_as_float(a.s7));
                    const float4   q2 = make_float4(__uint_as_float(b.x), __uint_as_float(b.y), __uint_as_float(b.z), __uint_as_float(b.w));
                    const uint32_t axis = (c.x >> kWideAxisShift) & 3u;
                    const uint32_t word0 = c.x & ~(3u << kWideAxisShift), word1 = c.y;
                    float          t0, t1;
                    bool           ok0, ok1;
                    slabPair(pr, q0, q1, q2, ok0, t0, ok1, t1);
                    const bool hit0 = active && ok0 && t0 < limit, hit1 = active && ok1 && t1 < limit;
                    const unsigned long long m0 = __ballot(hit0), m1 = __ballot(hit1);
                    bool secondFirst;
                    if (ANY_HIT) secondFirst = 2 * __popcll(__ballot(hit0 && hit1 && t1 < t0)) > __popcll(m0 & m1);
                    else secondFirst = ((passNeg >> axis) & 1u) != 0u;
                    const unsigned long long mN = secondFirst ? m1 : m0, mF = secondFirst ? m0 : m1;
                    const uint32_t           nearWord = secondFirst ? word1 : word0, farWord = secondFirst ? word0 : word1;
                    const bool               hitN = secondFirst ? hit1 : hit0, hitF = secondFirst ? hit0 : hit1;
                    const float              tF = secondFirst ? t0 : t1;
                    if (mN != 0ull)
                    {
                        if (mF != 0ull)
                        {
                            if (depth >= kPacketDepth)
                            {
                                overflow = true;
                                break;
                            }
                            myTMin[depth * kBlock] = hitF ? tF : kInf;
                            {
                                uint32_t keepM0;
                                asm volatile("s_mov_b32 %1, m0\n\ts_mov_b32 m0, %3\n\ts_nop 0\n\tv_writelane_b32 %0, %2, m0\n\ts_mov_b32 m0, %1"
                                             : "+v"(wordStack), "=&s"(keepM0)
                                             : "s"(farWord), "s"(depth));
                            }
                            ++depth;
                        }
                        node = nearWord;
                        active = hitN;
                    }
                    else if (mF != 0ull)
                    {
                        node = farWord;
                        active = hitF;
                    }
                    else popNow = true;
                }
                else
                {
                    uint32_t first = node & ((1u << kWideIndexBits) - 1u), n = ((node >> kWideIndexBits) & 7u) + 1u;
                    if (n == 8u)
                    {
                        const uint2 big = wide.bigLeaves[first];
                        first = __builtin_amdgcn_readfirstlane(big.x);
                        n = __builtin_amdgcn_readfirstlane(big.y);
                    }
                    for (uint32_t i = 0; i < n; ++i)
                    {
                        typedef uint32_t u8v __attribute__((ext_vector_type(8)));
                        typedef uint32_t u4v __attribute__((ext_vector_type(4)));
                        const uint32_t tri = first + i;
                        const float4*  ut = scene.triangles + kTriStride * static_cast<size_t>(tri);
                        u8v            ab;
                        u4v            cc;
                        asm volatile("s_load_dwordx8 %0, %2, 0x0\n\ts_load_dwordx4 %1, %2, 0x20\n\ts_waitcnt lgkmcnt(0)" : "=&s"(ab), "=&s"(cc) : "s"(ut) : "memory");
                        const Vec3 p0 = vec3(__uint_as_float(ab.s0), __uint_as_float(ab.s1), __uint_as_float(ab.s2));
                        const Vec3 p1 = vec3(__uint_as_float(ab.s4), __uint_as_float(ab.s5), __uint_as_float(ab.s6));
                        const Vec3 p2 = vec3(__uint_as_float(cc.x), __uint_as_float(cc.y), __uint_as_float(cc.z));
                        TriangleHit th;
                        if (active && intersectTriangle(o, dir, p0, p1, p2, limit, th))
                        {
                            if (ANY_HIT)
                            {
                                occluded = true;
                                limit = -kInf;
                                active = false;
                            }
                            else
                            {
                                limit = th.t;
                                best.u = th.u;
                                best.v = th.v;
                                best.triangle = tri;
                            }
                        }
                    }
                    if (ANY_HIT && __ballot(member && !occluded) == 0ull) break;
                    popNow = true;
                }
                if (popNow)
                {
                    bool found = false;
                    while (depth > 0)
                    {
                        --depth;
                        const float tm = myTMin[depth * kBlock];
                        active = tm < limit;
                        if (__ballot(active) != 0ull)
                        {
                            node = __builtin_amdgcn_readlane(wordStack, static_cast<uint32_t>(depth));
// ... 160 lines not shown
```

Before: 12940.

## Compress per-path noise stream to 32-bit keys with precomputed lookup tables

Measured after the change: 12840. About the same (-0.8%).

```diff
diff --git a/rayfinder_amd/csrc/rf_device.hpp b/rayfinder_amd/csrc/rf_device.hpp
--- a/rayfinder_amd/csrc/rf_device.hpp
+++ b/rayfinder_amd/csrc/rf_device.hpp
@@ -24,6 +24,9 @@
     uint64_t                 numTexels;
     const uint8_t*           blueNoise;
     const float*             albedoLut;
+    const float*             noiseNx;
+    const float2*            noiseTrig;
+    uint32_t                 noiseSamples;
 };
 
 #if defined(__HIPCC__)
@@ -376,15 +379,34 @@
     return vec3(lut[(bgra >> 16) & 0xffu], lut[(bgra >> 8) & 0xffu], lut[bgra & 0xffu]);
 }
 
+__device__ __forceinline__ float blueNoiseX(uint32_t byteX, uint32_t n)
+{
+    const float bx = static_cast<float>(byteX) / 255.0f;
+    const float a1 = 0.7548776662466927f;
+    return wFract(bx + wFract(a1 * static_cast<float>(n)));
+}
+__device__ __forceinline__ float blueNoiseY(uint32_t byteY, uint32_t n)
+{
+    const float by = static_cast<float>(byteY) / 255.0f;
+    const float a2 = 0.5698402909980532f;
+    return wFract(by + wFract(a2 * static_cast<float>(n)));
+}
+__device__ __forceinline__ uint32_t blueNoiseBytes(const uint8_t* table, uint32_t x, uint32_t y)
+{
+    const uint32_t idx = (y % 128u) * 128u + (x % 128u);
+    return static_cast<uint32_t>(table[2 * idx]) | (static_cast<uint32_t>(table[2 * idx + 1]) << 8);
+}
 __device__ __forceinline__ void animatedBlueNoiseN(const uint8_t* table, uint32_t x, uint32_t y, uint32_t n, float& nx, float& ny)
 {
-    const uint32_t idx = (y % 128u) * 128u + (x % 128u);
-    const float    bx = static_cast<float>(table[2 * idx]) / 255.0f;
-    const float    by = static_cast<float>(table[2 * idx + 1]) / 255.0f;
-    const float    a1 = 0.7548776662466927f;
-    const float    a2 = 0.5698402909980532f;
-    nx = wFract(bx + wFract(a1 * static_cast<float>(n)));
-    ny = wFract(by + wFract(a2 * static_cast<float>(n)));
+    const uint32_t bytes = blueNoiseBytes(table, x, y);
+    nx = blueNoiseX(bytes & 255u, n);
+    ny = blueNoiseY(bytes >> 8, n);
+}
+template<bool F32>
+__device__ __forceinline__ void blueNoiseTrig(float ny, float& cosPhi, float& sinPhi)
+{
+    const float phi = 2.0f * kPi * ny;
+    cosPhi = tCos<F32>(phi), sinPhi = tSin<F32>(phi);
 }
 __device__ __forceinline__ void animatedBlueNoise(const uint8_t* table, uint32_t x, uint32_t y, uint32_t frameIdx, uint32_t totalSampleCount, float& nx, float& ny)
 {
diff --git a/rayfinder_amd/csrc/rf_kernels.hpp b/rayfinder_amd/csrc/rf_kernels.hpp
--- a/rayfinder_amd/csrc/rf_kernels.hpp
+++ b/rayfinder_amd/csrc/rf_kernels.hpp
@@ -39,10 +39,10 @@
     float4* rad;
     float4* hit;
     P3*     pending;
-    P3*     noise;
+    uint32_t* noise;
     P3*     rayDOut;
     P3*     thrOut;
-    P3*     noiseOut;
+    uint32_t* noiseOut;
 };
 
 typedef float v3f __attribute__((ext_vector_type(3)));
@@ -73,6 +73,16 @@
 {
     const v3fu v = __builtin_nontemporal_load(reinterpret_cast<const v3fu*>(p));
     return vec3(v.x, v.y, v.z);
+}
+
+constexpr uint32_t kMaxBatchSamples = 8192;
+__device__ __forceinline__ uint32_t noiseKey(uint32_t rank, uint32_t tableBytes) { return (rank << 16) | tableBytes; }
+__device__ __forceinline__ Vec3 expandNoiseKey(const DeviceScene& scene, uint32_t key)
+{
+    const uint32_t rank = key >> 16;
+    const float    nx = scene.noiseNx[(key & 255u) * scene.noiseSamples + rank];
+    const float2   cs = scene.noiseTrig[((key >> 8) & 255u) * scene.noiseSamples + rank];
+    return vec3(nx, cs.x, cs.y);
 }
 
 __device__ __forceinline__ Vec3     load3s(const float4* p) { return load3(p); }
@@ -326,6 +336,7 @@
 
 
 using SamplePermutationKernel = void (*)(uint32_t firstFrame, uint32_t spp, uint32_t numSamples, uint32_t* perm, uint32_t* inv);
+using NoiseTablesKernel = void (*)(uint32_t firstFrame, FastDiv divSpp, uint32_t numSamples, const uint32_t* samplePerm, float* noiseNx, float2* noiseTrig);
 using RaygenKernel = void (*)(FrameParams fp, DeviceScene scene, const uint32_t* tileIds, PathStreams ps, uint32_t* queue, uint32_t* queueCount, DeviceCounters* counters);
 using TraceClosestKernel = void (*)(DeviceScene scene, PathStreams ps, const uint32_t* queue, const uint32_t* queueCount, DeviceCounters* counters);
 using ShadeKernel = void (*)(DeviceScene scene, SkyStateGpu sky, SunBasis sunBasis, PathStreams ps, const uint32_t* queue, const uint32_t* queueCount, uint32_t* hitQueue, uint32_t* hitCount, uint32_t* missQueue, uint32_t* missSlots, uint32_t* missCount, uint32_t* shadowList, uint32_t* shadowListCount, uint32_t bounceFlags, uint32_t sortScale, float4* aov);
@@ -355,7 +366,8 @@
 IntersectRaysKernel   intersectRaysKernel();
 OccludedRaysKernel    occludedRaysKernel();
 SamplePermutationKernel samplePermutationKernel();
-RaygenKernel            raygenKernel(bool f32Transcendentals);
+NoiseTablesKernel       noiseTablesKernel(bool f32Transcendentals);
+RaygenKernel            raygenKernel();
 ShadeKernel             shadeKernel(bool sorted, bool aov = false);
 SkyKernel               skyKernel(bool f32Transcendentals);
 BounceTotalsKernel      bounceTotalsKernel();
diff --git a/rayfinder_amd/csrc/rf_renderer.hip b/rayfinder_amd/csrc/rf_renderer.hip
--- a/rayfinder_amd/csrc/rf_renderer.hip
+++ b/rayfinder_amd/csrc/rf_renderer.hip
@@ -174,6 +174,10 @@
     unsigned long long      primaryRaysHost = 0;
     uint64_t                maxPaths = 0;
     DeviceBuffer<P3>        sRayO, sRayD, sRayD2, sThr, sThr2, sPending, sNoise, sNoise2;
+    static uint32_t*        noiseKeys(const DeviceBuffer<P3>& b) { return reinterpret_cast<uint32_t*>(b.ptr); }
+    PathStreams             pathStreams() const { return PathStreams{sRayO.ptr, sRayD.ptr, sThr.ptr, sRad.ptr, sHit.ptr, sPending.ptr, noiseKeys(sNoise), sRayD2.ptr, sThr2.ptr, noiseKeys(sNoise2)}; }
+    DeviceBuffer<float>     noiseNx;
+    DeviceBuffer<float2>    noiseTrig;
     DeviceBuffer<float4>    sRad, sHit;
     DeviceBuffer<float4>    sAov;
     DeviceBuffer<uint32_t>  queueA, queueB, missQueue, missSlots, shadowList, queueCounts;
@@ -604,15 +608,16 @@
         uint32_t numTiles;
         uint64_t validPixels;
     };
-    BatchPlan planBatch(uint32_t numSamples, const ActiveTiles* active) const
+    BatchPlan planBatch(uint32_t samplesWanted, const ActiveTiles* active) const
     {
         BatchPlan b{};
         const uint64_t validPixels = active ? active->validPixels : this->validPixels;
+        const uint32_t numSamples = std::min(samplesWanted, kMaxBatchSamples);
         b.numSamples = numSamples;
         b.numBounces = params.samplingParams.numBounces;
         b.numTiles = active ? active->numTiles : static_cast<uint32_t>(tiles.size());
         b.pixelsPadded = b.numTiles * 1024u;
-        b.samplePerm = optSampleSort && numSamples > 1 && numSamples <= 8192 && optSlotGroupShift != kSlotSampleMajor;
+        b.samplePerm = optSampleSort && numSamples > 1 && optSlotGroupShift != kSlotSampleMajor;
         const auto finite3 = [](Vec3 v) { return std::isfinite(v.x) && std::isfinite(v.y) && std::isfinite(v.z); };
         const Camera& camNow = params.camera;
         b.primaryLayout = closestLayoutFor(1);
@@ -700,7 +705,7 @@
         RF_HIP(hipMemsetAsync(queueCounts.ptr, 0, queueCounts.count * sizeof(uint32_t), stream));
         const uint32_t count = static_cast<uint32_t>(n);
         RF_HIP(hipMemcpyAsync(queueCounts.ptr, &count, sizeof count, hipMemcpyHostToDevice, stream));
-        PathStreams ps{sRayO.ptr, sRayD.ptr, sThr.ptr, sRad.ptr, sHit.ptr, sPending.ptr, sNoise.ptr, sRayD2.ptr, sThr2.ptr, sNoise2.ptr};
+        PathStreams ps = pathStreams();
         const dim3  grid(std::min<uint32_t>(static_cast<uint32_t>((n + kBlock - 1) / kBlock), wideBlocks));
         const WideArgs wa{ps, queueA.ptr, queueCounts.ptr + qc.queueWord(0), queueCounts.ptr + qc.cursorClosestWord(1), tMax, grid};
         if (shadow)
@@ -773,7 +778,7 @@
         uint64_t       depth = maxPaths;
         for (;;)
         {
-            const uint32_t perBatch = static_cast<uint32_t>(std::max<uint64_t>(1, depth / pixelsPadded));
+            const uint32_t perBatch = static_cast<uint32_t>(std::min<uint64_t>(std::max<uint64_t>(1, depth / pixelsPadded), kMaxBatchSamples));
             const uint32_t numBatches = (todo + perBatch - 1) / perBatch;
             n = (todo + numBatches - 1) / numBatches;
             const uint64_t need = static_cast<uint64_t>(n) * pixelsPadded;
@@ -921,6 +926,7 @@
     {
         const uint64_t validPixels = active ? active->validPixels : this->validPixels;
         BatchPlan      batch = planBatch(numSamples, active);
+        if (batch.numSamples != numSamples) throw std::logic_error("traceBatch: a batch deeper than kMaxBatchSamples");
         FrameParams    fp{};
         fp.width = params.width;
         fp.height = params.height;
@@ -941,6 +947,13 @@
         }
         fp.tilesX = grid().tilesX;
         if (fp.numTiles == 0) return;
+        const uint64_t tableEntries = 256ull * numSamples;
+        if (noiseNx.count < tableEntries)
+        {
+            RF_HIP(hipStreamSynchronize(stream));
+            noiseNx.alloc(tableEntries), noiseTrig.alloc(tableEntries);
+        }
+        scene.noiseNx = noiseNx.ptr, scene.noiseTrig = noiseTrig.ptr, scene.noiseSamples = numSamples;
         fp.divNumSamples = FastDiv::make(fp.numSamples), fp.divPixelsPadded = FastDiv::make(fp.pixelsPadded), fp.divTilesX = FastDiv::make(fp.tilesX);
         fp.divSamplesPerPixel = FastDiv::make(fp.samplesPerPixel);
         fp.skipOrigins = batch.constOrigin ? 1u : 0u;
@@ -951,7 +964,7 @@
         const uint64_t paths = static_cast<uint64_t>(numSamples) * fp.pixelsPadded;
         const uint32_t blocks = static_cast<uint32_t>((paths + kBlock - 1) / kBlock);
         primaryRaysHost += static_cast<unsigned long long>(numSamples) * validPixels;
-        PathStreams    ps{sRayO.ptr, sRayD.ptr, sThr.ptr, sRad.ptr, sHit.ptr, sPending.ptr, sNoise.ptr, sRayD2.ptr, sThr2.ptr, sNoise2.ptr};
+        PathStreams    ps = pathStreams();
         const uint32_t numBounces = fp.numBounces;
 
         wide.occGrid = nullptr;
@@ -997,7 +1010,9 @@
             hipLaunchKernelGGL(samplePermutationKernel(), dim3((numSamples + 255) / 256), dim3(256), 0, stream, firstFrame, fp.samplesPerPixel, numSamples,
                                const_cast<uint32_t*>(fp.samplePerm), const_cast<uint32_t*>(fp.sampleInvPerm));
         launchTimed(0, [&] {
-            hipLaunchKernelGGL(raygenKernel(optTranscendentalsF32), dim3(itemBlocks), dim3(kBlock), 0, stream, fp, scene, tileIds.ptr, io.ps, io.in, words.queueCount(0), counters.ptr);
+            hipLaunchKernelGGL(noiseTablesKernel(optTranscendentalsF32), dim3((numSamples + kBlock - 1) / kBlock, 256), dim3(kBlock), 0, stream, firstFrame, fp.divSamplesPerPixel,
+                               numSamples, fp.samplePerm, noiseNx.ptr, noiseTrig.ptr);
+            hipLaunchKernelGGL(raygenKernel(), dim3(itemBlocks), dim3(kBlock), 0, stream, fp, scene, tileIds.ptr, io.ps, io.in, words.queueCount(0), counters.ptr);
         });
         for (io.bounce = 1; io.bounce <= numBounces; ++io.bounce)
         {
diff --git a/rayfinder_amd/csrc/rf_shade.hip b/rayfinder_amd/csrc/rf_shade.hip
--- a/rayfinder_amd/csrc/rf_shade.hip
+++ b/rayfinder_amd/csrc/rf_shade.hip
@@ -20,6 +20,18 @@
 }
 
 template<bool F32>
+__global__ __launch_bounds__(kBlock) void kNoiseTables(uint32_t firstFrame, FastDiv divSpp, uint32_t numSamples, const uint32_t* samplePerm, float* noiseNx, float2* noiseTrig)
+{
+    const uint32_t r = blockIdx.x * kBlock + threadIdx.x, b = blockIdx.y;
+    if (r >= numSamples) return;
+    const uint32_t frame = firstFrame + (samplePerm ? samplePerm[r] : r);
+    const uint32_t n = frame - divSpp.div(frame) * divSpp.divisor;
+    float          cosPhi, sinPhi;
+    blueNoiseTrig<F32>(blueNoiseY(b, n), cosPhi, sinPhi);
+    noiseNx[b * numSamples + r] = blueNoiseX(b, n);
+    noiseTrig[b * numSamples + r] = make_float2(cosPhi, sinPhi);
+}
+
 __global__ __launch_bounds__(kBlock) void kRaygen(FrameParams fp, DeviceScene scene, const uint32_t* tileIds, PathStreams ps,
                                                    uint32_t* queue, uint32_t* queueCount, DeviceCounters* counters)
 {
@@ -65,16 +77,17 @@
         if (!keep[k]) continue;
         const uint32_t x = px[k], y = py[k];
         const uint32_t frame = fp.firstFrame + (fp.samplePerm ? fp.samplePerm[sample[k]] : sample[k]);
-        float          nx, ny;
-        animatedBlueNoiseN(scene.blueNoise, x, y, frame - fp.divSamplesPerPixel.div(frame) * fp.samplesPerPixel, nx, ny);
+        const uint32_t n = frame - fp.divSamplesPerPixel.div(frame) * fp.samplesPerPixel;
+        const uint32_t key = noiseKey(sample[k], blueNoiseBytes(scene.blueNoise, x, y));
+        const float    nx = blueNoiseX(key & 255u, n), ny = blueNoiseY((key >> 8) & 255u, n);
 
         const float u = (static_cast<float>(x) + 0.5f) / static_cast<float>(fp.width);
         const float v = (static_cast<float>(y) + 0.5f) / static_cast<float>(fp.height);
         const float s = u + nx / static_cast<float>(fp.width);
         const float t = (1.0f - v) + ny / static_cast<float>(fp.height);
 
-        const float phi = 2.0f * kPi * ny;
-        const float cosPhi = tCos<F32>(phi), sinPhi = tSin<F32>(phi);
+        const Vec3  nz = expandNoiseKey(scene, key);
+        const float cosPhi = nz.y, sinPhi = nz.z;
         const float r = rf_sqrt(nx);
         const float lensX = fp.camera.lensRadius * (r * cosPhi);
         const float lensY = fp.camera.lensRadius * (r * sinPhi);
@@ -83,7 +96,7 @@
 
         if (!fp.skipOrigins) store3(ps.rayO + pos[k], origin);
         store3(ps.rayD + pos[k], dir);
-        store3(ps.noise + pos[k], vec3(nx, cosPhi, sinPhi));
+        ps.noise[pos[k]] = key;
     }
     (void)counters;
 }
@@ -112,7 +125,7 @@
     __shared__ uint32_t sHist[SORTED ? kSortBins : 1], sStart[SORTED ? kSortBins : 1], sPerm[SORTED ? kItems * kBlock : 1];
     __shared__ float    sLut[256];
     constexpr uint32_t  kTile = kItems * kBlock;
-    __shared__ float    sIn[SORTED ? 10 * kTile : 1];
+    __shared__ float    sIn[SORTED ? 8 * kTile : 1];
     const uint32_t      count = *queueCount;
     const uint32_t tiles = (count + kItems * kBlock - 1) / (kItems * kBlock);
     if (blockIdx.x >= tiles) return;
@@ -151,25 +164,26 @@
     }
     if constexpr (SORTED)
     {
-        Vec3 thrIn[kItems], noiseIn[kItems];
+        Vec3     thrIn[kItems];
+        uint32_t noiseIn[kItems];
 #pragma unroll
         for (int k = 0; k < kItems; ++k)
         {
             const uint32_t i = (tile * kItems + k) * kBlock + threadIdx.x;
             const uint32_t iL = isHit[k] ? i : 0u;
             thrIn[k] = isFirstBounce ? vec3(1.0f, 1.0f, 1.0f) : load3nt(ps.thr + iL);
-            noiseIn[k] = load3nt(ps.noise + iL);
+            noiseIn[k] = __builtin_nontemporal_load(ps.noise + iL);
         }
 #pragma unroll
         for (int k = 0; k < kItems; ++k)
         {
             if (!isHit[k]) continue;
             const uint32_t l = static_cast<uint32_t>(k) * kBlock + threadIdx.x;
-            const Vec3     t = thrIn[k], z = noiseIn[k], hitRec = hitRecs[k];
+            const Vec3     t = thrIn[k], hitRec = hitRecs[k];
             sIn[l] = t.x, sIn[kTile + l] = t.y, sIn[2 * kTile + l] = t.z;
-            sIn[3 * kTile + l] = z.x, sIn[4 * kTile + l] = z.y, sIn[5 * kTile + l] = z.z;
-            sIn[6 * kTile + l] = hitRec.x, sIn[7 * kTile + l] = hitRec.y, sIn[8 * kTile + l] = hitRec.z;
-            sIn[9 * kTile + l] = __uint_as_float(slots[k]);
+            sIn[3 * kTile + l] = __uint_as_float(noiseIn[k]);
+            sIn[4 * kTile + l] = hitRec.x, sIn[5 * kTile + l] = hitRec.y, sIn[6 * kTile + l] = hitRec.z;
+            sIn[7 * kTile + l] = __uint_as_float(slots[k]);
         }
     }
     uint32_t sortedHits = 0, sortedBase = 0;
@@ -223,7 +237,7 @@
             if (!isHit[k]) continue;
             const uint32_t local = sPerm[p];
             hitTri[k] = local;
-            slots[k] = __float_as_uint(sIn[9 * kTile + local]);
+            slots[k] = __float_as_uint(sIn[7 * kTile + local]);
             hitQueue[outPos[k]] = slots[k];
         }
         __syncthreads();
@@ -240,7 +254,7 @@
     if constexpr (kPipelined)
     {
 #pragma unroll
-        for (int k = 0; k < kItems; ++k) hits[k] = isHit[k] ? vec3(sIn[6 * kTile + hitTri[k]], sIn[7 * kTile + hitTri[k]], sIn[8 * kTile + hitTri[k]]) : Vec3{};
+        for (int k = 0; k < kItems; ++k) hits[k] = isHit[k] ? vec3(sIn[4 * kTile + hitTri[k]], sIn[5 * kTile + hitTri[k]], sIn[6 * kTile + hitTri[k]]) : Vec3{};
     }
     struct ShadeRecord
     {
@@ -281,20 +295,22 @@
             store3nt(ps.rayO + out, hp);
             shadowOrigin = hp;
         }
-        Vec3 throughput, nz;
+        Vec3     throughput;
+        uint32_t key;
         if constexpr (SORTED)
         {
             const uint32_t local = hitTri[k];
             throughput = vec3(sIn[local], sIn[kTile + local], sIn[2 * kTile + local]);
-            nz = vec3(sIn[3 * kTile + local], sIn[4 * kTile + local], sIn[5 * kTile + local]);
+            key = __float_as_uint(sIn[3 * kTile + local]);
         }
         else
         {
             throughput = isFirstBounce ? vec3(1.0f, 1.0f, 1.0f) : load3nt(ps.thr + i);
-            nz = load3nt(ps.noise + i);
-        }
+            key = __builtin_nontemporal_load(ps.noise + i);
+        }
+        __builtin_nontemporal_store(key, ps.noiseOut + out);
+        const Vec3  nz = expandNoiseKey(scene, key);
         const float nx = nz.x, cosPhi = nz.y, sinPhi = nz.z;
-        store3nt(ps.noiseOut + out, nz);
         const float4  a0 = cur.a0, a1 = cur.a1, a2 = cur.a2, a3 = cur.a3;
         const Vec3    n0 = vec3(a0.x, a0.y, a0.z), n1 = vec3(a0.w, a1.x, a1.y), n2 = vec3(a1.z, a1.w, a2.x);
         const float   b0 = 1.0f - hu - hv, b1 = hu, b2 = hv;
@@ -725,7 +741,8 @@
 namespace kern
 {
 SamplePermutationKernel samplePermutationKernel() { return kSamplePermutation; }
-RaygenKernel            raygenKernel(bool f32) { return f32 ? kRaygen<true> : kRaygen<false>; }
+NoiseTablesKernel       noiseTablesKernel(bool f32Transcendentals) { return f32Transcendentals ? kNoiseTables<true> : kNoiseTables<false>; }
+RaygenKernel            raygenKernel() { return kRaygen; }
 ShadeKernel             shadeKernel(bool sorted, bool aov) { return aov ? kShade<false, true> : sorted ? kShade<true, false> : kShade<false, false>; }
 SkyKernel               skyKernel(bool f32) { return f32 ? kSky<true> : kSky<false>; }
 BounceTotalsKernel      bounceTotalsKernel() { return kBounceTotals; }
diff --git a/rayfinder_amd/csrc/rf_trace.hip b/rayfinder_amd/csrc/rf_trace.hip
--- a/rayfinder_amd/csrc/rf_trace.hip
+++ b/rayfinder_amd/csrc/rf_trace.hip
@@ -49,7 +49,7 @@
     {
         const uint32_t slot = queue[i];
         const Vec3     o = load3(ps.rayO + i);
-        const Vec3     nz = load3(ps.noiseOut + i);
+        const Vec3     nz = expandNoiseKey(scene, ps.noiseOut[i]);
         const Vec3     l = sunSample(sky, sunBasis, nz.x, nz.y, nz.z);
         ClosestHit     h;
         const bool     occluded = traverse<true, COUNT>(scene, o, l, kTMax, &sStack[threadIdx.x], h, tc);
@@ -328,7 +328,7 @@
                 const Vec3 o = (!ANY_HIT && (flags & kFlagConstOrigin) != 0u) ? vec3(wide.constOriginX, wide.constOriginY, wide.constOriginZ) : load3s(ps.rayO + resultIndex);
                 if (ANY_HIT && !shadowDirFromStream)
                 {
-                    const Vec3 nz = load3s(ps.noiseOut + resultIndex);
+                    const Vec3 nz = expandNoiseKey(scene, loadQ(ps.noiseOut + resultIndex));
                     dir = sunSample(sky, sunBasis, nz.x, nz.y, nz.z);
                 }
                 const RayPrep ray = prepareRay(o, dir);
@@ -1312,7 +1312,7 @@
             uint32_t        e[kOccSlots];
             loadOccluderCell(cell, e);
             if (e[0] == 0u) continue;
-            const Vec3    nz = load3(ps.noiseOut + i);
+            const Vec3    nz = expandNoiseKey(scene, ps.noiseOut[i]);
             const Vec3    dir = sunSample(sky, sunBasis, nz.x, nz.y, nz.z);
             const RayPrep ray = prepareRay(o, dir);
             if (classifyRay(ray) != kRayPlain) continue;
@@ -1398,7 +1398,7 @@
             o = load3s(ps.rayO + idx);
             if (ANY_HIT && !shadowDirFromStream)
             {
-                const Vec3 nz = load3s(ps.noiseOut + idx);
+                const Vec3 nz = expandNoiseKey(scene, loadQ(ps.noiseOut + idx));
                 dir = sunSample(sky, sunBasis, nz.x, nz.y, nz.z);
             }
             else dir = load3s(ps.rayD + idx);
```
